# trevorcampbell/bayesian-coresets

Hardware: AMD Instinct MI355X
Metric: greedy coreset iterations/sec (N=10000000, d=512) (higher is better)
Workload: dtype f32 scan + f64 state

## Files before the change

bayesian-coresets_amd/bayesiancoresets_amd/_native.py:

```python
import ctypes
import os

import numpy as np

_HERE = os.path.dirname(os.path.abspath(__file__))
LIB_PATH = os.path.join(os.path.dirname(_HERE), "lib", "libbcx.so")
if not os.path.exists(LIB_PATH) and os.path.exists(os.path.join(_HERE, "_lib", "libbcx.so")):
    LIB_PATH = os.path.join(_HERE, "_lib", "libbcx.so")

ALG_GIGA, ALG_FW, ALG_OMP = 0, 1, 2
F32, F64, F16 = 0, 1, 2
OK, ERR_ARG, ERR_HIP, ERR_ZERO_ROW, ERR_ZERO_B, ERR_NOMEM, ERR_STATE, ERR_EXCHANGE, ERR_TIMEOUT = 0, -1, -2, -3, -4, -5, -6, -7, -8
IT_OK, IT_FAIL_SELECT, IT_FAIL_REWEIGHT, IT_FAIL_MONOTONE = 0, 1, 2, 3
REC_HDR = 4
LOAD_CENTER_ROWS = 1
MAX_ROW_LENGTH = 1048576
CHUNK_ROWS = 1024

SYMBOLS = (
    "bcx_create", "bcx_destroy", "bcx_last_error", "bcx_set_stream", "bcx_load_rows", "bcx_chunk_sums", "bcx_export_chunk_sums",
    "bcx_finalize", "bcx_build_begin", "bcx_step_scan", "bcx_step_apply", "bcx_build_enqueue", "bcx_build_poll",
    "bcx_step_scan_exact", "bcx_build_trace", "bcx_active_count", "bcx_get_weights", "bcx_error", "bcx_optimize",
    "bcx_reset", "bcx_reached_numeric_limit", "bcx_get_vector", "bcx_get_norms", "bcx_get_stored_rows", "bcx_argmax_correlation", "bcx_time_scan",
    "bcx_stats", "bcx_screen_stats", "bcx_screen4_stats", "bcx_screen_read", "bcx_screen4_read", "bcx_screen4_probe", "bcx_profile_scan", "bcx_profile_read", "bcx_version",
    "bcx_project_write", "bcx_project_colsum", "bcx_project_select", "bcx_project_last_error",
    "bcx_build_enqueue_exact", "bcx_exchange_export", "bcx_exchange_attach", "bcx_exchange_probe", "bcx_exchange_disable", "bcx_exchange_set_timeout",
    "bcx_set_check_monotone", "bcx_project_profile", "bcx_project_profile_read", "bcx_exchange_stats", "bcx_load_rows_flags", "bcx_project_write_raw", "bcx_omp_stats", "bcx_project_select_ws", "bcx_project_select_scratch_bytes",
    "bcx_project_moments", "bcx_project_colsum_moments", "bcx_project_moments_scratch_bytes",
    "bcx_project_colsum_moments_scratch_bytes", "bcx_gram", "bcx_gram_scratch_bytes", "bcx_gram_check",
    "bcx_project_colsum_moments_at", "bcx_project_points_colsum_moments", "bcx_linreg_posterior_draw", "bcx_sparsevi_adam_step",
    "bcx_linreg_posterior_apply", "bcx_linreg_posterior_apply_ok",
    "bcx_linreg_posterior_factor", "bcx_linreg_posterior_factor_scratch_bytes", "bcx_linreg_posterior_factor_status",
    "bcx_linreg_posterior_factor_clear_status",
    "bcx_linreg_posterior_draw_factored",
    "bcx_sparsevi_adam_step_ws", "bcx_sparsevi_adam_scratch_bytes", "bcx_standard_normal", "bcx_column_means",
    "bcx_center_rows", "bcx_row_sumsq", "bcx_project_write_points",
    "bcx_laplace_sampler", "bcx_laplace_sampler_ok", "bcx_laplace_sampler_lds_bytes",
    "bcx_project_grad_points", "bcx_psvi_gradient", "bcx_psvi_gradient_scratch_bytes",
    "bcx_gaussian_operand", "bcx_gaussian_first_moment", "bcx_gaussian_first_moment_scratch_bytes", "bcx_gaussian_colsum_moments",
    "bcx_gaussian_posterior_draw", "bcx_project_grad_points_gaussian", "bcx_psvi_gradient_gaussian",
    "bcx_psvi_adam_step",
    "bcx_project_colsum_rows", "bcx_project_select_rows_ws", "bcx_project_select_rows_scratch_bytes", "bcx_gather_rows",
    "bcx_log_joint_grad", "bcx_log_joint_grad_scratch_bytes", "bcx_hmc_coreset", "bcx_hmc_coreset_ok", "bcx_hmc_coreset_lds_bytes",
    "bcx_hmc_stream", "bcx_hmc_stream_scratch_bytes",
    "bcx_nuts_coreset", "bcx_nuts_coreset_ok", "bcx_nuts_coreset_lds_bytes",
    "bcx_nuts_adapt", "bcx_nuts_adapt_ok", "bcx_nuts_adapt_schedule",
    "bcx_nuts_batch", "bcx_nuts_batch_table_bytes",
    "bcx_nuts_stream", "bcx_nuts_stream_scratch_bytes",
    "bcx_log_predictive", "bcx_log_predictive_scratch_bytes",
    "bcx_laplace_sampler_stream", "bcx_laplace_stream_scratch_bytes",
    "bcx_quasi_newton_step", "bcx_quasi_newton_scratch_bytes",
    "bcx_cmc_advance", "bcx_cmc_advance_ok", "bcx_cmc_advance_lds_bytes", "bcx_cmc_state_bytes",
    "bcx_pair_stat", "bcx_pair_stat_scratch_bytes",
)


class Config(ctypes.Structure):
    _fields_ = [
        ("alg", ctypes.c_int32), ("store_dtype", ctypes.c_int32), ("keep_exact_rows", ctypes.c_int32),
        ("device", ctypes.c_int32), ("d", ctypes.c_int32), ("world_size", ctypes.c_int32),
        ("rank", ctypes.c_int32), ("refresh_every", ctypes.c_int32),
        ("n_local", ctypes.c_int64), ("n_global", ctypes.c_int64), ("row_offset", ctypes.c_int64),
    ]


class NutsProblem(ctypes.Structure):
    _fields_ = [
        ("w_dev", ctypes.c_void_p), ("pts_dev", ctypes.c_void_p), ("ldp", ctypes.c_int64),
        ("mu_dev", ctypes.c_void_p), ("W_dev", ctypes.c_void_p), ("ldw", ctypes.c_int64),
        ("k", ctypes.c_int32), ("index", ctypes.c_int32),
    ]


_lib = None


def ensure_ipc_mode():
    import logging
    cur = os.environ.get("HSA_ENABLE_IPC_MODE_LEGACY")
    if cur == "0":
        return True
    if os.environ.get("BCX_KEEP_IPC_MODE"):
        return False
    initialised = False
    try:
        import sys
        t = sys.modules.get("torch")
        initialised = bool(t is not None and t.cuda.is_initialized())
    except Exception:
        pass
    os.environ["HSA_ENABLE_IPC_MODE_LEGACY"] = "0"
    if initialised:
        logging.getLogger().warning("bayesiancoresets_amd: the HIP runtime was initialised before HSA_ENABLE_IPC_MODE_LEGACY=0 "
                                    "could be set (it was %r); peer mailboxes / RCCL between processes may fail -- export it "
                                    "before the first GPU call", cur)
    return not initialised


def load():
    global _lib
    if _lib is not None:
        return _lib
    if not os.path.exists(LIB_PATH):
        raise RuntimeError(
            "libbcx.so not found at %s -- build it with `make -C bayesian-coresets_amd` "
            "(or python -c 'import __graft_entry__ as g; g.build()'). There is no CPU fallback." % LIB_PATH)
    ensure_ipc_mode()
    if not os.environ.get("BCX_NO_TORCH_PRELOAD"):
        try:
            import torch
        except ImportError:
            pass
    lib = ctypes.CDLL(LIB_PATH)
    vp, i32, i64, dbl = ctypes.c_void_p, ctypes.c_int32, ctypes.c_int64, ctypes.c_double
    P = ctypes.POINTER
    lib.bcx_version.restype = ctypes.c_char_p
    lib.bcx_last_error.restype = ctypes.c_char_p
    lib.bcx_last_error.argtypes = [vp]
    sigs = {
        "bcx_create": [P(Config), P(vp)],
        "bcx_destroy": [vp],
        "bcx_set_stream": [vp, vp],
        "bcx_load_rows": [vp, vp, i32, i32, i64, i64, i64],
        "bcx_load_rows_flags": [vp, vp, i32, i32, i64, i64, i64, i32],
        "bcx_chunk_sums": [vp, P(vp), P(i64), P(i64)],
        "bcx_export_chunk_sums": [vp, vp, i64],
        "bcx_finalize": [vp, vp, vp, i64],
        "bcx_build_begin": [vp, i64, dbl, P(i32)],
        "bcx_step_scan": [vp, vp],
        "bcx_step_scan_exact": [vp, vp],
        "bcx_step_apply": [vp, vp],
        "bcx_build_enqueue": [vp, i64],
        "bcx_build_poll": [vp, P(i64), P(i32), P(i32)],
        "bcx_build_trace": [vp, vp, vp, vp, i64, P(i64)],
        "bcx_active_count": [vp, P(i64)],
        "bcx_get_weights": [vp, vp, vp, i64, P(i64)],
        "bcx_error": [vp, P(dbl)],
        "bcx_optimize": [vp, dbl, P(i32)],
        "bcx_reset": [vp],
        "bcx_set_check_monotone": [vp, i32],
        "bcx_reached_numeric_limit": [vp, P(i32)],
        "bcx_get_vector": [vp, i32, vp],
        "bcx_get_norms": [vp, i64, i64, vp],
        "bcx_get_stored_rows": [vp, i64, i64, vp, P(i32)],
        "bcx_argmax_correlation": [vp, vp, P(i64), P(dbl)],
        "bcx_time_scan": [vp, i32, i32, P(dbl), P(dbl)],
        "bcx_stats": [vp, P(i64), P(i64), P(i64)],
        "bcx_omp_stats": [vp, vp],
        "bcx_screen_stats": [vp, vp],
        "bcx_screen4_stats": [vp, vp],
        "bcx_screen_read": [vp, i64, i64, vp, vp, vp, P(i32)],
        "bcx_screen4_read": [vp, i64, i64, vp, vp, vp, P(i32)],
        "bcx_screen4_probe": [vp, vp, vp, P(i32), vp, vp, i32, vp],
        "bcx_profile_scan": [vp, i32],
        "bcx_profile_read": [vp, P(dbl), P(i64)],
        "bcx_build_enqueue_exact": [vp],
        "bcx_exchange_export": [vp, vp, i32],
        "bcx_exchange_attach": [vp, vp, i32, dbl],
        "bcx_exchange_probe": [vp, P(i32)],
        "bcx_exchange_disable": [vp],
        "bcx_exchange_set_timeout": [vp, dbl],
        "bcx_exchange_stats": [vp, P(i64), P(dbl), P(dbl), P(dbl), P(dbl), i32],
    }
    proj_common = [vp, i32, vp, i64, i64, i32, i32, vp, i32, i32, dbl]
    sigs["bcx_project_write"] = proj_common + [vp, i64, vp]
    sigs["bcx_project_write_raw"] = proj_common + [vp, i64]
    sigs["bcx_project_write_points"] = proj_common + [vp, i64, i32]
    sigs["bcx_project_colsum"] = proj_common + [vp, vp]
    sigs["bcx_project_select"] = proj_common + [vp, dbl, vp, vp]
    sigs["bcx_project_select_ws"] = proj_common + [vp, dbl, vp, vp, i64]
    sigs["bcx_project_colsum_rows"] = proj_common + [vp, i64, vp, vp]
    sigs["bcx_project_select_rows_ws"] = proj_common + [vp, i64, vp, dbl, vp, vp, i64]
    sigs["bcx_gather_rows"] = [vp, vp, i64, i32, vp, i64, vp, i64]
    sigs["bcx_project_profile"] = [i32]
    sigs["bcx_project_profile_read"] = [P(dbl), P(i64), P(dbl)]
    sigs["bcx_project_moments"] = [vp, vp, i64, i64, i32, vp, i64, vp, i64]
    sigs["bcx_project_colsum_moments"] = [vp, vp, i64, i32, i32, vp, i32, i32, dbl, vp, vp]
    sigs["bcx_project_colsum_moments_at"] = [vp, vp, i64, i32, i32, vp, i32, i32, dbl, vp, vp, vp]
    sigs["bcx_project_points_colsum_moments"] = [vp, vp, i64, i64, i32, i32, vp, i32, i32, dbl, vp, i64, vp, i64, i32, vp, vp, vp]
    sigs["bcx_linreg_posterior_draw"] = [vp, i32, i32, i32, vp, vp, vp, vp, vp, vp, vp, vp, dbl, vp, vp, i32, vp, vp]
    sigs["bcx_linreg_posterior_apply"] = [vp, i32, i32, i32, vp, vp, vp, vp, vp, vp, vp, dbl, vp, vp, i32, vp, vp, vp]
    sigs["bcx_linreg_posterior_apply_ok"] = [i32, i32]
    sigs["bcx_sparsevi_adam_step"] = [vp, i32, i32, vp, dbl, vp, i64, vp, vp, vp, vp, i32, dbl, dbl, dbl, vp, i32]
    sigs["bcx_gram"] = [vp, vp, i32, i32, i64, vp, i64, vp, i64]
    sigs["bcx_gram_check"] = [vp, vp]
    sigs["bcx_linreg_posterior_factor"] = [vp, i32, i32, i32, vp, vp, vp, vp, i32, vp, dbl, vp, i64, vp, i64, vp, vp]
    sigs["bcx_linreg_posterior_factor_status"] = [vp, i32, vp]
    sigs["bcx_linreg_posterior_factor_clear_status"] = [vp, i32, vp]
    sigs["bcx_standard_normal"] = [vp, ctypes.c_uint64, ctypes.c_uint64, i64, vp]
    sigs["bcx_column_means"] = [vp, vp, i32, i32, i32, i64, vp, i64]
    sigs["bcx_center_rows"] = [vp, vp, i64, i32, i64]
    sigs["bcx_laplace_sampler"] = [vp, i32, i32, i32, vp, vp, i64, vp, i32, dbl, i32, vp, vp, i32, i32, vp, vp, vp]
    sigs["bcx_laplace_sampler_ok"] = [i32, i32]
    lib.bcx_laplace_sampler_lds_bytes.restype = ctypes.c_int64
    lib.bcx_laplace_sampler_lds_bytes.argtypes = [i32, i32]
    sigs["bcx_laplace_sampler_stream"] = sigs["bcx_laplace_sampler"] + [vp, i64]
    lib.bcx_laplace_stream_scratch_bytes.restype = ctypes.c_int64
    lib.bcx_laplace_stream_scratch_bytes.argtypes = [i32, i32]
    sigs["bcx_row_sumsq"] = [vp, vp, i64, i32, i64, vp]
    sigs["bcx_project_grad_points"] = [vp, i32, vp, i32, i64, i32, i32, vp, i32, i32, dbl, vp, vp]
    sigs["bcx_psvi_gradient"] = [vp, i32, vp, i32, i64, i32, i32, vp, i32, i32, dbl, vp, vp, i64, vp, dbl, vp, vp]
    sigs["bcx_gaussian_operand"] = [vp, vp, i32, i64, i32, vp, i64, vp, vp, i64, i32, vp]
    sigs["bcx_gaussian_first_moment"] = [vp, vp, i64, i64, i32, vp, vp, i64]
    lib.bcx_gaussian_first_moment_scratch_bytes.restype = ctypes.c_int64
    lib.bcx_gaussian_first_moment_scratch_bytes.argtypes = [i64, i32]
    sigs["bcx_gaussian_colsum_moments"] = [vp, vp, dbl, i32, vp, i32, i64, vp]
    sigs["bcx_gaussian_posterior_draw"] = [vp, i32, i32, vp, vp, i64, vp, vp, vp, vp, vp, vp, vp, i32, i32, vp, vp, vp, vp]
    sigs["bcx_project_grad_points_gaussian"] = [vp, vp, i32, i64, i32, vp, i32, i64, vp, vp]
    sigs["bcx_psvi_gradient_gaussian"] = [vp, vp, i32, i64, i32, vp, i32, i64, vp, vp, i64, vp, dbl, vp, vp]
    sigs["bcx_psvi_adam_step"] = [vp, i32, i32, vp, i32, vp, vp, i64, vp, vp, vp, i32, dbl, dbl, dbl, vp, i64, vp, vp]
    sigs["bcx_log_joint_grad"] = [vp, i32, vp, i64, i64, i32, vp, vp, i32, i32, vp, vp, vp]
    lib.bcx_log_joint_grad_scratch_bytes.restype = ctypes.c_int64
    lib.bcx_log_joint_grad_scratch_bytes.argtypes = [i64, i32, i32]
    hmc_common = [vp, vp, i64, i32, i32, i32, i32, dbl, dbl, vp, i32, vp, vp, vp, vp, vp, vp, vp]
    sigs["bcx_hmc_coreset"] = [vp, i32, i32, i32, vp, vp, i64] + hmc_common
    sigs["bcx_hmc_stream"] = [vp, i32, i64, i32, vp, vp, i64] + hmc_common + [vp, i64]
    sigs["bcx_hmc_coreset_ok"] = [i32, i32]
    lib.bcx_hmc_coreset_lds_bytes.restype = ctypes.c_int64
    lib.bcx_hmc_coreset_lds_bytes.argtypes = [i32, i32]
    sigs["bcx_cmc_advance"] = [vp, i32, i32, i32, vp, vp, i64, vp, vp, i64, i32, i32, i32, dbl, i32, i32, i32, vp, vp, vp, i64, i64, vp, i64,
                               vp, i64, vp, i32, vp, vp, vp, vp, vp]
    sigs["bcx_cmc_advance_ok"] = [i32, i32]
    lib.bcx_cmc_advance_lds_bytes.restype = ctypes.c_int64
    lib.bcx_cmc_advance_lds_bytes.argtypes = [i32, i32]
    lib.bcx_cmc_state_bytes.restype = ctypes.c_int64
    lib.bcx_cmc_state_bytes.argtypes = [i32]
    sigs["bcx_nuts_coreset"] = [vp, i32, i32, i32, vp, vp, i64, vp, vp, i64, i32, i32, i32, i32, dbl, dbl, vp, i64, i32, vp, vp, vp, vp, vp, vp, vp]
    sigs["bcx_nuts_coreset_ok"] = [i32, i32]
    lib.bcx_nuts_coreset_lds_bytes.restype = ctypes.c_int64
    lib.bcx_nuts_coreset_lds_bytes.argtypes = [i32, i32]
    sigs["bcx_nuts_adapt"] = sigs["bcx_nuts_coreset"] + [i32, vp, vp]
    sigs["bcx_nuts_adapt_ok"] = [i32, i32]
    sigs["bcx_nuts_adapt_schedule"] = [i32, ctypes.POINTER(ctypes.c_int32), i32]
    sigs["bcx_nuts_batch"] = [vp, i32, i32, ctypes.POINTER(NutsProblem), vp, i32, i32, i32, i32, i32, dbl, vp, i64, i32, vp, vp, vp, vp, vp, vp,
                              vp, i32, vp, vp]
    lib.bcx_nuts_batch_table_bytes.restype = ctypes.c_int64
# ... 232 lines not shown
            if done < itrs and not limit:
                self.enqueue(itrs - done)
        return self.trace(itrs)

    def sparse_weights(self):
        k = ctypes.c_int64()
        self._check(self.lib.bcx_active_count(self.h, ctypes.byref(k)))
        idx = np.empty(k.value, dtype=np.int64)
        w = np.empty(k.value, dtype=np.float64)
        if k.value:
            self._check(self.lib.bcx_get_weights(self.h, idx.ctypes.data, w.ctypes.data, k.value, ctypes.byref(k)))
        return idx, w

    def error(self):
        e = ctypes.c_double()
        self._check(self.lib.bcx_error(self.h, ctypes.byref(e)))
        return e.value

    def optimize(self, tol):
        acc = ctypes.c_int32()
        self._check(self.lib.bcx_optimize(self.h, tol, ctypes.byref(acc)))
        return bool(acc.value)

    def reset(self):
        self._check(self.lib.bcx_reset(self.h))

    def set_check_monotone(self, on):
        self._check(self.lib.bcx_set_check_monotone(self.h, int(bool(on))))

    def reached_numeric_limit(self):
        v = ctypes.c_int32()
        self._check(self.lib.bcx_reached_numeric_limit(self.h, ctypes.byref(v)))
        return bool(v.value)

    def vector(self, which):
        out = np.empty(self.d, dtype=np.float64)
        self._check(self.lib.bcx_get_vector(self.h, which, out.ctypes.data))
        return out

    def norms(self, begin=0, count=None):
        count = self.n_local - begin if count is None else count
        out = np.empty(count, dtype=np.float64)
        if count:
            self._check(self.lib.bcx_get_norms(self.h, begin, count, out.ctypes.data))
        return out

    def stored_rows(self, begin=0, count=None):
        count = self.n_local - begin if count is None else count
        ld = ctypes.c_int32()
        self._check(self.lib.bcx_get_stored_rows(self.h, begin, 0, None, ctypes.byref(ld)))
        dt = {F64: np.float64, F16: np.float16}.get(self.cfg.store_dtype, np.float32)
        out = np.empty((count, ld.value), dtype=dt)
        if count:
            self._check(self.lib.bcx_get_stored_rows(self.h, begin, count, out.ctypes.data, ctypes.byref(ld)))
        return out[:, :self.d]

    def argmax_correlation(self, query):
        q = np.ascontiguousarray(query, dtype=np.float64)
        assert q.shape == (self.d,)
        idx, score = ctypes.c_int64(), ctypes.c_double()
        self._check(self.lib.bcx_argmax_correlation(self.h, ctypes.c_void_p(q.ctypes.data), ctypes.byref(idx),
                                                    ctypes.byref(score)))
        return idx.value, score.value

    def time_scan(self, reps=20, exact=False):
        ms, by = ctypes.c_double(), ctypes.c_double()
        self._check(self.lib.bcx_time_scan(self.h, reps, int(exact), ctypes.byref(ms), ctypes.byref(by)))
        return ms.value, by.value

    def stats(self):
        a, b, c = ctypes.c_int64(), ctypes.c_int64(), ctypes.c_int64()
        self._check(self.lib.bcx_stats(self.h, ctypes.byref(a), ctypes.byref(b), ctypes.byref(c)))
        return {"exact_fallbacks": a.value, "candidates": b.value, "resolves": c.value}

    SCREEN_DROP = {0: "in use", 1: "dropped by the overflow rule until reset()", 2: "no device memory for the shadow",
                   3: "switched off or not applicable"}

    SCREEN4_STATE = {0: "in use", 1: "dropped to 8-bit", 2: "no device memory for the second shadow",
                     3: "switched off or not applicable"}

    def screen_stats(self):
        out = (ctypes.c_int64 * 8)()
        self._check(self.lib.bcx_screen_stats(self.h, out))
        o4 = (ctypes.c_int64 * 8)()
        self._check(self.lib.bcx_screen4_stats(self.h, o4))
        return {"active": bool(out[0]), "screened": out[1], "survivors": out[2], "overflows": out[3], "storage_redos": out[4],
                "state": self.SCREEN_DROP.get(int(out[5]), "?"), "device_bytes": out[6], "build_us": out[7],
                "front4_active": bool(o4[0]), "front4_iterations": o4[1], "front4_listed": o4[2], "front4_overflows": o4[3],
                "front4_redos": o4[4], "front4_state": self.SCREEN4_STATE.get(int(o4[5]), "?"), "front4_device_bytes": o4[6],
                "front4_drops": o4[7]}

    def screen_read(self, begin=0, count=None):
        count = self.n_local - begin if count is None else count
        ld8 = (self.d + 15) // 16 * 16
        codes = np.empty((count, ld8), dtype=np.uint8)
        sc = np.empty(count, dtype=np.float32)
        bd = np.empty(count, dtype=np.float32)
        got = ctypes.c_int32()
        self._check(self.lib.bcx_screen_read(self.h, begin, count, codes.ctypes.data, sc.ctypes.data, bd.ctypes.data,
                                             ctypes.byref(got)))
        assert got.value == ld8
        return codes, sc, bd

    def screen4_read(self, begin=0, count=None):
        count = self.n_local - begin if count is None else count
        ld4 = (self.d + 31) // 32 * 16
        codes = np.empty((count, ld4), dtype=np.uint8)
        sc = np.empty(count, dtype=np.float32)
        bd = np.empty(count, dtype=np.float32)
        got = ctypes.c_int32()
        self._check(self.lib.bcx_screen4_read(self.h, begin, count, codes.ctypes.data, sc.ctypes.data, bd.ctypes.data,
                                              ctypes.byref(got)))
        assert got.value == ld4
        return codes, sc, bd

    SCREEN4_MAX_WAVES = 2048

    def screen4_probe(self, query, sentinels, list_stride=1024):
        q = np.ascontiguousarray(query, dtype=np.float64)
        sent = np.ascontiguousarray(sentinels, dtype=np.int32)
        assert q.shape == (self.d,) and sent.shape == (64,)
        cap = self.SCREEN4_MAX_WAVES
        nw = ctypes.c_int32()
        counts = np.zeros(cap, dtype=np.int32)
        lst = np.full((cap, list_stride), -1, dtype=np.int32)
        raw = np.zeros(cap * 40, dtype=np.uint8)
        self._check(self.lib.bcx_screen4_probe(self.h, q.ctypes.data, sent.ctypes.data, ctypes.byref(nw), counts.ctypes.data,
                                               lst.ctypes.data, list_stride, raw.ctypes.data))
        n = nw.value
        dbl = raw[:32 * n].view(np.float64).reshape(4, n)
        idx = raw[32 * n:40 * n].view(np.int32).reshape(2, n)
        return {"counts": counts[:n].copy(), "list": lst[:n].copy(), "U1": dbl[0].copy(), "U2": dbl[1].copy(), "U3": dbl[2].copy(),
                "L": dbl[3].copy(), "i1": idx[0].copy(), "i2": idx[1].copy()}

    def omp_stats(self):
        out = (ctypes.c_int64 * 4)()
        self._check(self.lib.bcx_omp_stats(self.h, out))
        return {"steps": out[0], "columns_left": out[1], "resolves": out[2], "extra_entered": out[3]}

    def profile(self, on):
        self._check(self.lib.bcx_profile_scan(self.h, int(on)))

    def profile_read(self):
        ms, n = ctypes.c_double(), ctypes.c_int64()
        self._check(self.lib.bcx_profile_read(self.h, ctypes.byref(ms), ctypes.byref(n)))
        return ms.value, n.value


def device_row_sumsq(rows):
    import torch
    lib = load()
    if rows.dtype != torch.float64 or rows.stride(1) != 1:
        rows = rows.to(torch.float64).contiguous()
    out = torch.empty(rows.shape[0], dtype=torch.float64, device=rows.device)
    with torch.cuda.device(rows.device):
        rc = lib.bcx_row_sumsq(int(torch.cuda.current_stream(rows.device).cuda_stream), rows.data_ptr(), rows.shape[0], rows.shape[1],
                               rows.stride(0), out.data_ptr())
    if rc != 0:
        raise EngineError(rc, lib.bcx_project_last_error().decode())
    return out.cpu().numpy()


def device_centred_copy(rows):
    import torch
    lib = load()
    out = rows.to(torch.float64).contiguous().clone()
    with torch.cuda.device(out.device):
        rc = lib.bcx_center_rows(int(torch.cuda.current_stream(out.device).cuda_stream), out.data_ptr(), out.shape[0], out.shape[1], out.stride(0))
    if rc != 0:
        raise EngineError(rc, lib.bcx_project_last_error().decode())
    return out
```

bayesian-coresets_amd/csrc/api.hip:

```cpp
#include <stdio.h>
#include <string.h>
#include <algorithm>
#include <cmath>
#include "bcx_internal.h"
#include "dev_util.h"

static thread_local std::string g_create_err;
namespace {
void bounce_acquire(int device);
void bounce_release(int device);
}

extern "C" const char* bcx_version(void) { return "bcx 0.1 gfx950"; }

extern "C" const char* bcx_last_error(const bcx_solver* s) { return s ? s->err.c_str() : g_create_err.c_str(); }

template <typename T> static hipError_t dev_alloc(T** p, size_t count, bool zero = true) {
  *p = nullptr;
  if (count == 0) count = 1;
  hipError_t e = hipMalloc((void**)p, count * sizeof(T));
  if (e != hipSuccess) return e;
  if (zero) e = hipMemset(*p, 0, count * sizeof(T));
  return e;
}

static int round_up(int x, int m) { return (x + m - 1) / m * m; }

static void free_all(bcx_solver* s) {
  void* ptrs[] = {s->An, s->A64, s->norms, s->chunk_sums, s->staging, s->st, s->b, s->bn, s->xw, s->q64, s->qst,
                  s->tmp, s->partials, s->rec_local, s->act_idx, s->act_w, s->act_rows, s->act_norm, s->gram,
                  s->hinv, s->hinv_lo, s->cvec, s->plist, s->ppos, s->nn_x, s->nn_z, s->nn_wv, s->nn_tmp, s->nn_flag, s->nn_wbak, s->nn_xr, s->tr_sel, s->tr_err,
                  s->tr_status};
  for (void* p : ptrs)
    if (p) (void)hipFree(p);
  for (size_t w = 0; w < s->peer_mbox.size(); ++w)
    if (s->peer_mbox[w] && s->peer_mbox[w] != s->mbox) (void)hipIpcCloseMemHandle(s->peer_mbox[w]);
  void* xptrs[] = {s->mbox, s->peer_tab, s->xseq, s->xprobe, s->rec_gather, s->grid_counter, s->fin_part, s->gram_work, s->warm_buf,
                   s->Aq, s->scr_sb, s->scr_partials, s->scr_stat, s->A4, s->s4_sb, s->s4_list, s->s4_counts, s->s4_sent};
  for (void* p : xptrs)
    if (p) (void)hipFree(p);
  for (auto& ev : s->prof_events) { (void)hipEventDestroy(ev.first); (void)hipEventDestroy(ev.second); }
}

extern "C" int bcx_create(const bcx_config* cfg, bcx_solver** out) {
  if (!cfg || !out) { g_create_err = "bcx_create: null argument"; return BCX_ERR_ARG; }
  *out = nullptr;
  if (cfg->alg < BCX_ALG_GIGA || cfg->alg > BCX_ALG_OMP || cfg->d < 1 || cfg->n_local < 0 ||
      cfg->world_size < 1 || cfg->rank < 0 || cfg->rank >= cfg->world_size ||
      (cfg->store_dtype != BCX_F32 && cfg->store_dtype != BCX_F64 && cfg->store_dtype != BCX_F16)) {
    g_create_err = "bcx_create: invalid configuration";
    return BCX_ERR_ARG;
  }
  const int maxd = BCX_MAX_D;
  if (cfg->d > maxd) { g_create_err = "bcx_create: d exceeds the supported row length (" + std::to_string(maxd) + ")"; return BCX_ERR_ARG; }
  if (cfg->n_local >= (int64_t)0x7fffffff) { g_create_err = "bcx_create: n_local must be < 2^31 per shard"; return BCX_ERR_ARG; }
  if (cfg->row_offset % BCX_CHUNK_ROWS != 0) {
    g_create_err = "bcx_create: row_offset must be a multiple of the chunk size (1024 rows)";
    return BCX_ERR_ARG;
  }
  bcx_solver* s = new bcx_solver();
  s->cfg = *cfg;
  if (s->cfg.refresh_every == 0) s->cfg.refresh_every = 64;
  if (const char* e = bcx_dev_env("BCX_SCREEN8")) s->scr_enabled = atoi(e) != 0;
  if (const char* e = bcx_dev_env("BCX_SCREEN4_SEGCAP")) { const int v = atoi(e); if (v >= 1 && v <= BCX_S4_SEG_CAP) s->s4_seg_cap = v; }
  if (const char* e = bcx_dev_env("BCX_SCREEN4")) s->s4_enabled = atoi(e) != 0;
  hipError_t e = hipSetDevice(cfg->device);
  if (e != hipSuccess) { g_create_err = std::string("hipSetDevice: ") + hipGetErrorString(e); delete s; return BCX_ERR_HIP; }
  const int d = cfg->d;
  const int64_t n = cfg->n_local;
  s->elem = cfg->store_dtype == BCX_F32 ? 4 : (cfg->store_dtype == BCX_F16 ? 2 : 8);
  s->qelem = cfg->store_dtype == BCX_F64 ? 8 : 4;
  s->ld = round_up(d, 16 / s->elem);
  s->ld64 = round_up(d, 2);
  s->n_chunks = (n + BCX_CHUNK_ROWS - 1) / BCX_CHUNK_ROWS;
  bool ok = true;
  auto chk = [&](hipError_t r) { if (r != hipSuccess && ok) { ok = false; g_create_err = std::string("hipMalloc: ") + hipGetErrorString(r); } };
  chk(dev_alloc((char**)&s->An, (size_t)n * s->ld * s->elem));
  if (cfg->keep_exact_rows && cfg->store_dtype != BCX_F64) chk(dev_alloc(&s->A64, (size_t)n * s->ld64));
  chk(dev_alloc(&s->norms, (size_t)n));
  chk(dev_alloc(&s->chunk_sums, (size_t)s->n_chunks * (d + 1)));
  chk(dev_alloc(&s->st, 1));
  chk(dev_alloc(&s->b, (size_t)d));
  chk(dev_alloc(&s->bn, (size_t)d));
  chk(dev_alloc(&s->xw, (size_t)d));
  chk(dev_alloc(&s->q64, (size_t)2 * s->ld64));
  chk(dev_alloc((char**)&s->qst, (size_t)2 * s->ld * s->qelem));
  chk(dev_alloc(&s->tmp, (size_t)20 * d));
  s->n_partials = 0;
  chk(dev_alloc((char**)&s->partials, (size_t)bcx_scan_grid(s) * BCX_PARTIAL_BYTES));
  chk(dev_alloc(&s->rec_local, (size_t)(d + BCX_REC_HDR)));
  if (!ok) { free_all(s); delete s; return BCX_ERR_NOMEM; }
  bounce_acquire(cfg->device);
  *out = s;
  return BCX_OK;
}

extern "C" int bcx_destroy(bcx_solver* s) {
  if (!s) return BCX_OK;
  (void)hipSetDevice(s->cfg.device);
  (void)hipDeviceSynchronize();
  free_all(s);
  bounce_release(s->cfg.device);
  delete s;
  return BCX_OK;
}

extern "C" int bcx_set_stream(bcx_solver* s, void* hip_stream) {
  if (!s) return BCX_ERR_ARG;
  s->stream = (hipStream_t)hip_stream;
  return BCX_OK;
}

static int read_state(bcx_solver* s, DevState* h);

#include <mutex>
#include <thread>
namespace {
constexpr size_t kBounceBytes = (size_t)32 << 20;
constexpr int kMaxDevices = 64;
struct Bounce {
  std::mutex mu;
  void* buf[2] = {nullptr, nullptr};
  int users = 0;
};
Bounce g_bounce[kMaxDevices];
Bounce& bounce_of(int device) { return g_bounce[(device >= 0 && device < kMaxDevices) ? device : 0]; }
void bounce_acquire(int device) {
  Bounce& b = bounce_of(device);
  std::lock_guard<std::mutex> lock(b.mu);
  b.users += 1;
}
void bounce_release(int device) {
  Bounce& b = bounce_of(device);
  std::lock_guard<std::mutex> lock(b.mu);
  if (--b.users <= 0) {
    b.users = 0;
    for (int i = 0; i < 2; ++i)
      if (b.buf[i]) { (void)hipHostFree(b.buf[i]); b.buf[i] = nullptr; }
  }
}

void copy_rows_mt(char* dst, size_t dpitch, const char* src, size_t spitch, size_t width, int64_t rows) {
  const size_t bytes = (size_t)rows * width;
  int nt = (int)std::min<size_t>(8, bytes / ((size_t)2 << 20));
  const unsigned hw = std::thread::hardware_concurrency();
  if (hw && (unsigned)nt > hw) nt = (int)hw;
  auto work = [=](int64_t r0, int64_t r1) {
// ... 265 lines not shown
  s->prof_now = (s->prof_tick++ % s->prof_every) == 0;
  if (!s->prof_now) return BCX_OK;
  if (s->prof_used == s->prof_events.size()) {
    hipEvent_t a, b;
    BCX_HIP(hipEventCreate(&a));
    BCX_HIP(hipEventCreate(&b));
    s->prof_events.emplace_back(a, b);
  }
  BCX_HIP(hipEventRecord(s->prof_events[s->prof_used].first, s->stream));
  return BCX_OK;
}
static int prof_end(bcx_solver* s) {
  if (!s->profile || !s->prof_now) return BCX_OK;
  BCX_HIP(hipEventRecord(s->prof_events[s->prof_used].second, s->stream));
  s->prof_used++;
  return BCX_OK;
}

static int step_scan(bcx_solver* s, void* send_dev, int exact, bool with_tail) {
  if (!s->finalized) { s->err = "solver not finalized"; return BCX_ERR_STATE; }
  double* send = send_dev ? (double*)send_dev : s->rec_local;
  int rc;
  if (exact && (rc = bcx_launch_resume_exact(s))) return rc;
  if ((rc = prof_begin(s))) return rc;
  if ((rc = bcx_launch_scan(s, exact))) return rc;
  if ((rc = prof_end(s))) return rc;
  if (with_tail) return bcx_launch_tail(s, exact);
  return bcx_launch_resolve(s, send, exact);
}

static int front_scan(bcx_solver* s, int exact, bool tier, bool four) {
  int rc;
  if (exact && (rc = bcx_launch_resume_exact(s))) return rc;
  if ((rc = prof_begin(s))) return rc;
  if ((rc = (tier && !exact) ? (four ? bcx_launch_screen4(s) : bcx_launch_screen(s)) : bcx_launch_scan(s, exact))) return rc;
  return prof_end(s);
}

extern "C" int bcx_step_scan(bcx_solver* s, void* send_dev) { if (s) s->scr_batch = false; return s ? step_scan(s, send_dev, 0, false) : BCX_ERR_ARG; }
extern "C" int bcx_step_scan_exact(bcx_solver* s, void* send_dev) { if (s) s->scr_batch = false; return s ? step_scan(s, send_dev, 1, false) : BCX_ERR_ARG; }

extern "C" int bcx_step_apply(bcx_solver* s, const void* recv_dev) {
  if (!s) return BCX_ERR_ARG;
  return bcx_launch_apply(s, recv_dev ? (const double*)recv_dev : s->rec_local);
}

static int enqueue_one_launch(bcx_solver* s, int exact, bool tier, bool four) {
  if (!s->finalized) { s->err = "solver not finalized"; return BCX_ERR_STATE; }
  int rc;
  if (s->cfg.world_size != 1) {
    if (!s->exchange_ready) {
      s->err = "bcx_build_enqueue on a row shard needs bcx_exchange_attach (or drive bcx_step_scan / bcx_step_apply)";
      return BCX_ERR_ARG;
    }
    if ((rc = front_scan(s, exact, tier, false))) return rc;
    return bcx_launch_tail_exchange(s, exact);
  }
  if ((rc = front_scan(s, exact, tier, four))) return rc;
  if (s->cfg.alg == BCX_ALG_OMP) {
    rc = bcx_launch_omp_fused(s, exact);
    if (rc != 1) return rc;
    if ((rc = bcx_launch_resolve(s, s->rec_local, exact))) return rc;
    return bcx_launch_apply(s, s->rec_local);
  }
  return bcx_launch_tail(s, exact);
}

static int enqueue_one(bcx_solver* s, int exact, bool tier, bool four = false) {
  const int rc = enqueue_one_launch(s, exact, tier, four);
  if (rc == BCX_OK) s->enq_unpolled = true;
  return rc;
}

static int enqueue_many(bcx_solver* s, int64_t itrs) {
  int rc = bcx_screen_build(s);
  if (rc != BCX_OK) return rc;
  const bool tier = bcx_screen_on(s) && s->scr_valid;
  if (tier && (rc = bcx_screen4_build(s))) return rc;
  const bool tier4 = tier && bcx_screen4_on(s) && s->s4_valid;
  s->scr_batch = false;
  for (int64_t i = 0; i < itrs; ++i) {
    s->scr_batch = tier;
    const bool four = tier4 && s->s4_warm == 0;
    rc = enqueue_one(s, 0, tier, four);
    if (rc != BCX_OK) return rc;
    if (tier && s->s4_warm > 0) s->s4_warm -= 1;
  }
  return BCX_OK;
}

extern "C" int bcx_build_enqueue(bcx_solver* s, int64_t itrs) {
  if (!s) return BCX_ERR_ARG;
  if (!s->finalized) { s->err = "solver not finalized"; return BCX_ERR_STATE; }
  return enqueue_many(s, itrs);
}

extern "C" int bcx_build_enqueue_exact(bcx_solver* s) {
  if (!s) return BCX_ERR_ARG;
  if (!s->finalized) { s->err = "solver not finalized"; return BCX_ERR_STATE; }
  s->scr_batch = false;
  return enqueue_one(s, 1, false);
}

static int mailbox_alloc(bcx_solver* s) {
  if (s->mbox) return BCX_OK;
  const int world = s->cfg.world_size;
  const size_t bytes = bcx_mailbox_slot_offset(world) + 2 * (size_t)world * (s->cfg.d + BCX_REC_HDR) * sizeof(double);
  hipError_t e = hipExtMallocWithFlags(&s->mbox, bytes, hipDeviceMallocFinegrained);
  if (e != hipSuccess) {
    (void)hipGetLastError();
    s->mbox = nullptr;
    s->err = std::string("peer mailbox: fine-grained allocation failed: ") + hipGetErrorString(e);
    return BCX_ERR_HIP;
  }
  s->mbox_bytes = bytes;
  BCX_HIP(hipMemset(s->mbox, 0, bytes));
  BCX_HIP(hipDeviceSynchronize());
  return BCX_OK;
}

extern "C" int bcx_exchange_export(bcx_solver* s, void* handle_out, int32_t handle_bytes) {
  if (!s || !handle_out) return BCX_ERR_ARG;
  if (handle_bytes < (int32_t)sizeof(hipIpcMemHandle_t)) { s->err = "bcx_exchange_export: handle buffer too small"; return BCX_ERR_ARG; }
  if ((size_t)s->cfg.d * sizeof(double) > 144 * 1024) {
    s->err = "peer mailbox: rows of more than 18432 values exchange their records through the all-gather";
    return BCX_ERR_ARG;
  }
  BCX_HIP(hipSetDevice(s->cfg.device));
  int rc = mailbox_alloc(s);
  if (rc != BCX_OK) return rc;
  hipIpcMemHandle_t h;
  BCX_HIP(hipIpcGetMemHandle(&h, s->mbox));
  memset(handle_out, 0, handle_bytes);
  memcpy(handle_out, &h, sizeof(h));
  return BCX_OK;
}

extern "C" int bcx_exchange_attach(bcx_solver* s, const void* handles, int32_t handle_bytes, double timeout_s) {
  if (!s || !handles) return BCX_ERR_ARG;
  if (s->exchange_ready) return BCX_OK;
  if (!s->mbox) { s->err = "bcx_exchange_attach: call bcx_exchange_export first"; return BCX_ERR_STATE; }
  if (handle_bytes < (int32_t)sizeof(hipIpcMemHandle_t)) return BCX_ERR_ARG;
  BCX_HIP(hipSetDevice(s->cfg.device));
  const int world = s->cfg.world_size;
  if (world > BCX_APPLY_THREADS) { s->err = "peer mailbox supports at most 256 shards"; return BCX_ERR_ARG; }
  s->peer_mbox.assign(world, nullptr);
  for (int w = 0; w < world; ++w) {
    if (w == s->cfg.rank) { s->peer_mbox[w] = s->mbox; continue; }
    hipIpcMemHandle_t h;
    memcpy(&h, (const char*)handles + (size_t)w * handle_bytes, sizeof(h));
    hipError_t e = hipIpcOpenMemHandle(&s->peer_mbox[w], h, hipIpcMemLazyEnablePeerAccess);
    if (e != hipSuccess) {
      (void)hipGetLastError();
      s->peer_mbox[w] = nullptr;
      s->err = "peer mailbox: cannot map shard " + std::to_string(w) + ": " + hipGetErrorString(e);
      for (int v = 0; v < w; ++v)
        if (v != s->cfg.rank && s->peer_mbox[v]) { (void)hipIpcCloseMemHandle(s->peer_mbox[v]); s->peer_mbox[v] = nullptr; }
      s->peer_mbox.clear();
      return BCX_ERR_HIP;
    }
  }
  hipError_t e;
  if ((e = dev_alloc(&s->peer_tab, (size_t)world)) != hipSuccess || (e = dev_alloc(&s->xseq, 8)) != hipSuccess ||
      (e = dev_alloc(&s->xprobe, 1)) != hipSuccess ||
      (e = dev_alloc(&s->rec_gather, (size_t)world * (s->cfg.d + BCX_REC_HDR))) != hipSuccess) {
    s->err = std::string("peer mailbox: ") + hipGetErrorString(e);
    return BCX_ERR_NOMEM;
// ... 250 lines not shown
  BCX_HIP(hipSetDevice(s->cfg.device));
  DevState h;
  int rc = read_state(s, &h);
  if (rc != BCX_OK) return rc;
  DevState forced = h;
  forced.active = 1;
  BCX_HIP(hipMemcpy(s->st, &forced, sizeof forced, hipMemcpyHostToDevice));
  hipEvent_t e0, e1;
  BCX_HIP(hipEventCreate(&e0));
  BCX_HIP(hipEventCreate(&e1));
  for (int i = 0; i < 3 && rc == BCX_OK; ++i) rc = bcx_launch_scan(s, exact);
  if (rc == BCX_OK) (void)hipEventRecord(e0, s->stream);
  for (int i = 0; i < reps && rc == BCX_OK; ++i) rc = bcx_launch_scan(s, exact);
  if (rc != BCX_OK) {
    (void)hipEventDestroy(e0); (void)hipEventDestroy(e1);
    (void)hipMemcpy(s->st, &h, sizeof h, hipMemcpyHostToDevice);
    return rc;
  }
  BCX_HIP(hipEventRecord(e1, s->stream));
  BCX_HIP(hipEventSynchronize(e1));
  float ms = 0.f;
  BCX_HIP(hipEventElapsedTime(&ms, e0, e1));
  BCX_HIP(hipEventDestroy(e0));
  BCX_HIP(hipEventDestroy(e1));
  BCX_HIP(hipMemcpy(s->st, &h, sizeof h, hipMemcpyHostToDevice));
  if (ms_per_launch) *ms_per_launch = (double)ms / reps;
  const bool raw64 = exact && s->cfg.store_dtype != BCX_F64 && s->A64;
  if (bytes_per_launch) *bytes_per_launch = (double)s->cfg.n_local * s->cfg.d * (raw64 ? 8.0 : (double)s->elem);
  return BCX_OK;
}

static int upload_query(bcx_solver* s, const double* query_host, bool with64, double* qn_out, int* E_out) {
  const int d = s->cfg.d;
  std::vector<double> q64((size_t)s->ld64, 0.0);
  double qmax = 0.0;
  for (int j = 0; j < d; ++j) { q64[j] = query_host[j]; qmax = std::fmax(qmax, std::fabs(query_host[j])); }
  const bool scalable = qmax > 0.0 && qmax < INFINITY;
  const int E0 = scalable ? std::ilogb(qmax) : 0;
  double qn = 0.0;
  for (int j = 0; j < d; ++j) { const double t = std::ldexp(query_host[j], -E0); qn += t * t; }
  qn = std::sqrt(qn);
  int E = 0;
  if (with64) BCX_HIP(hipMemcpy(s->q64, q64.data(), (size_t)s->ld64 * 8, hipMemcpyHostToDevice));
  if (s->cfg.store_dtype == BCX_F64) {
    std::vector<double> qs((size_t)s->ld, 0.0);
    for (int j = 0; j < d; ++j) qs[j] = query_host[j];
    BCX_HIP(hipMemcpy(s->qst, qs.data(), (size_t)s->ld * 8, hipMemcpyHostToDevice));
    qn = std::ldexp(qn, E0);
  } else {
    const int E1 = (scalable && qn > 0.0 && qn < INFINITY) ? std::ilogb(qn) : 0;
    E = E0 + E1;
    std::vector<float> qs((size_t)s->ld, 0.f);
    for (int j = 0; j < d; ++j) qs[j] = (float)std::ldexp(query_host[j], -E);
    BCX_HIP(hipMemcpy(s->qst, qs.data(), (size_t)s->ld * 4, hipMemcpyHostToDevice));
    qn = std::ldexp(qn, -E1);
  }
  *qn_out = qn; *E_out = E;
  return BCX_OK;
}

extern "C" int bcx_argmax_correlation(bcx_solver* s, const double* query_host, int64_t* idx, double* score) {
  if (!s || !query_host || !idx || !score) return BCX_ERR_ARG;
  if (!s->finalized) { s->err = "solver not finalized"; return BCX_ERR_STATE; }
  if (s->cfg.alg == BCX_ALG_GIGA) { s->err = "bcx_argmax_correlation needs a single-query solver (FW/OMP)"; return BCX_ERR_ARG; }
  BCX_HIP(hipSetDevice(s->cfg.device));
  DevState h;
  int rc = read_state(s, &h);
  if (rc != BCX_OK) return rc;
  double qn = 0.0;
  int E = 0;
  if ((rc = upload_query(s, query_host, true, &qn, &E))) return rc;
  DevState forced = h;
  forced.active = 1; forced.exact_mode = 0; forced.qscale = qn; forced.qexp = E;
  double rec[BCX_REC_HDR];
  for (int attempt = 0; attempt < 2; ++attempt) {
    forced.exact_mode = attempt;
    BCX_HIP(hipMemcpy(s->st, &forced, sizeof forced, hipMemcpyHostToDevice));
    if ((rc = bcx_launch_scan(s, attempt))) return rc;
    if ((rc = bcx_launch_resolve(s, s->rec_local, attempt))) return rc;
    BCX_HIP(hipStreamSynchronize(s->stream));
    BCX_HIP(hipMemcpy(rec, s->rec_local, sizeof rec, hipMemcpyDeviceToHost));
    if (rec[3] != BCX_REC_OVERFLOW) break;
  }
  BCX_HIP(hipMemcpy(s->st, &h, sizeof h, hipMemcpyHostToDevice));
  if (rec[3] != BCX_REC_VALID) { s->err = "no rows to scan"; return BCX_ERR_STATE; }
  *idx = (int64_t)rec[1];
  *score = rec[0];
  return BCX_OK;
}

extern "C" int bcx_stats(bcx_solver* s, int64_t* exact_fallbacks, int64_t* candidates, int64_t* resolves) {
  if (!s) return BCX_ERR_ARG;
  DevState h;
  int rc = read_state(s, &h);
  if (rc != BCX_OK) return rc;
  if (exact_fallbacks) *exact_fallbacks = h.n_exact;
  if (candidates) *candidates = h.n_cand;
  if (resolves) *resolves = h.n_resolved;
  return BCX_OK;
}

extern "C" int bcx_screen_stats(bcx_solver* s, int64_t* out8) {
  if (!s || !out8) return BCX_ERR_ARG;
  unsigned long long st8[SCR_WORDS] = {0, 0, 0, 0, 0, 0, 0, 0};
  if (s->scr_stat) {
    BCX_HIP(hipSetDevice(s->cfg.device));
    BCX_HIP(hipStreamSynchronize(s->stream));
    BCX_HIP(hipMemcpy(st8, s->scr_stat, sizeof st8, hipMemcpyDeviceToHost));
  }
  const bool possible = s->scr_enabled && s->cfg.store_dtype != BCX_F64 && s->cfg.d <= 4096 && s->cfg.n_local > 0;
  out8[0] = bcx_screen_on(s) ? 1 : 0;
  out8[1] = (int64_t)st8[SCR_ITERS];
  out8[2] = (int64_t)st8[SCR_SURVIVORS];
  out8[3] = (int64_t)st8[SCR_OVERFLOWS];
  out8[4] = (int64_t)st8[SCR_REDOS];
  out8[5] = !possible ? 3 : s->scr_dropped;
  out8[6] = s->Aq ? (int64_t)s->scr_cap_rows * (s->ld8 + 8) + (int64_t)BCX_MAX_PARTIALS * BCX_PARTIAL_BYTES + SCR_WORDS * 8 : 0;
  out8[7] = (int64_t)(s->scr_build_ms * 1e3f);
  return BCX_OK;
}

extern "C" int bcx_screen4_stats(bcx_solver* s, int64_t* out8) {
  if (!s || !out8) return BCX_ERR_ARG;
  unsigned long long st8[SCR_WORDS];
  for (auto& w : st8) w = 0;
  if (s->scr_stat) {
    BCX_HIP(hipSetDevice(s->cfg.device));
    BCX_HIP(hipStreamSynchronize(s->stream));
    BCX_HIP(hipMemcpy(st8, s->scr_stat, sizeof st8, hipMemcpyDeviceToHost));
  }
  const bool possible = s->s4_enabled && s->scr_enabled && s->cfg.store_dtype != BCX_F64 && s->cfg.d <= 4096 && s->cfg.n_local > 0 &&
                        s->cfg.alg != BCX_ALG_GIGA && s->cfg.world_size == 1;
  out8[0] = bcx_screen4_on(s) ? 1 : 0;
  out8[1] = (int64_t)st8[SCR4_ITERS];
  out8[2] = (int64_t)st8[SCR4_LISTED];
  out8[3] = (int64_t)st8[SCR4_OVERFLOWS];
  out8[4] = s->s4_redos;
  out8[5] = !possible ? 3 : s->s4_dropped;
  out8[6] = s->A4 ? (int64_t)s->s4_cap_rows * (s->ld4 + 8) + (int64_t)BCX_MAX_PARTIALS * (BCX_S4_SEG_CAP + 1) * 4 : 0;
  out8[7] = s->s4_drops;
  return BCX_OK;
}

extern "C" int bcx_screen_read(bcx_solver* s, int64_t begin, int64_t count, void* codes, float* scales, float* bounds, int32_t* ld8_out) {
  if (!s || begin < 0 || count < 0 || begin + count > s->cfg.n_local) return BCX_ERR_ARG;
  if (!s->finalized) { s->err = "solver not finalized"; return BCX_ERR_STATE; }
  BCX_HIP(hipSetDevice(s->cfg.device));
  int rc = bcx_screen_build(s);
  if (rc != BCX_OK) return rc;
  if (!bcx_screen_on(s) || !s->scr_valid) { s->err = "bcx_screen_read: the 8-bit tier is not in use"; return BCX_ERR_STATE; }
  BCX_HIP(hipStreamSynchronize(s->stream));
  if (ld8_out) *ld8_out = s->ld8;
  if (count == 0) return BCX_OK;
  if (codes) BCX_HIP(hipMemcpy(codes, (const char*)s->Aq + (size_t)begin * s->ld8, (size_t)count * s->ld8, hipMemcpyDeviceToHost));
  std::vector<float> sb((size_t)count * 2);
  BCX_HIP(hipMemcpy(sb.data(), (const char*)s->scr_sb + (size_t)begin * 8, (size_t)count * 8, hipMemcpyDeviceToHost));
  for (int64_t i = 0; i < count; ++i) {
    if (scales) scales[i] = sb[2 * i];
    if (bounds) bounds[i] = sb[2 * i + 1];
  }
  return BCX_OK;
}

static int screen4_ready(bcx_solver* s, const char* who) {
  if (!s->finalized) { s->err = "solver not finalized"; return BCX_ERR_STATE; }
  BCX_HIP(hipSetDevice(s->cfg.device));
  int rc = bcx_screen_build(s);
  if (rc != BCX_OK) return rc;
  if (bcx_screen_on(s) && s->scr_valid && (rc = bcx_screen4_build(s))) return rc;
  if (!bcx_screen_on(s) || !s->scr_valid || !bcx_screen4_on(s) || !s->s4_valid) {
    s->err = std::string(who) + ": the 4-bit front pass is not in use";
    return BCX_ERR_STATE;
  }
  return BCX_OK;
}

extern "C" int bcx_screen4_read(bcx_solver* s, int64_t begin, int64_t count, void* codes, float* scales, float* bounds, int32_t* ld4_out) {
  if (!s || begin < 0 || count < 0 || begin + count > s->cfg.n_local) return BCX_ERR_ARG;
  int rc = screen4_ready(s, "bcx_screen4_read");
  if (rc != BCX_OK) return rc;
  BCX_HIP(hipStreamSynchronize(s->stream));
  if (ld4_out) *ld4_out = s->ld4;
  if (count == 0) return BCX_OK;
  if (codes) BCX_HIP(hipMemcpy(codes, (const char*)s->A4 + (size_t)begin * s->ld4, (size_t)count * s->ld4, hipMemcpyDeviceToHost));
  std::vector<float> sb((size_t)count * 2);
  BCX_HIP(hipMemcpy(sb.data(), (const char*)s->s4_sb + (size_t)begin * 8, (size_t)count * 8, hipMemcpyDeviceToHost));
  for (int64_t i = 0; i < count; ++i) {
    if (scales) scales[i] = sb[2 * i];
    if (bounds) bounds[i] = sb[2 * i + 1];
  }
  return BCX_OK;
}

extern "C" int bcx_screen4_probe(bcx_solver* s, const double* query_host, const int32_t* sentinels, int32_t* n_waves_out,
                                 int32_t* counts, int32_t* list, int32_t list_stride, void* partials) {
  if (!s || !query_host || !sentinels || !n_waves_out || list_stride < 0) return BCX_ERR_ARG;
  for (int i = 0; i < BCX_S4_SENTINELS; ++i)
    if (!(sentinels[i] == -1 || (sentinels[i] >= 0 && (int64_t)sentinels[i] < s->cfg.n_local))) {
      s->err = "bcx_screen4_probe: sentinel " + std::to_string(i) + " is neither -1 nor a local row";
      return BCX_ERR_ARG;
    }
  if (s->enq_unpolled) { s->err = "bcx_screen4_probe: iterations are enqueued; call bcx_build_poll first"; return BCX_ERR_STATE; }
  int rc = screen4_ready(s, "bcx_screen4_probe");
  if (rc != BCX_OK) return rc;
  DevState h;
  if ((rc = read_state(s, &h))) return rc;
  BCX_HIP(hipStreamSynchronize(s->stream));
  int32_t sent_was[BCX_S4_SENTINELS];
  std::vector<char> q_was((size_t)s->ld * 4);
  BCX_HIP(hipMemcpy(sent_was, s->s4_sent, sizeof sent_was, hipMemcpyDeviceToHost));
  BCX_HIP(hipMemcpy(q_was.data(), s->qst, q_was.size(), hipMemcpyDeviceToHost));
  double qn = 0.0;
  int E = 0;
  if ((rc = upload_query(s, query_host, false, &qn, &E))) return rc;
  DevState forced = h;
  forced.active = 1; forced.exact_mode = 0; forced.qscale = qn; forced.qexp = E;
  BCX_HIP(hipMemcpy(s->st, &forced, sizeof forced, hipMemcpyHostToDevice));
  BCX_HIP(hipMemcpy(s->s4_sent, sentinels, sizeof sent_was, hipMemcpyHostToDevice));
  int nw = 0;
  rc = bcx_launch_front4_probe(s, &nw);
  hipError_t e = hipStreamSynchronize(s->stream);
  BCX_HIP(hipMemcpy(s->st, &h, sizeof h, hipMemcpyHostToDevice));
  BCX_HIP(hipMemcpy(s->s4_sent, sent_was, sizeof sent_was, hipMemcpyHostToDevice));
  BCX_HIP(hipMemcpy(s->qst, q_was.data(), q_was.size(), hipMemcpyHostToDevice));
  if (rc != BCX_OK) return rc;
  BCX_HIP(e);
  *n_waves_out = nw;
  std::vector<int32_t> cnt((size_t)nw);
  BCX_HIP(hipMemcpy(cnt.data(), s->s4_counts, (size_t)nw * 4, hipMemcpyDeviceToHost));
  if (counts) memcpy(counts, cnt.data(), (size_t)nw * 4);
  if (list && list_stride > 0) {
    std::vector<int32_t> all((size_t)nw * BCX_S4_SEG_CAP);
    BCX_HIP(hipMemcpy(all.data(), s->s4_list, all.size() * 4, hipMemcpyDeviceToHost));
    for (int b = 0; b < nw; ++b) {
      int m = cnt[b] < s->s4_seg_cap ? cnt[b] : s->s4_seg_cap;
      if (m > list_stride) m = list_stride;
      if (m > 0) memcpy(list + (size_t)b * list_stride, all.data() + (size_t)b * BCX_S4_SEG_CAP, (size_t)m * 4);
    }
  }
  if (partials) BCX_HIP(hipMemcpy(partials, s->scr_partials, (size_t)nw * BCX_PARTIAL_BYTES, hipMemcpyDeviceToHost));
  return BCX_OK;
}

extern "C" int bcx_omp_stats(bcx_solver* s, int64_t* out4) {
  if (!s || !out4) return BCX_ERR_ARG;
  DevState h;
  int rc = read_state(s, &h);
  if (rc != BCX_OK) return rc;
  for (int i = 0; i < 4; ++i) out4[i] = h.n_omp[i];
  out4[2] += s->opt_fallbacks;
  return BCX_OK;
}

extern "C" int bcx_profile_scan(bcx_solver* s, int32_t on) {
  if (!s) return BCX_ERR_ARG;
  s->profile = on != 0;
  s->prof_every = on > 1 ? on : 1;
  s->prof_tick = 0;
  s->prof_ms = 0.0;
  s->prof_launches = 0;
  s->prof_used = 0;
  return BCX_OK;
}

extern "C" int bcx_profile_read(bcx_solver* s, double* scan_ms_total, int64_t* scan_launches) {
  if (!s) return BCX_ERR_ARG;
  if (scan_ms_total) *scan_ms_total = s->prof_ms;
  if (scan_launches) *scan_launches = s->prof_launches;
  return BCX_OK;
}

extern "C" int bcx_debug_stamps(bcx_solver* s, long long* out32) {
  DevState h;
  int rc = read_state(s, &h);
  if (rc != BCX_OK) return rc;
  for (int i = 0; i < 32; ++i) out32[i] = h.dbg_t[i];
  return BCX_OK;
}

extern "C" int bcx_debug_wbak(bcx_solver* s, double* out, int32_t count) {
  if (!s || !s->nn_wbak || count > s->gram_cap) return BCX_ERR_ARG;
  BCX_HIP(hipDeviceSynchronize());
  BCX_HIP(hipMemcpy(out, s->nn_wbak, (size_t)count * sizeof(double), hipMemcpyDeviceToHost));
  return BCX_OK;
}
```

bayesian-coresets_amd/csrc/apply_common.h:

```cpp
#pragma once
#include "bcx_internal.h"
#include "dev_util.h"

struct ApplyArgs {
  DevState* st;
  const double* recs;
  int world;
  int d, ld, ld64;
  int alg;
  int store_f64;
  int refresh_every;
  const double* b;
  const double* bn;
  double* xw;
  double* q64;
  void* qst;
  double* tmp;
  int64_t cap;
  int64_t* act_idx;
  double* act_w;
  double* act_rows;
  double* act_norm;
  int64_t* tr_sel;
  double* tr_err;
  int32_t* tr_status;
};

static __device__ __forceinline__ int query_exponent(const ApplyArgs& a, double qnorm) {
  return (a.store_f64 || !(qnorm > 0.0) || !(qnorm < INFINITY)) ? 0 : ilogb(qnorm);
}

static __device__ __forceinline__ void store_query(const ApplyArgs& a, int which, int j, double v, int E = 0) {
  a.q64[(size_t)which * a.ld64 + j] = v;
  if (a.store_f64) ((double*)a.qst)[(size_t)which * a.ld + j] = v;
  else ((float*)a.qst)[(size_t)which * a.ld + j] = (float)(E ? ldexp(v, -E) : v);
}

static __device__ __forceinline__ void set_query_scale(DevState* st, double qnorm, int E) {
  st->qscale = E ? ldexp(qnorm, -E) : qnorm;
  st->qexp = E;
}

static __device__ bool prepare_query(const ApplyArgs& a, double* scratch) {
  DevState* st = a.st;
  const int d = a.d;
  if (a.alg != BCX_ALG_GIGA) {
    const double qn = st->err;
    const int E = query_exponent(a, qn);
    for (int j = threadIdx.x; j < d; j += blockDim.x) store_query(a, 0, j, a.b[j] - a.xw[j], E);
    if (threadIdx.x == 0) set_query_scale(st, qn, E);
    return true;
  }
  const double nw = st->nw;
  double v[1] = {0.0};
  for (int j = threadIdx.x; j < d; j += blockDim.x) v[0] += a.bn[j] * (a.xw[j] / nw);
  block_allsum<1>(v, scratch);
  const double t = v[0];
  double c2[1] = {0.0};
  for (int j = threadIdx.x; j < d; j += blockDim.x) {
    const double xh = a.xw[j] / nw;
    const double c = a.bn[j] - t * xh;
    a.tmp[j] = c;
    c2[0] += c * c;
  }
  block_allsum<1>(c2, scratch);
  const double cn = sqrt(c2[0]);
  if (cn < st->tol) return false;
  for (int j = threadIdx.x; j < d; j += blockDim.x) {
    store_query(a, 0, j, a.tmp[j] / cn);
    store_query(a, 1, j, a.xw[j] / nw);
  }
  if (threadIdx.x == 0) set_query_scale(st, 1.0, 0);
  return true;
}

static __device__ void refresh_state(const ApplyArgs& a, double* scratch, bool recompute_xw) {
  DevState* st = a.st;
  const int d = a.d, k = st->k;
  double v[2] = {0.0, 0.0};
  for (int j = threadIdx.x; j < d; j += blockDim.x) {
    double x;
    if (recompute_xw) {
      x = 0.0;
      int s = 0;
      for (; s + 8 <= k; s += 8) {
        double r[8], w[8];
#pragma unroll
        for (int t = 0; t < 8; ++t) { w[t] = a.act_w[s + t]; r[t] = a.act_rows[(size_t)(s + t) * d + j]; }
#pragma unroll
        for (int t = 0; t < 8; ++t) x += w[t] * r[t];
      }
      for (; s < k; ++s) x += a.act_w[s] * a.act_rows[(size_t)s * d + j];
      a.xw[j] = x;
    } else {
      x = a.xw[j];
    }
    const double r = x - a.b[j];
    v[0] += r * r;
    v[1] += x * x;
  }
  block_allsum<2>(v, scratch);
  if (threadIdx.x == 0) {
    st->err = sqrt(v[0]);
    const double nw = sqrt(v[1]);
    st->nw = (nw == 0.0) ? 1.0 : nw;
    if (recompute_xw) st->since_refresh = 0;
  }
  __syncthreads();
}

static __device__ void prepare_next(const ApplyArgs& a, double* scratch) {
  DevState* st = a.st;
  __shared__ int go;
  for (;;) {
    __syncthreads();
    if (threadIdx.x == 0) {
      go = 1;
      if (st->it >= st->itrs) { st->active = 0; st->halt = HALT_DONE; go = 0; }
    }
    __syncthreads();
    if (!go) return;
    if (a.refresh_every > 0 && st->since_refresh >= a.refresh_every) refresh_state(a, scratch, true);
    const bool ok = prepare_query(a, scratch);
    if (ok) return;
    __syncthreads();
    if (threadIdx.x == 0) {
      const int64_t it = st->it;
      a.tr_sel[it] = -1; a.tr_err[it] = st->err; a.tr_status[it] = BCX_IT_FAIL_SELECT;
      st->it = it + 1;
      if (st->retried) { st->limit = 1; st->active = 0; st->halt = HALT_LIMIT; go = 0; }
      else st->retried = 1;
    }
    __syncthreads();
    if (!go) return;
  }
}


static inline void fill_apply_args(bcx_solver* s, ApplyArgs& a, const double* recs) {
  a.st = s->st;
  a.recs = recs;
  a.world = s->cfg.world_size;
  a.d = s->cfg.d; a.ld = s->ld; a.ld64 = s->ld64;
  a.alg = s->cfg.alg;
  a.store_f64 = s->cfg.store_dtype == BCX_F64;
  a.refresh_every = s->cfg.refresh_every;
  a.b = s->b; a.bn = s->bn; a.xw = s->xw; a.q64 = s->q64; a.qst = s->qst; a.tmp = s->tmp;
  a.cap = s->cap;
  a.act_idx = s->act_idx; a.act_w = s->act_w; a.act_rows = s->act_rows; a.act_norm = s->act_norm;
  a.tr_sel = s->tr_sel; a.tr_err = s->tr_err; a.tr_status = s->tr_status;
}
```

bayesian-coresets_amd/csrc/bcx_internal.h:

```cpp
#pragma once
#include <hip/hip_runtime.h>
#include <stdint.h>
#include <string>
#include <utility>
#include <vector>
#include "../../include/bcx.h"

#define BCX_CHUNK_ROWS 1024
#define BCX_MAX_CAND 64
#define BCX_REC_HDR 4
#define BCX_REC_VALID 1.0
#define BCX_REC_OVERFLOW 2.0
#define BCX_MAX_D BCX_MAX_ROW_LENGTH
#define BCX_SCAN_THREADS 256
#define BCX_APPLY_THREADS 256

enum { HALT_NONE = 0, HALT_DONE = 1, HALT_LIMIT = 2, HALT_NEED_EXACT = 3, HALT_EXCHANGE_TIMEOUT = 4, HALT_GRID_TIMEOUT = 5 };
enum { OMP_IDLE = 0, OMP_DONE = 1, OMP_FAST_TRY = 2, OMP_FAST_ACCEPT = 3, OMP_GENERAL = 4,
       OMP_OPT_FALLBACK = 5 };

struct PartialView {
  double *U1, *U2, *U3, *L;
  int32_t *i1, *i2;
};
#define BCX_PARTIAL_BYTES 40
#define BCX_MAX_PARTIALS 2048
#define BCX_SCREEN_MAX_SURV 256
enum { SCR_ARMED = 0,
       SCR_ITERS = 1,
       SCR_SURVIVORS = 2,
       SCR_OVERFLOWS = 3,
       SCR_REDOS = 4,
       SCR4_ITERS = 5,
       SCR4_LISTED = 6,
       SCR4_OVERFLOWS = 7,
       SCR4_LAST = 8,
       SCR_WORDS = 9 };
#define BCX_S4_SEG_CAP 1024
#define BCX_S4_SENTINELS 64
static inline __host__ __device__ PartialView partial_view(void* base, int n) {
  PartialView v;
  v.U1 = (double*)base; v.U2 = v.U1 + n; v.U3 = v.U2 + n; v.L = v.U3 + n;
  v.i1 = (int32_t*)(v.L + n); v.i2 = v.i1 + n;
  return v;
}

struct Mailbox {
  void* const* peers;
  unsigned long long* seq;
  int32_t* probe;
  unsigned long long* stat;
  int world, rank, recw;
  unsigned off_slots;
  long long timeout_ticks;
};

static inline unsigned bcx_mailbox_slot_offset(int world) { return (unsigned)((2u * world * 8u + 255u) / 256u * 256u); }

struct DevState {
  int64_t itrs;
  int64_t it;
  int32_t active;
  int32_t halt;
  int32_t retried;
  int32_t limit;
  int32_t k;
  int32_t since_refresh;
  int32_t exact_mode;
  int32_t zero_row;
  int32_t no_monotone;
  int32_t np;
  int32_t hvalid;
  int32_t hlo_valid;
  int32_t omp_mode;
  int32_t omp_slot, omp_fresh, omp_checked, omp_p;
  int32_t omp_ill;
  int64_t omp_f;
  double omp_nf, omp_gff, omp_cf, omp_t, omp_inv;
  double tol;
  double err;
  double nw;
  double bnorm;
  double sigma;
  int64_t n_exact;
  int64_t n_cand;
  int64_t n_resolved;
  int64_t n_omp[4];
  double qscale;
  int32_t qexp;
  int32_t qexp_pad;
  long long dbg_t[32];
};

struct bcx_solver {
  bcx_config cfg;
  hipStream_t stream = nullptr;
  std::string err;
  int ld = 0;
  int elem = 4;
  int qelem = 4;
  int ld64 = 0;
  void* An = nullptr;
  double* A64 = nullptr;
  double* norms = nullptr;
  double* chunk_sums = nullptr;
  int64_t n_chunks = 0;
  void* staging = nullptr;
  size_t staging_bytes = 0;
  DevState* st = nullptr;
  double* b = nullptr;
  double* bn = nullptr;
  double* xw = nullptr;
  double* q64 = nullptr;
  void* qst = nullptr;
  double* tmp = nullptr;
  void* partials = nullptr;
  int n_partials = 0;
  double* rec_local = nullptr;
  double* fin_part = nullptr;
  int64_t fin_cap = 0;
  void* mbox = nullptr;
  size_t mbox_bytes = 0;
  std::vector<void*> peer_mbox;
  void** peer_tab = nullptr;
  unsigned long long* xseq = nullptr;
  int32_t* xprobe = nullptr;
  double* rec_gather = nullptr;
  bool exchange_ready = false;
  double exchange_timeout_s = 20.0;
  int64_t cap = 0;
  int64_t* act_idx = nullptr;
  double* act_w = nullptr;
  double* act_rows = nullptr;
  double* act_norm = nullptr;
  double* gram = nullptr;
  double* hinv = nullptr;
  double* hinv_lo = nullptr;
  double* cvec = nullptr;
  int32_t* plist = nullptr;
  int32_t* ppos = nullptr;
  double* nn_x = nullptr;
  double* nn_z = nullptr;
  double* nn_wv = nullptr;
  double* nn_tmp = nullptr;
  int32_t* nn_flag = nullptr;
  double* nn_wbak = nullptr;
  double* nn_xr = nullptr;
  int64_t gram_cap = 0;
  double* gram_work = nullptr;
  size_t gram_work_bytes = 0;
  void* warm_buf = nullptr;
  size_t warm_bytes = 0;
  int64_t opt_warm = 0, opt_warm_failed = 0;
  int64_t k_ub = 0;
  unsigned long long* grid_counter = nullptr;
  uint64_t grid_epoch = 0;
  int64_t opt_fallbacks = 0;
  bool grid_dirty = false;
  size_t omp_lds_allowed = 0;
  int64_t trace_cap = 0;
  int64_t* tr_sel = nullptr;
  double* tr_err = nullptr;
  int32_t* tr_status = nullptr;
  bool finalized = false;
  int64_t rows_loaded = 0;
  void* Aq = nullptr;
  void* scr_sb = nullptr;
  void* scr_partials = nullptr;
  unsigned long long* scr_stat = nullptr;
  int ld8 = 0;
  int64_t scr_cap_rows = 0;
  bool scr_enabled = true;
  int scr_dropped = 0;
  bool scr_valid = false;
  bool scr_batch = false;
  float scr_build_ms = 0.f;
  uint64_t scr_ovf_at[4] = {0, 0, 0, 0};
  int64_t scr_halts = 0;
  int scr_n_in = 0;
  void* A4 = nullptr;
  void* s4_sb = nullptr;
  void* s4_list = nullptr;
  void* s4_counts = nullptr;
  void* s4_sent = nullptr;
  int ld4 = 0;
  int s4_seg_cap = BCX_S4_SEG_CAP;
  int64_t s4_cap_rows = 0;
  bool s4_enabled = true;
  int s4_dropped = 0;
  bool s4_valid = false;
  int s4_warm = 2;
  uint64_t s4_ovf_at[4] = {0, 0, 0, 0};
  int64_t s4_halts = 0;
  int64_t s4_redos = 0, s4_drops = 0;
  bool enq_unpolled = false;
  bool profile = false;
  bool prof_now = false;
  int prof_every = 1;
  int64_t prof_tick = 0;
  double prof_ms = 0.0;
  int64_t prof_launches = 0;
  std::vector<std::pair<hipEvent_t, hipEvent_t>> prof_events;
  size_t prof_used = 0;
};

int bcx_launch_ingest(bcx_solver* s, const void* src, int src_dtype, int64_t ld_src, int64_t row_begin, int64_t rows,
                      int center);
int bcx_launch_finalize(bcx_solver* s, int have_b, const double* gathered, int64_t n_gathered);
int bcx_launch_scan(bcx_solver* s, int exact);
int bcx_launch_resolve(bcx_solver* s, double* send_dev, int exact);
int bcx_launch_begin(bcx_solver* s, int64_t itrs, double tol);
int bcx_launch_apply(bcx_solver* s, const double* recv_dev);
int bcx_launch_tail(bcx_solver* s, int exact);
int bcx_launch_omp_fused(bcx_solver* s, int exact);
int bcx_launch_tail_exchange(bcx_solver* s, int exact);
int bcx_launch_exchange_probe(bcx_solver* s);
Mailbox bcx_mailbox(const bcx_solver* s);
int bcx_launch_resume_exact(bcx_solver* s);
int bcx_launch_error_refresh(bcx_solver* s);
int bcx_launch_optimize(bcx_solver* s, double tol);
int64_t bcx_gram_rows_scratch_bytes(int k, int d);
int bcx_gram_rows(hipStream_t st, const double* rows, int k, int d, int64_t ld, double* G, int64_t ldg, double* work);
int64_t bcx_gram_tiled_scratch_bytes(int k, int d);
int bcx_gram_rows_tiled(hipStream_t st, const double* rows, int k, int d, int64_t ld, double* G, int64_t ldg, double* work);
unsigned long long bcx_gram_sk_epoch_now();
int bcx_gram_sk_timed_out(hipStream_t st, const double* work, unsigned long long since);
int bcx_scan_grid(const bcx_solver* s);
bool bcx_screen_on(const bcx_solver* s);
int bcx_screen_build(bcx_solver* s);
int bcx_launch_screen(bcx_solver* s);
int bcx_launch_resume_store(bcx_solver* s);
int bcx_launch_refine(bcx_solver* s, int n_in, bool four);
bool bcx_screen4_on(const bcx_solver* s);
int bcx_screen4_build(bcx_solver* s);
int bcx_launch_screen4(bcx_solver* s);
int bcx_launch_front4_probe(bcx_solver* s, int* n_waves);
void bcx_project_set_error(const std::string& msg);
const double* proj_tables();

#ifdef BCX_TIMING
#define BCX_STAMP(st, i) do { if (threadIdx.x == 0) (st)->dbg_t[i] = wall_clock64(); } while (0)
#else
#define BCX_STAMP(st, i) do {} while (0)
#endif

#define BCX_HIP(call)                                                        \
  do {                                                                       \
    hipError_t _e = (call);                                                  \
    if (_e != hipSuccess) {                                                  \
      s->err = std::string(#call) + ": " + hipGetErrorString(_e);            \
      return BCX_ERR_HIP;                                                    \
    }                                                                        \
  } while (0)
```

bayesian-coresets_amd/csrc/resolve.hip:

```cpp
#include <hip/hip_fp16.h>
#include "bcx_internal.h"
#include "dev_util.h"
#include "apply_common.h"

#include "resolve_core.h"
#include "tail_core.h"


__global__ __launch_bounds__(256) void resolve_kernel(ResolveArgs a) {
  if (!a.st->active) return;
  __shared__ double scratch[BCX_SCRATCH];
  __shared__ Winner win;
  resolve_core(a, &win, nullptr, scratch);
}

template <int ALG, bool BIG>
__global__ __launch_bounds__(BCX_APPLY_THREADS) void apply_kernel(ApplyArgs a) {
  DevState* st = a.st;
  if (!st->active) return;
  extern __shared__ double dyn[];
  __shared__ double scratch[BCX_SCRATCH];
  __shared__ int s_win, s_overflow;
  const StateVecs v = carve(vec_base<BIG>(a, dyn), a.d);
  const SlotPre pre = slot_prefetch(a);
  stage_state(a, v);
  const int tid = threadIdx.x, d = a.d;
  const int recw = d + BCX_REC_HDR;
  if (tid == 0) {
    int win = -1, ovf = 0;
    for (int r = 0; r < a.world; ++r) {
      const double* rec = a.recs + (size_t)r * recw;
      if (rec[3] == BCX_REC_OVERFLOW) ovf = 1;
      if (rec[3] != BCX_REC_VALID) continue;
      if (win < 0) { win = r; continue; }
      const double* best = a.recs + (size_t)win * recw;
      if (rec[0] > best[0] || (rec[0] == best[0] && rec[1] < best[1])) win = r;
    }
    s_win = win; s_overflow = ovf;
  }
  __syncthreads();
  if (s_overflow) { if (tid == 0) { st->active = 0; st->halt = HALT_NEED_EXACT; } return; }
  if (s_win < 0) { if (tid == 0) { st->active = 0; st->halt = HALT_DONE; } return; }
  const double* rec = a.recs + (size_t)s_win * recw;
  for (int j = tid; j < d; j += blockDim.x) v.xf[j] = rec[BCX_REC_HDR + j];
  const int64_t f = (int64_t)rec[1];
  const double nf = rec[2];
  __syncthreads();
  apply_core<ALG>(a, v, f, nf, scratch, pre);
}

template <int ALG, bool BIG>
__global__ __launch_bounds__(BCX_APPLY_THREADS) void tail_kernel(ResolveArgs r, ApplyArgs a) {
  DevState* st = a.st;
  if (!st->active) return;
  extern __shared__ double dyn[];
  __shared__ double scratch[BCX_SCRATCH];
  __shared__ Winner win;
  BCX_STAMP(st, 0);
  const StateVecs v = carve(vec_base<BIG>(a, dyn), a.d);
  const SlotPre pre = slot_prefetch(a);
  stage_state(a, v);
  resolve_core(r, &win, v.xf, scratch);
  if (win.flags == BCX_REC_OVERFLOW) { if (threadIdx.x == 0) { st->active = 0; st->halt = HALT_NEED_EXACT; } return; }
  if (win.flags != BCX_REC_VALID) { if (threadIdx.x == 0) { st->active = 0; st->halt = HALT_DONE; } return; }
  apply_core<ALG>(a, v, win.gidx, win.norm, scratch, pre);
}

static __device__ __forceinline__ void st_sys(double* p, double v) {
  __hip_atomic_store((unsigned long long*)p, (unsigned long long)__double_as_longlong(v), __ATOMIC_RELAXED,
                     __HIP_MEMORY_SCOPE_SYSTEM);
}
static __device__ __forceinline__ double ld_sys(const double* p) {
  return __longlong_as_double((long long)__hip_atomic_load((const unsigned long long*)p, __ATOMIC_RELAXED,
                                                           __HIP_MEMORY_SCOPE_SYSTEM));
}

static __device__ const double* mailbox_exchange(const Mailbox& m, const double* hdr, const double* row, int* s_flag) {
  const int tid = threadIdx.x;
  const unsigned long long seq = *m.seq + 1;
  const int par = (int)(seq & 1ull);
  const long long t_in = tid == 0 ? wall_clock64() : 0;
  const size_t my_slot = m.off_slots + ((size_t)par * m.world + m.rank) * m.recw * sizeof(double);
  for (int w = 0; w < m.world; ++w) {
    double* dst = (double*)((char*)m.peers[w] + my_slot);
    for (int j = tid; j < m.recw; j += blockDim.x) st_sys(dst + j, j < BCX_REC_HDR ? hdr[j] : row[j - BCX_REC_HDR]);
  }
  __threadfence_system();
  asm volatile("s_waitcnt vmcnt(0)" ::: "memory");
  if (tid == 0) *s_flag = 0;
  __syncthreads();
  const long long t_posted = tid == 0 ? wall_clock64() : 0;
  if (tid < m.world) {
    unsigned long long* out = (unsigned long long*)m.peers[tid] + (par * m.world + m.rank);
    __hip_atomic_store(out, seq, __ATOMIC_RELEASE, __HIP_MEMORY_SCOPE_SYSTEM);
    const unsigned long long* in = (const unsigned long long*)m.peers[m.rank] + (par * m.world + tid);
    const long long t0 = wall_clock64();
    unsigned polls = 0;
    while (__hip_atomic_load(in, __ATOMIC_ACQUIRE, __HIP_MEMORY_SCOPE_SYSTEM) < seq) {
      ++polls;
      if (polls < 64) __builtin_amdgcn_s_sleep(2);
      else if (polls < 256) __builtin_amdgcn_s_sleep(32);
      else { for (int z = 0; z < 40; ++z) __builtin_amdgcn_s_sleep(127); }
      if (wall_clock64() - t0 > m.timeout_ticks) {
        atomicOr(s_flag, 1);
        atomicOr(&m.stat[5], 1ull << (tid & 63));
        m.stat[6] = seq;
        break;
      }
    }
  }
  __syncthreads();
  __threadfence_system();
  if (*s_flag) return nullptr;
  if (tid == 0) {
    *m.seq = seq;
    const unsigned long long now = (unsigned long long)wall_clock64();
    const unsigned long long wait = now - (unsigned long long)t_posted, all = now - (unsigned long long)t_in;
    m.stat[0] += 1ull;
    m.stat[1] += wait; if (wait > m.stat[2]) m.stat[2] = wait;
    m.stat[3] += all;  if (all > m.stat[4]) m.stat[4] = all;
  }
  return (const double*)((const char*)m.peers[m.rank] + m.off_slots + (size_t)par * m.world * m.recw * sizeof(double));
}

static __device__ int pick_record(const double* recs, int world, int recw, int* overflow) {
  int win = -1;
  double bs = 0.0, bi = 0.0;
  *overflow = 0;
  for (int r = 0; r < world; ++r) {
    const double* rec = recs + (size_t)r * recw;
    const double fl = ld_sys(rec + 3);
    if (fl == BCX_REC_OVERFLOW) *overflow = 1;
    if (fl != BCX_REC_VALID) continue;
    const double sc = ld_sys(rec), gi = ld_sys(rec + 1);
    if (win < 0 || sc > bs || (sc == bs && gi < bi)) { win = r; bs = sc; bi = gi; }
  }
  return win;
}

template <int ALG, bool BIG>
__global__ __launch_bounds__(BCX_APPLY_THREADS) void tail_exchange_kernel(ResolveArgs r, ApplyArgs a, Mailbox m) {
  DevState* st = a.st;
  if (!st->active) return;
  extern __shared__ double dyn[];
  __shared__ double scratch[BCX_SCRATCH];
  __shared__ Winner win;
  __shared__ double s_hdr[BCX_REC_HDR];
  __shared__ int s_flag, s_win, s_overflow;
// ... 81 lines not shown
void bcx_fill_resolve_args(bcx_solver* s, ResolveArgs& a, double* send_dev, int exact) {
  a.pv = partial_view(s->partials, s->n_partials);
  a.n_partials = s->n_partials;
  a.st = s->st;
  a.An = s->An;
  a.store_f64 = s->cfg.store_dtype == BCX_F64;
  a.store_f16 = s->cfg.store_dtype == BCX_F16;
  a.ld = s->ld;
  a.A64 = s->A64;
  a.ld64 = s->ld64;
  a.norms = s->norms;
  a.q64 = s->q64;
  a.d = s->cfg.d;
  a.alg = s->cfg.alg;
  a.n_local = s->cfg.n_local;
  a.row_offset = s->cfg.row_offset;
  a.exact = exact || a.store_f64;
  a.need_score = 1;
  a.rec = send_dev;
}

#define BCX_LDS_VEC_MAX_D 3584
static bool vec_big(const bcx_solver* s) { return s->cfg.d > BCX_LDS_VEC_MAX_D; }
static size_t vec_lds_bytes(const bcx_solver* s) { return vec_big(s) ? 0 : 5 * (size_t)s->cfg.d * sizeof(double); }

template <typename K> static int allow_lds(bcx_solver* s, K kfn, size_t bytes) {
  if (bytes > 48 * 1024) BCX_HIP(hipFuncSetAttribute((const void*)kfn, hipFuncAttributeMaxDynamicSharedMemorySize, (int)bytes));
  return BCX_OK;
}

int bcx_launch_resolve(bcx_solver* s, double* send_dev, int exact) {
  ResolveArgs a;
  bcx_fill_resolve_args(s, a, send_dev, exact);
  hipLaunchKernelGGL(resolve_kernel, dim3(1), dim3(256), 0, s->stream, a);
  BCX_HIP(hipGetLastError());
  return BCX_OK;
}

int bcx_launch_begin(bcx_solver* s, int64_t itrs, double tol) {
  ApplyArgs a;
  fill_apply_args(s, a, nullptr);
  hipLaunchKernelGGL(begin_kernel, dim3(1), dim3(BCX_APPLY_THREADS), 0, s->stream, a, itrs, tol);
  BCX_HIP(hipGetLastError());
  return BCX_OK;
}

int bcx_launch_resume_exact(bcx_solver* s) {
  hipLaunchKernelGGL(resume_exact_kernel, dim3(1), dim3(64), 0, s->stream, s->st);
  BCX_HIP(hipGetLastError());
  return BCX_OK;
}

int bcx_launch_apply_omp(bcx_solver* s, const double* recv_dev);

int bcx_launch_apply(bcx_solver* s, const double* recv_dev) {
  if (s->cfg.alg == BCX_ALG_OMP) return bcx_launch_apply_omp(s, recv_dev);
  ApplyArgs a;
  fill_apply_args(s, a, recv_dev);
  const size_t lds = vec_lds_bytes(s);
  int rc;
  if (s->cfg.alg == BCX_ALG_GIGA) {
    if (vec_big(s)) hipLaunchKernelGGL((apply_kernel<BCX_ALG_GIGA, true>), dim3(1), dim3(BCX_APPLY_THREADS), 0, s->stream, a);
    else {
      if ((rc = allow_lds(s, apply_kernel<BCX_ALG_GIGA, false>, lds))) return rc;
      hipLaunchKernelGGL((apply_kernel<BCX_ALG_GIGA, false>), dim3(1), dim3(BCX_APPLY_THREADS), lds, s->stream, a);
    }
  } else {
    if (vec_big(s)) hipLaunchKernelGGL((apply_kernel<BCX_ALG_FW, true>), dim3(1), dim3(BCX_APPLY_THREADS), 0, s->stream, a);
    else {
      if ((rc = allow_lds(s, apply_kernel<BCX_ALG_FW, false>, lds))) return rc;
      hipLaunchKernelGGL((apply_kernel<BCX_ALG_FW, false>), dim3(1), dim3(BCX_APPLY_THREADS), lds, s->stream, a);
    }
  }
  BCX_HIP(hipGetLastError());
  return BCX_OK;
}

int bcx_launch_tail(bcx_solver* s, int exact) {
  ResolveArgs r;
  bcx_fill_resolve_args(s, r, nullptr, exact);
  r.need_score = 0;
  ApplyArgs a;
  fill_apply_args(s, a, nullptr);
  const size_t lds = vec_lds_bytes(s);
  int rc;
  if (s->cfg.alg == BCX_ALG_GIGA) {
    if (vec_big(s)) hipLaunchKernelGGL((tail_kernel<BCX_ALG_GIGA, true>), dim3(1), dim3(BCX_APPLY_THREADS), 0, s->stream, r, a);
    else {
      if ((rc = allow_lds(s, tail_kernel<BCX_ALG_GIGA, false>, lds))) return rc;
      hipLaunchKernelGGL((tail_kernel<BCX_ALG_GIGA, false>), dim3(1), dim3(BCX_APPLY_THREADS), lds, s->stream, r, a);
    }
  } else {
    if (vec_big(s)) hipLaunchKernelGGL((tail_kernel<BCX_ALG_FW, true>), dim3(1), dim3(BCX_APPLY_THREADS), 0, s->stream, r, a);
    else {
      if ((rc = allow_lds(s, tail_kernel<BCX_ALG_FW, false>, lds))) return rc;
      hipLaunchKernelGGL((tail_kernel<BCX_ALG_FW, false>), dim3(1), dim3(BCX_APPLY_THREADS), lds, s->stream, r, a);
    }
  }
  BCX_HIP(hipGetLastError());
  return BCX_OK;
}

Mailbox bcx_mailbox(const bcx_solver* s) {
  Mailbox m;
  m.peers = s->peer_tab;
  m.seq = s->xseq;
  m.stat = s->xseq + 1;
  m.probe = s->xprobe;
  m.world = s->cfg.world_size;
  m.rank = s->cfg.rank;
  m.recw = s->cfg.d + BCX_REC_HDR;
  m.off_slots = bcx_mailbox_slot_offset(s->cfg.world_size);
  m.timeout_ticks = (long long)(s->exchange_timeout_s * 1e8);
  return m;
}

int bcx_launch_tail_exchange(bcx_solver* s, int exact) {
  ResolveArgs r;
  bcx_fill_resolve_args(s, r, nullptr, exact);
  const Mailbox m = bcx_mailbox(s);
  int rc;
  if (s->cfg.alg == BCX_ALG_OMP) {
    const size_t lds = (size_t)s->cfg.d * sizeof(double);
    if ((rc = allow_lds(s, resolve_exchange_kernel, lds))) return rc;
    hipLaunchKernelGGL(resolve_exchange_kernel, dim3(1), dim3(BCX_APPLY_THREADS), lds, s->stream, r, m, s->rec_gather);
    BCX_HIP(hipGetLastError());
    return bcx_launch_apply_omp(s, s->rec_gather);
  }
  ApplyArgs a;
  fill_apply_args(s, a, nullptr);
  const size_t lds = vec_lds_bytes(s);
  if (s->cfg.alg == BCX_ALG_GIGA) {
    if (vec_big(s)) hipLaunchKernelGGL((tail_exchange_kernel<BCX_ALG_GIGA, true>), dim3(1), dim3(BCX_APPLY_THREADS), 0, s->stream, r, a, m);
    else {
      if ((rc = allow_lds(s, tail_exchange_kernel<BCX_ALG_GIGA, false>, lds))) return rc;
      hipLaunchKernelGGL((tail_exchange_kernel<BCX_ALG_GIGA, false>), dim3(1), dim3(BCX_APPLY_THREADS), lds, s->stream, r, a, m);
    }
  } else {
    if (vec_big(s)) hipLaunchKernelGGL((tail_exchange_kernel<BCX_ALG_FW, true>), dim3(1), dim3(BCX_APPLY_THREADS), 0, s->stream, r, a, m);
    else {
      if ((rc = allow_lds(s, tail_exchange_kernel<BCX_ALG_FW, false>, lds))) return rc;
      hipLaunchKernelGGL((tail_exchange_kernel<BCX_ALG_FW, false>), dim3(1), dim3(BCX_APPLY_THREADS), lds, s->stream, r, a, m);
    }
  }
  BCX_HIP(hipGetLastError());
  return BCX_OK;
}

int bcx_launch_exchange_probe(bcx_solver* s) {
  const Mailbox m = bcx_mailbox(s);
  int rc;
  if ((rc = allow_lds(s, exchange_probe_kernel, (size_t)s->cfg.d * sizeof(double)))) return rc;
  hipLaunchKernelGGL(exchange_probe_kernel, dim3(1), dim3(BCX_APPLY_THREADS), (size_t)s->cfg.d * sizeof(double), s->stream, m);
  BCX_HIP(hipGetLastError());
  return BCX_OK;
}

int bcx_launch_error_refresh(bcx_solver* s) {
  ApplyArgs a;
  fill_apply_args(s, a, nullptr);
  hipLaunchKernelGGL(error_refresh_kernel, dim3(1), dim3(BCX_APPLY_THREADS), 0, s->stream, a);
  BCX_HIP(hipGetLastError());
  return BCX_OK;
}
```

bayesian-coresets_amd/csrc/screen4.hip:

```cpp
#include <float.h>
#include "screen_core.h"

#define BCX_S4_CLIP 0.8
#define BCX_S4_QMAX 1911.0
#define BCX_S4_MAX_NW4 512

struct Front4Head { float Lg, qstep, eA, eB; };

template <int CTRL> __device__ __forceinline__ int dpp_mov_i(int v) { return __builtin_amdgcn_update_dpp(0, v, CTRL, 0xf, 0xf, false); }
template <int G> __device__ __forceinline__ int group_allsum_i32(int v) {
  if (G >= 2) v += dpp_mov_i<0xB1>(v);
  if (G >= 4) v += dpp_mov_i<0x4E>(v);
  if (G >= 8) v += dpp_mov_i<0x141>(v);
  if (G >= 16) v += dpp_mov_i<0x140>(v);
  if (G >= 32) { const v2u r = __builtin_amdgcn_permlane16_swap((unsigned)v, (unsigned)v, false, false); const unsigned x = r.x, y = r.y; v = (int)(x + y); }
  if (G >= 64) { const v2u r = __builtin_amdgcn_permlane32_swap((unsigned)v, (unsigned)v, false, false); const unsigned x = r.x, y = r.y; v = (int)(x + y); }
  return v;
}

static __device__ __forceinline__ float round_up_f32(double v) {
  float f = (float)v;
  if ((double)f < v) f = nextafterf(f, INFINITY);
  return f;
}

struct Front4Args {
  const uint4* A4;
  const float2* sb;
  const float* q;
  const int* sent;
  const unsigned char* Aq;
  const float2* sb8;
  const DevState* st;
  int* list;
  int* counts;
  int64_t n;
  int ldv, nw4, seg_cap;
  int ld8, d;
  float kacc, err_coef;
  PartialView out;
  int ldv8;
};

#define BCX_S4_SPW (BCX_S4_SENTINELS / BCX_SCREEN_WAVES)

static __device__ __forceinline__ Front4Head front4_head(const Front4Args& a, int myrow, float2 mysb, float qscale,
                                                         unsigned* planes, double* scratch) {
  const int tid = threadIdx.x, lane = tid & 63, wave = tid >> 6;
  constexpr int NW = BCX_SCREEN_WAVES;
  constexpr int SPW = BCX_S4_SPW;
  int rows[SPW];
#pragma unroll
  for (int r = 0; r < SPW; ++r) rows[r] = __builtin_amdgcn_readlane(myrow, r);
  double acc[SPW];
#pragma unroll
  for (int r = 0; r < SPW; ++r) acc[r] = 0.0;
  double m = 0.0;
  const int nw8 = a.ld8 / 4;
  const unsigned* A8 = (const unsigned*)a.Aq;
  for (int w0 = lane; w0 < nw8; w0 += 128) {
    unsigned cw[2][SPW];
    float qf[2][4];
#pragma unroll
    for (int h = 0; h < 2; ++h) {
      const int w = w0 + 64 * h;
      const int wc = w < nw8 ? w : 0;
#pragma unroll
      for (int k = 0; k < 4; ++k) { const int j = 4 * w + k; qf[h][k] = a.q[(w < nw8 && j < a.d) ? j : 0]; }
#pragma unroll
      for (int r = 0; r < SPW; ++r) cw[h][r] = A8[(int64_t)(rows[r] < 0 ? 0 : rows[r]) * nw8 + wc];
    }
    __builtin_amdgcn_sched_barrier(0);
    double qv[2][4];
#pragma unroll
    for (int h = 0; h < 2; ++h)
#pragma unroll
      for (int k = 0; k < 4; ++k) {
        const int w = w0 + 64 * h, j = 4 * w + k;
        qv[h][k] = (w < nw8 && j < a.d) ? (double)qf[h][k] : 0.0;
        const double v = fabs(qv[h][k]);
        m = fmax(m, v == v ? v : INFINITY);
      }
#pragma unroll
    for (int h = 0; h < 2; ++h)
#pragma unroll
      for (int r = 0; r < SPW; ++r)
#pragma unroll
        for (int k = 0; k < 4; ++k) acc[r] = fma((double)((int)((cw[h][r] >> (8 * k)) & 0xffu) - 128), qv[h][k], acc[r]);
  }
  double tot = 0.0;
#pragma unroll
  for (int r = 0; r < SPW; ++r) { const double t = wave_allsum(acc[r]); tot = (lane & (SPW - 1)) == r ? t : tot; }
  float lmax = -INFINITY;
  {
    const float s0 = (float)((double)mysb.x * tot);
    float U, L;
    screen_interval(s0, mysb.x, mysb.y, a.kacc, a.err_coef, qscale, U, L);
    if (myrow >= 0) lmax = fmaxf(lmax, L);
  }
  lmax = (float)wave_allmax((double)lmax);
  m = wave_allmax(m);
  float step = (float)(m / BCX_S4_QMAX);
  const bool qok = m < INFINITY && step >= FLT_MIN;
  if (!qok) step = 0.0f;
  double err2 = 0.0;
  for (int w = tid; w < a.nw4; w += BCX_SCAN_THREADS) {
    unsigned p0 = 0, p1 = 0, p2 = 0;
    float q8[8];
#pragma unroll
    for (int k = 0; k < 8; ++k) { const int j = 8 * w + k; q8[k] = a.q[j < a.d ? j : 0]; }
#pragma unroll
    for (int k = 0; k < 8; ++k) {
      const int j = 8 * w + k;
      int x = 0;
      if (j < a.d && qok) {
        const double v = (double)q8[k];
        double c = rint(v / (double)step);
        c = c > BCX_S4_QMAX ? BCX_S4_QMAX : (c < -BCX_S4_QMAX ? -BCX_S4_QMAX : c);
        x = (int)c;
        const double r = v - c * (double)step;
        err2 = fma(r, r, err2);
      }
      const int l = ((x + 8) & 15) - 8;
      const int x1 = (x - l) >> 4;
      const int h1 = ((x1 + 8) & 15) - 8;
      const int h2 = (x1 - h1) >> 4;
      p0 |= (unsigned)(l & 15) << (4 * k); p1 |= (unsigned)(h1 & 15) << (4 * k); p2 |= (unsigned)(h2 & 15) << (4 * k);
    }
    planes[w] = p0; planes[a.nw4 + w] = p1; planes[2 * a.nw4 + w] = p2;
  }
  err2 = wave_allsum(err2);
  if (lane == 0) { scratch[wave] = err2; scratch[NW + wave] = (double)lmax; }
  __syncthreads();
  err2 = scratch[0];
  double lg = scratch[NW];
#pragma unroll
  for (int w = 1; w < NW; ++w) { err2 += scratch[w]; lg = fmax(lg, scratch[NW + w]); }
  const double qerr = sqrt(err2) * (1.0 + 9.5367431640625e-07);
  const double qs = (double)qscale;
  Front4Head h;
  h.Lg = qok ? (float)lg : -INFINITY;
  h.qstep = step;
  h.eA = round_up_f32((qs * 1.000002 + qerr) * 1.000004);
  h.eB = round_up_f32(((double)a.err_coef * qs + 1.001 * qerr) * 1.000004 + 1e-37);
  return h;
}

template <int G, int CH, int UR>
__device__ __forceinline__ void settle8(const Front4Args& a, const int* seg, int b, int cnt, float qscale) {
  constexpr int RPW = 64 / G;
  const int lane = threadIdx.x & 63;
  const int sub = lane % G, rsub = lane / G;
  const bool ovf = cnt > a.seg_cap;

  Track<float> tr;
  tr.U1 = tr.U2 = tr.U3 = tr.L = -INFINITY;
  tr.i1 = tr.i2 = 0x7fffffff;
  if (!ovf && cnt > 0) {
    Q16 q0[CH];
    int voff[CH];
    float qs0 = 0.0f;
#pragma unroll
    for (int c = 0; c < CH; ++c) {
      const int v = c * G + sub;
      const bool ok = v < a.ldv8;
      voff[c] = ok ? v : 0;
      q0[c] = load_q16(a.q, v, a.d, ok, qs0);
    }
    const float off0 = -128.0f * qs0;
    int nxt[UR];
#pragma unroll
    for (int u = 0; u < UR; ++u) { const int kk = u * RPW + rsub; nxt[u] = kk < cnt ? seg[kk] : -1; }
    for (int k0 = 0; k0 < cnt; k0 += RPW * UR) {
      int row[UR];
      uint4 x[UR][CH];
      float2 sbv[UR];
#pragma unroll
      for (int u = 0; u < UR; ++u) row[u] = nxt[u];
#pragma unroll
      for (int u = 0; u < UR; ++u) { const int kk = k0 + RPW * UR + u * RPW + rsub; nxt[u] = kk < cnt ? seg[kk] : -1; }
#pragma unroll
      for (int u = 0; u < UR; ++u) {
        const int64_t rc = row[u] < 0 ? 0 : row[u];
        const uint4* p = (const uint4*)a.Aq + rc * a.ldv8;
#pragma unroll
        for (int c = 0; c < CH; ++c) x[u][c] = stream_load(p + voff[c]);
        sbv[u] = a.sb8[rc];
      }
      __builtin_amdgcn_sched_barrier(0);
#pragma unroll
      for (int u = 0; u < UR; ++u) {
        float t0 = off0;
#pragma unroll
        for (int c = 0; c < CH; ++c) t0 = dot16(x[u][c], q0[c], t0);
        float s0 = group_allsum<float, G>(t0);
        s0 *= sbv[u].x;
        float U, L;
        screen_interval(s0, sbv[u].x, sbv[u].y, a.kacc, a.err_coef, qscale, U, L);
        if (row[u] < 0) { U = -INFINITY; L = -INFINITY; }
        track_update<float>(tr, U, L, row[u] < 0 ? 0x7fffffff : row[u]);
      }
    }
#pragma unroll
    for (int off = G; off < 64; off <<= 1) tr = merge<float>(tr, shfl_track<float>(tr, off));
  }
  if (lane == 0) {
    if (ovf) {
      tr.U1 = tr.U2 = tr.L = -INFINITY; tr.U3 = INFINITY; tr.i1 = tr.i2 = 0x7fffffff;
    }
    a.out.U1[b] = (double)tr.U1; a.out.U2[b] = (double)tr.U2; a.out.U3[b] = (double)tr.U3; a.out.L[b] = (double)tr.L;
    a.out.i1[b] = tr.i1; a.out.i2[b] = tr.i2;
  }
}

template <int G, int CH, int UR, int G8, int CH8, int UR8>
__global__ __launch_bounds__(BCX_SCAN_THREADS) void front4_kernel(Front4Args a) {
  int myrow = a.sent[(threadIdx.x >> 6) * BCX_S4_SPW + (threadIdx.x & (BCX_S4_SPW - 1))];
  const float qscale = (float)a.st->qscale;
  const int active = a.st->active;
  asm volatile("" : "+v"(myrow));
  if (!active) return;
  if (!(myrow >= 0 && (int64_t)myrow < a.n)) myrow = -1;
  const float2 mysb = a.sb8[myrow < 0 ? 0 : myrow];
  __shared__ double scratch[BCX_SCRATCH];
  __shared__ unsigned planes[3 * BCX_S4_MAX_NW4];
  __shared__ int lseg[BCX_SCREEN_WAVES][BCX_S4_SEG_CAP];
  constexpr int RPW = 64 / G;
  constexpr int WAVES = BCX_SCREEN_WAVES;
  constexpr int RPB = WAVES * RPW * UR;
  const int lane = threadIdx.x & 63, wave = threadIdx.x >> 6;
  const int sub = lane % G, rsub = lane / G;
  int voff[CH];
  bool vok[CH];
#pragma unroll
  for (int c = 0; c < CH; ++c) {
    const int v = c * G + sub;
    vok[c] = v < a.ldv;
    voff[c] = vok[c] ? v : 0;
  }
  const int b = blockIdx.x * WAVES + wave;
  int* seg = a.list + (size_t)b * BCX_S4_SEG_CAP;
  int cnt = 0;
  const int64_t n = a.n;
  const int64_t stride = (int64_t)gridDim.x * RPB;
  uint4 x[UR][CH];
  float2 sbv[UR];
  auto load_trip = [&](int64_t r0) {
#pragma unroll
    for (int u = 0; u < UR; ++u) {
      const int64_t rw = r0 + (int64_t)(u * WAVES + wave) * RPW + rsub;
      const int64_t rc = rw < n ? rw : n - 1;
      const uint4* p = a.A4 + rc * a.ldv;
#pragma unroll
      for (int c = 0; c < CH; ++c) x[u][c] = stream_load(p + voff[c]);
      sbv[u] = a.sb[rc];
    }
  };
  int64_t r0 = (int64_t)blockIdx.x * RPB;
  load_trip(r0);
  __builtin_amdgcn_sched_barrier(0);
  const Front4Head h = front4_head(a, myrow, mysb, qscale, planes, scratch);
  int qp[CH][4][3];
#pragma unroll
  for (int c = 0; c < CH; ++c)
#pragma unroll
    for (int k = 0; k < 4; ++k)
#pragma unroll
      for (int p = 0; p < 3; ++p) qp[c][k][p] = vok[c] ? (int)planes[p * a.nw4 + 4 * voff[c] + k] : 0;
  for (;;) {
    __builtin_amdgcn_sched_barrier(0);
#pragma unroll
    for (int u = 0; u < UR; ++u) {
      int a0 = 0, a1 = 0, a2 = 0;
#pragma unroll
      for (int c = 0; c < CH; ++c) {
        const unsigned xs[4] = {x[u][c].x, x[u][c].y, x[u][c].z, x[u][c].w};
#pragma unroll
        for (int k = 0; k < 4; ++k) {
          const int cw = (int)(xs[k] ^ 0x88888888u);
          a0 = __builtin_amdgcn_sdot8(cw, qp[c][k][0], a0, false);
          a1 = __builtin_amdgcn_sdot8(cw, qp[c][k][1], a1, false);
          a2 = __builtin_amdgcn_sdot8(cw, qp[c][k][2], a2, false);
        }
      }
      const int tot = group_allsum_i32<G>((a2 * 16 + a1) * 16 + a0);
      const float s4 = (sbv[u].x * h.qstep) * (float)tot;
      const float e4 = fmaf(sbv[u].y, h.eA, h.eB) + fabsf(s4) * 5e-7f;
      const float U4 = s4 + e4;
      const int64_t rw = r0 + (int64_t)(u * WAVES + wave) * RPW + rsub;
      const bool want = rw < n && sub == 0 && !(U4 < h.Lg);
      const unsigned long long bal = __ballot(want);
      if (bal) {
        const int pos = cnt + (int)__builtin_amdgcn_mbcnt_hi((unsigned)(bal >> 32), __builtin_amdgcn_mbcnt_lo((unsigned)bal, 0u));
        if (want && pos < a.seg_cap) { seg[pos] = (int)rw; lseg[wave][pos] = (int)rw; }
        cnt += __popcll(bal);
      }
    }
    r0 += stride;
    if (!(r0 < n)) break;
    load_trip(r0);
  }
  if (lane == 0) a.counts[b] = cnt;
  settle8<G8, CH8, UR8>(a, lseg[wave], b, cnt, qscale);
}

template <bool F16>
__global__ __launch_bounds__(256) void quantise4_kernel(const void* An, int ld, int d, int nw4, int64_t n, unsigned* A4, float2* sb) {
  const int lane = threadIdx.x & 63;
  const int64_t row = (int64_t)blockIdx.x * 4 + (threadIdx.x >> 6);
  if (row >= n) return;
  auto elem = [&](int j) -> float {
    if (F16) return __half2float(((const __half*)An)[row * (int64_t)ld + j]);
    return ((const float*)An)[row * (int64_t)ld + j];
  };
  float m = 0.0f;
  for (int j = lane; j < d; j += 64) m = fmaxf(m, fabsf(elem(j)));
  m = (float)wave_allmax((double)m);
  float sc = (float)((double)m * BCX_S4_CLIP / 7.0);
  if (!(sc >= FLT_MIN)) sc = FLT_MIN;
  const double dsc = (double)sc;
  double r2 = 0.0;
  for (int w = lane; w < nw4; w += 64) {
    unsigned word = 0;
#pragma unroll
    for (int k = 0; k < 8; ++k) {
      const int j = 8 * w + k;
      int code = 0;
      if (j < d) {
        const double v = (double)elem(j);
        double c = rint(v / dsc);
        c = c > 7.0 ? 7.0 : (c < -7.0 ? -7.0 : c);
        if (c != c) c = 0.0;
        code = (int)c;
        const double r = v - c * dsc;
        r2 = fma(r, r, r2);
      }
      word |= (unsigned)(code + 8) << (4 * k);
    }
    A4[row * (int64_t)nw4 + w] = word;
  }
  r2 = wave_allsum(r2);
  if (lane == 0) {
    const double b = sqrt(r2) * (1.0 + 9.5367431640625e-07);
    float bf = (float)b;
    if ((double)bf < b) bf = nextafterf(bf, INFINITY);
    if (!(bf == bf)) bf = INFINITY;
    sb[row] = make_float2(sc, bf);
  }
}

bool bcx_screen4_on(const bcx_solver* s) {
  return s->s4_enabled && !s->s4_dropped && bcx_screen_on(s) && s->cfg.alg != BCX_ALG_GIGA && s->cfg.world_size == 1;
}

int bcx_screen4_build(bcx_solver* s) {
  if (s->s4_valid || !bcx_screen4_on(s) || !s->scr_valid) return BCX_OK;
  const int d = s->cfg.d;
  const int64_t n = s->cfg.n_local;
  s->ld4 = (d + 31) / 32 * 16;
  const int nw4 = s->ld4 / 4;
  if (s->s4_cap_rows < n || !s->A4) {
    void** all[] = {&s->A4, &s->s4_sb, &s->s4_list, &s->s4_counts, &s->s4_sent};
    for (void** p : all) { if (*p) (void)hipFree(*p); *p = nullptr; }
    s->s4_cap_rows = 0;
    hipError_t e = hipMalloc(&s->A4, (size_t)n * s->ld4);
    if (e == hipSuccess) e = hipMalloc(&s->s4_sb, (size_t)n * 8);
    if (e == hipSuccess) e = hipMalloc(&s->s4_list, (size_t)BCX_MAX_PARTIALS * BCX_S4_SEG_CAP * 4);
    if (e == hipSuccess) e = hipMalloc(&s->s4_counts, (size_t)BCX_MAX_PARTIALS * 4);
    if (e == hipSuccess) e = hipMalloc(&s->s4_sent, (size_t)BCX_S4_SENTINELS * 4);
    if (e != hipSuccess) {
      (void)hipGetLastError();
      for (void** p : all) { if (*p) (void)hipFree(*p); *p = nullptr; }
      s->s4_dropped = 2;
      return BCX_OK;
    }
    s->s4_cap_rows = n;
    BCX_HIP(hipMemsetAsync(s->s4_sent, 0xff, (size_t)BCX_S4_SENTINELS * 4, s->stream));
  }
  const unsigned grid = (unsigned)((n + 3) / 4);
  if (s->cfg.store_dtype == BCX_F16)
    hipLaunchKernelGGL((quantise4_kernel<true>), dim3(grid), dim3(256), 0, s->stream, s->An, s->ld, d, nw4, n, (unsigned*)s->A4, (float2*)s->s4_sb);
  else
    hipLaunchKernelGGL((quantise4_kernel<false>), dim3(grid), dim3(256), 0, s->stream, s->An, s->ld, d, nw4, n, (unsigned*)s->A4, (float2*)s->s4_sb);
  BCX_HIP(hipGetLastError());
  s->s4_valid = true;
  s->s4_warm = 2;
  return BCX_OK;
}

static int launch_front4(bcx_solver* s, const Front4Args& a, int G, int CH, int G8, int CH8, int grid) {
  dim3 g(grid), b(BCX_SCAN_THREADS);
#define L(GG, CC, UU, G8_, C8_, U8_)                                                                   \
  if (G == GG && CH == CC && G8 == G8_ && CH8 == C8_) {                                                \
    hipLaunchKernelGGL((front4_kernel<GG, CC, UU, G8_, C8_, U8_>), g, b, 0, s->stream, a);             \
    return BCX_OK;                                                                                     \
  }
  L(1, 1, 8, 1, 1, 16) L(1, 1, 8, 2, 1, 16) L(2, 1, 8, 4, 1, 16) L(4, 1, 8, 8, 1, 16) L(8, 1, 8, 16, 1, 16)
  L(16, 1, 8, 32, 1, 16) L(32, 1, 8, 64, 1, 16) L(64, 1, 8, 64, 2, 8) L(64, 2, 4, 64, 4, 4)
#undef L
  s->err = "front4: unsupported row length";
  return BCX_ERR_ARG;
}

struct Front4Plan { Front4Args f; int G, CH, G8, CH8, grid, n_in; };

static int front4_plan(bcx_solver* s, Front4Plan* p) {
  const int d = s->cfg.d;
  const int64_t n = s->cfg.n_local;
  const int nw4 = s->ld4 / 4;
  if (nw4 > BCX_S4_MAX_NW4) { s->err = "front4: unsupported row length"; return BCX_ERR_ARG; }
  ScanArgs sa;
  ScanPlan sp;
  int rc = bcx_scan_plan(s, 0, &sa, &sp);
  if (rc != BCX_OK) return rc;
  const int ldv8 = s->ld8 / 16;
  const int G8 = screen_group(ldv8), CH8 = screen_chunks(ldv8, G8);
  const float kacc = screen_kacc(G8, CH8, d);

  Front4Args& f = p->f;
  f.A4 = (const uint4*)s->A4; f.sb = (const float2*)s->s4_sb; f.q = (const float*)s->qst; f.sent = (const int*)s->s4_sent;
  f.Aq = (const unsigned char*)s->Aq; f.sb8 = (const float2*)s->scr_sb; f.st = s->st;
  f.list = (int*)s->s4_list; f.counts = (int*)s->s4_counts;
  f.n = n; f.ldv = s->ld4 / 16; f.nw4 = nw4; f.seg_cap = s->s4_seg_cap;
  f.ld8 = s->ld8; f.d = d; f.kacc = kacc; f.err_coef = sa.err_coef;
  const int G = screen_group(f.ldv), CH = screen_chunks(f.ldv, G);
  const int ur = CH == 1 ? 8 : 4;
  const int rpb = BCX_SCREEN_WAVES * (64 / G) * ur;
  const int64_t want = (n + rpb - 1) / rpb;
  int cap = 512;
  if (cap > BCX_MAX_PARTIALS / BCX_SCREEN_WAVES) cap = BCX_MAX_PARTIALS / BCX_SCREEN_WAVES;
  const int grid = (int)(want < 1 ? 1 : (want > cap ? cap : want));

  const int n_in = grid * BCX_SCREEN_WAVES;
  f.out = partial_view(s->scr_partials, n_in); f.ldv8 = ldv8;
  p->G = G; p->CH = CH; p->G8 = G8; p->CH8 = CH8; p->grid = grid; p->n_in = n_in;
  return BCX_OK;
}

int bcx_launch_screen4(bcx_solver* s) {
  Front4Plan p;
  int rc = front4_plan(s, &p);
  if (rc != BCX_OK) return rc;
  if ((rc = launch_front4(s, p.f, p.G, p.CH, p.G8, p.CH8, p.grid))) return rc;
  BCX_HIP(hipGetLastError());
  s->scr_n_in = p.n_in;
  return bcx_launch_refine(s, p.n_in, true);
}

int bcx_launch_front4_probe(bcx_solver* s, int* n_waves) {
  Front4Plan p;
  int rc = front4_plan(s, &p);
  if (rc != BCX_OK) return rc;
  if ((rc = launch_front4(s, p.f, p.G, p.CH, p.G8, p.CH8, p.grid))) return rc;
  BCX_HIP(hipGetLastError());
  *n_waves = p.n_in;
  return BCX_OK;
}
```

bayesian-coresets_amd/csrc/screen8.hip:

```cpp
#include <float.h>
#include "screen_core.h"

#define BCX_REFINE_THREADS 1024

struct ScreenArgs {
  const uint4* Aq;
  const float2* sb;
  const float* q;
  const DevState* st;
  PartialView out;
  int64_t n;
  int ldv;
  int ldq;
  int d;
  float kacc;
  float err_coef;
};

template <bool DUAL, int G, int CH, int UR>
__global__ __launch_bounds__(BCX_SCAN_THREADS) void screen_kernel(ScreenArgs a) {
  if (!a.st->active) return;
  constexpr int RPW = 64 / G;
  constexpr int WAVES = BCX_SCREEN_WAVES;
  constexpr int RPB = WAVES * RPW * UR;
// ... 47 lines not shown
    __builtin_amdgcn_sched_barrier(0);
#pragma unroll
    for (int t = 0; t < NT; ++t) {
      float s0, s1 = 0.0f;
      if constexpr (PACK4) {
        float a0[4], a1[4];
#pragma unroll
        for (int u = 0; u < 4; ++u) {
          float t0 = off0, t1 = off1;
#pragma unroll
          for (int c = 0; c < CH; ++c) {
            t0 = dot16(x[t * 4 + u][c], q0[c], t0);
            if (DUAL) t1 = dot16(x[t * 4 + u][c], q1[c], t1);
          }
          a0[u] = t0; a1[u] = t1;
        }
        s0 = reduce4_pack<G, float>(a0[0], a0[1], a0[2], a0[3]);
        if (DUAL) s1 = reduce4_pack<G, float>(a1[0], a1[1], a1[2], a1[3]);
      } else {
        float t0 = off0, t1 = off1;
#pragma unroll
        for (int c = 0; c < CH; ++c) {
          t0 = dot16(x[t][c], q0[c], t0);
          if (DUAL) t1 = dot16(x[t][c], q1[c], t1);
        }
        s0 = group_allsum<float, G>(t0);
        if (DUAL) s1 = group_allsum<float, G>(t1);
      }
      const int64_t myrow = tracked(r0, t);
      const float scale = sbv[t].x, bound = sbv[t].y;
      s0 *= scale; s1 *= scale;
      float U, L;
      if (DUAL) giga_interval(s0, s1, (fmaf(scale, a.kacc, bound) * 1.000002f + a.err_coef) * qscale, U, L);
      else screen_interval(s0, scale, bound, a.kacc, a.err_coef, qscale, U, L);
      if (!(myrow < n)) { U = -INFINITY; L = -INFINITY; }
      track_update<float>(tr, U, L, (int)myrow);
    }
  }
#pragma unroll
  for (int off = GSZ; off < 64; off <<= 1) tr = merge<float>(tr, shfl_track<float>(tr, off));
  if (lane == 0) {
    const int b = blockIdx.x * WAVES + wave;
    a.out.U1[b] = (double)tr.U1; a.out.U2[b] = (double)tr.U2; a.out.U3[b] = (double)tr.U3; a.out.L[b] = (double)tr.L;
    a.out.i1[b] = tr.i1; a.out.i2[b] = tr.i2;
  }
}

struct RefineArgs {
  PartialView in;
  int n_in;
  PartialView out;
  DevState* st;
  unsigned long long* stat;
  const void* An;
  const float* q;
  int store_f16, ld, ldq, d, dual;
  double coef_mid;
  int* sent;
  const int* counts;
  int seg_cap;
  int64_t n;
};

#define BCX_REFINE_PF 8

__global__ __launch_bounds__(BCX_REFINE_THREADS) void refine_kernel(RefineArgs a) {
  if (!a.st->active) return;
  __shared__ double scratch[BCX_SCRATCH];
  __shared__ int surv[BCX_SCREEN_MAX_SURV];
  __shared__ int nsurv, overflow, listed, full;
  constexpr int PP = BCX_MAX_PARTIALS / BCX_REFINE_THREADS;
  const int tid = threadIdx.x, lane = tid & 63, wave = tid >> 6, nwaves = BCX_REFINE_THREADS / 64;
  double u1[PP], u2[PP], u3[PP], lo[PP];
  int r1[PP], r2[PP], cn[PP];
#pragma unroll
  for (int t = 0; t < PP; ++t) {
    const int p = tid + t * BCX_REFINE_THREADS;
    const bool ok = p < a.n_in;
    u1[t] = ok ? a.in.U1[p] : -INFINITY; u2[t] = ok ? a.in.U2[p] : -INFINITY;
    u3[t] = ok ? a.in.U3[p] : -INFINITY; lo[t] = ok ? a.in.L[p] : -INFINITY;
    r1[t] = ok ? a.in.i1[p] : 0; r2[t] = ok ? a.in.i2[p] : 0;
    cn[t] = (ok && a.counts) ? a.counts[p] : 0;
  }
  if (tid == 0) { nsurv = 0; overflow = 0; listed = 0; full = 0; }
  double lmax = -INFINITY;
#pragma unroll
  for (int t = 0; t < PP; ++t) lmax = fmax(lmax, lo[t]);
  const double Lstar = block_allmax(lmax, scratch);
#pragma unroll
  for (int t = 0; t < PP; ++t) {
    if (u1[t] > -INFINITY && u1[t] >= Lstar) { const int s = atomicAdd(&nsurv, 1); if (s < BCX_SCREEN_MAX_SURV) surv[s] = r1[t]; }
    if (u2[t] > -INFINITY && u2[t] >= Lstar) { const int s = atomicAdd(&nsurv, 1); if (s < BCX_SCREEN_MAX_SURV) surv[s] = r2[t]; }
    if (u3[t] > -INFINITY && u3[t] >= Lstar) overflow = 1;
  }
  if (a.counts) {
    double li = 0.0, fu = 0.0;
#pragma unroll
    for (int t = 0; t < PP; ++t) { li += (double)(cn[t] > a.seg_cap ? a.seg_cap : cn[t]); fu += cn[t] > a.seg_cap ? 1.0 : 0.0; }
    li = wave_allsum(li); fu = wave_allsum(fu);
    if (lane == 0) { atomicAdd(&listed, (int)li); atomicAdd(&full, (int)fu); }
  }
  __syncthreads();
  const int ns = nsurv;
  const bool ovf = overflow || ns > BCX_SCREEN_MAX_SURV;
  for (int p = tid; p < BCX_SCREEN_MAX_SURV; p += BCX_REFINE_THREADS) {
    if (ovf || p >= ns) {
      const bool mark = ovf && p == 0;
      a.out.U1[p] = -INFINITY; a.out.U2[p] = -INFINITY; a.out.U3[p] = mark ? INFINITY : -INFINITY; a.out.L[p] = mark ? 0.0 : -INFINITY;
      a.out.i1[p] = 0x7fffffff; a.out.i2[p] = 0x7fffffff;
    }
  }
  if (tid == 0) {
    a.stat[SCR_ARMED] = 1ull;
    atomicAdd(&a.stat[SCR_ITERS], 1ull);
    if (ovf) atomicAdd(&a.stat[SCR_OVERFLOWS], 1ull); else atomicAdd(&a.stat[SCR_SURVIVORS], (unsigned long long)ns);
    a.stat[SCR4_LAST] = a.counts ? 1ull : 0ull;
    if (a.counts) {
      atomicAdd(&a.stat[SCR4_ITERS], 1ull);
      atomicAdd(&a.stat[SCR4_LISTED], (unsigned long long)listed);
      atomicAdd(&a.stat[SCR4_OVERFLOWS], (unsigned long long)full);
    }
  }
  auto stored = [&](int64_t i, int j) -> double {
    return a.store_f16 ? (double)__half2float(((const __half*)a.An)[i * (int64_t)a.ld + j])
                       : (double)((const float*)a.An)[i * (int64_t)a.ld + j];
  };
  double pv[BCX_REFINE_PF];
  float pq0[BCX_REFINE_PF];
  const bool ahead = a.sent && !a.dual && !ovf && wave < ns;
#pragma unroll
  for (int k = 0; k < BCX_REFINE_PF; ++k) { pv[k] = 0.0; pq0[k] = 0.0f; }
  if (ahead) {
    const int64_t row0 = surv[wave];
#pragma unroll
    for (int k = 0; k < BCX_REFINE_PF; ++k) {
      const int j = lane + 64 * k, jc = j < a.d ? j : 0;
      pv[k] = stored(row0, jc); pq0[k] = a.q[jc];
    }
  }
  __builtin_amdgcn_sched_barrier(0);
  if (a.sent) {
    constexpr int SPW = BCX_S4_SENTINELS / (BCX_REFINE_THREADS / 64);
    double cu[2 * PP];
    int ci[2 * PP];
#pragma unroll
    for (int t = 0; t < 2 * PP; ++t) {
      const double u = (t & 1) ? u2[t >> 1] : u1[t >> 1];
      const int i = (t & 1) ? r2[t >> 1] : r1[t >> 1];
      const bool use = u > -INFINITY && u < INFINITY && i >= 0 && (int64_t)i < a.n;
      cu[t] = use ? u : -INFINITY; ci[t] = use ? i : -1;
    }
#pragma unroll
    for (int r = 0; r < SPW; ++r) {
      double best = -INFINITY;
      int bt = -1, bi = -1;
#pragma unroll
      for (int t = 0; t < 2 * PP; ++t) if (cu[t] > best) { best = cu[t]; bt = t; bi = ci[t]; }
      const double wm = wave_allmax(best);
      const unsigned long long bal = __ballot(bt >= 0 && best == wm);
      const int src = bal ? __ffsll((long long)bal) - 1 : 0;
      const int row = __shfl(bi, src, BCX_WAVE);
      if (lane == 0) a.sent[wave * SPW + r] = bal ? row : -1;
#pragma unroll
      for (int t = 0; t < 2 * PP; ++t) if (bal && lane == src && t == bt) cu[t] = -INFINITY;
    }
  }
  if (ovf) return;
  const double qs = a.st->qscale;
  const double e = a.coef_mid * qs;
  for (int c = wave; c < ns; c += nwaves) {
    const int64_t i = surv[c];
    double s0 = 0.0, s1 = 0.0;
    int j = lane;
    if (ahead && c == wave) {
#pragma unroll
      for (int k = 0; k < BCX_REFINE_PF; ++k, j += 64) {
        const double t0 = fma(pv[k], (double)pq0[k], s0);
        s0 = j < a.d ? t0 : s0;
      }
    }
    for (; j < a.d; j += 64) {
      const double v = stored(i, j);
      s0 = fma(v, (double)a.q[j], s0);
      if (a.dual) s1 = fma(v, (double)a.q[a.ldq + j], s1);
    }
    s0 = wave_allsum(s0);
    if (a.dual) s1 = wave_allsum(s1);
    if (lane == 0) {
      double U, L;
      if (a.dual) {
        float Uf, Lf;
        giga_interval((float)s0, (float)s1, (float)(e * 1.000001) , Uf, Lf);
        U = Uf; L = Lf;
      } else { U = s0 + e; L = s0 - e; }
      a.out.U1[c] = U; a.out.L[c] = L; a.out.i1[c] = (int)i;
      a.out.U2[c] = -INFINITY; a.out.U3[c] = -INFINITY; a.out.i2[c] = 0x7fffffff;
    }
  }
}

__global__ __launch_bounds__(64) void resume_store_kernel(DevState* st, unsigned long long* stat) {
  if (threadIdx.x == 0 && st->halt == HALT_NEED_EXACT && stat[SCR_ARMED]) {
    st->active = 1; st->halt = HALT_NONE; st->exact_mode = 0;
// ... 181 lines not shown
```

bayesian-coresets_amd/csrc/tail_core.h:

```cpp
#pragma once
#include "bcx_internal.h"
#include "dev_util.h"
#include "apply_common.h"
#include "resolve_core.h"

struct StateVecs {
  double *xw, *b, *bn, *xf, *tx;
};

template <bool BIG> static __device__ __forceinline__ double* vec_base(const ApplyArgs& a, double* dyn) {
  return BIG ? a.tmp + 8 * (size_t)a.d : dyn;
}
static __device__ __forceinline__ StateVecs carve(double* dyn, int d) {
  StateVecs v;
  v.xw = dyn; v.b = dyn + d; v.bn = dyn + 2 * (size_t)d; v.xf = dyn + 3 * (size_t)d; v.tx = dyn + 4 * (size_t)d;
  return v;
}

static __device__ __forceinline__ void stage_state(const ApplyArgs& a, const StateVecs& v) {
  for (int j = threadIdx.x; j < a.d; j += blockDim.x) {
    v.xw[j] = a.xw[j];
    v.b[j] = a.b[j];
    v.bn[j] = a.bn[j];
  }
}

#define SLOT_PRE 4
struct SlotPre {
  long long id[SLOT_PRE];
  double w[SLOT_PRE];
  int k;
  double nw, err0, bnorm, sigma, tol;
  int64_t it, itrs;
  int retried, since;
};
static __device__ __forceinline__ SlotPre slot_prefetch(const ApplyArgs& a) {
  SlotPre p;
  const DevState* st = a.st;
  p.k = st->k;
  p.nw = st->nw; p.err0 = st->err; p.bnorm = st->bnorm; p.sigma = st->sigma; p.tol = st->tol;
  p.it = st->it; p.itrs = st->itrs; p.retried = st->retried; p.since = st->since_refresh;
#pragma unroll
  for (int t = 0; t < SLOT_PRE; ++t) {
    const int s = threadIdx.x + t * blockDim.x;
    const bool ok = s < p.k;
    p.id[t] = ok ? a.act_idx[s] : -1;
    p.w[t] = ok ? a.act_w[s] : 0.0;
  }
  return p;
}

template <int ALG>
static __device__ void apply_core(const ApplyArgs& a, const StateVecs& v, int64_t f, double nf, double* scratch,
                                  const SlotPre& pre) {
  DevState* st = a.st;
  __shared__ int s_slot, s_npos;
  __shared__ double s_wf;
  const int tid = threadIdx.x, d = a.d;
  const int k = pre.k;
  const double nw = pre.nw, err0 = pre.err0, bnorm = pre.bnorm, sigma = pre.sigma, tol = pre.tol;
  const int64_t it = pre.it, itrs = pre.itrs;
  const int retried = pre.retried, since = pre.since;
  if (tid == 0) { s_slot = 0x7fffffff; s_npos = 0; }
  __syncthreads();
  {
    int npos = 0, slot = 0x7fffffff;
    double wf = 0.0;
    if (k <= SLOT_PRE * (int)blockDim.x) {
#pragma unroll
      for (int t = 0; t < SLOT_PRE; ++t) {
        if (pre.id[t] == f && pre.id[t] >= 0) { slot = tid + t * blockDim.x; wf = pre.w[t]; }
        if (pre.w[t] > 0.0) ++npos;
      }
    } else {
      for (int s = tid; s < k; s += blockDim.x) {
        const int64_t id = a.act_idx[s];
        const double w = a.act_w[s];
        if (id == f) { slot = s; wf = w; }
        if (w > 0.0) ++npos;
      }
    }
    if (slot != 0x7fffffff) { atomicMin(&s_slot, slot); s_wf = wf; }
#pragma unroll
    for (int off = 32; off >= 1; off >>= 1) npos += __shfl_xor(npos, off, BCX_WAVE);
    if ((tid & 63) == 0 && npos) atomicAdd(&s_npos, npos);
  }
  __syncthreads();
  BCX_STAMP(st, 5);
  const bool checked = s_npos > 0;
  const int slot = s_slot == 0x7fffffff ? -1 : s_slot;
  const double wf_old = slot >= 0 ? s_wf : 0.0;
  int status = BCX_IT_OK;
  double alpha = 0.0, beta = 0.0;
  if (ALG == BCX_ALG_GIGA) {
    double r[3] = {0.0, 0.0, 0.0};
    for (int j = tid; j < d; j += blockDim.x) {
      const double xh = v.xw[j] / nw, fh = v.xf[j] / nf, bj = v.bn[j];
      r[0] += bj * fh; r[1] += bj * xh; r[2] += xh * fh;
    }
    block_allsum<3>(r, scratch);
    const double gA = r[0] - r[1] * r[2];
    const double gB = r[1] - r[0] * r[2];
    if (gA <= 0.0 || gB < 0.0) {
      status = BCX_IT_FAIL_REWEIGHT;
    } else {
      const double ca = gB / (gA + gB) / nw;
      const double cb = gA / (gA + gB) / nf;
      double u[2] = {0.0, 0.0};
      for (int j = tid; j < d; j += blockDim.x) {
        const double x = ca * v.xw[j] + cb * v.xf[j];
        u[0] += x * x;
        u[1] += x * v.bn[j];
      }
      block_allsum<2>(u, scratch);
      const double nx = sqrt(u[0]);
      const double scale = bnorm / nx * (u[1] / nx);
      alpha = ca * scale; beta = cb * scale;
    }
  } else {
    if (!checked) {
      alpha = 0.0; beta = sigma / nf;
    } else {
      const double sc = sigma / nf;
      double r[2] = {0.0, 0.0};
      for (int j = tid; j < d; j += blockDim.x) {
        const double vv = sc * v.xf[j] - v.xw[j];
        r[0] += vv * (v.b[j] - v.xw[j]);
        r[1] += vv * vv;
      }
      block_allsum<2>(r, scratch);
      const double gnum = r[0], gden = r[1];
      if (gnum < 0.0 || gden == 0.0 || gnum > gden) status = BCX_IT_FAIL_REWEIGHT;
      else { alpha = 1.0 - gnum / gden; beta = sc * gnum / gden; }
    }
  }
  BCX_STAMP(st, 6);
  double new_err = err0, new_nw = nw, tdot = 0.0, wf_new = 0.0;
  if (status == BCX_IT_OK) {
    const double wf_scaled = alpha * wf_old;
    wf_new = fmax(0.0, wf_scaled + beta);
    const double delta = wf_new - wf_scaled;
    double r[3] = {0.0, 0.0, 0.0};
    for (int j = tid; j < d; j += blockDim.x) {
      const double x = alpha * v.xw[j] + delta * v.xf[j];
      v.tx[j] = x;
      const double e = x - v.b[j];
      r[0] += e * e; r[1] += x * x;
      if (ALG == BCX_ALG_GIGA) r[2] += v.bn[j] * x;
    }
    block_allsum<3>(r, scratch);
    new_err = sqrt(r[0]);
    const double n2 = sqrt(r[1]);
    new_nw = n2 == 0.0 ? 1.0 : n2;
    tdot = r[2];
    if (checked && !st->no_monotone && new_err > err0) status = BCX_IT_FAIL_MONOTONE;
  }
  BCX_STAMP(st, 7);
  bool limit = false;
  if (status == BCX_IT_OK) {
    for (int s = tid; s < k; s += blockDim.x)
      if (s != slot) a.act_w[s] = alpha * a.act_w[s];
    for (int j = tid; j < d; j += blockDim.x) { const double x = v.tx[j]; a.xw[j] = x; v.xw[j] = x; }
    const int dst = slot >= 0 ? slot : k;
    if (slot < 0)
      for (int j = tid; j < d; j += blockDim.x) a.act_rows[(size_t)dst * d + j] = v.xf[j];
    if (tid == 0) {
      a.act_w[dst] = wf_new;
      if (slot < 0) { a.act_idx[dst] = f; a.act_norm[dst] = nf; st->k = k + 1; }
      st->err = new_err;
      st->nw = new_nw;
      st->since_refresh = since + 1;
      if (checked && !st->no_monotone) st->retried = 0;
    }
  } else {
    limit = retried != 0;
  }
  if (tid == 0) {
    a.tr_sel[it] = f; a.tr_err[it] = (status == BCX_IT_OK) ? new_err : err0; a.tr_status[it] = status;
    st->it = it + 1;
    st->exact_mode = 0;
    if (status != BCX_IT_OK) {
      if (limit) { st->limit = 1; st->active = 0; st->halt = HALT_LIMIT; }
      else st->retried = 1;
    }
  }
  BCX_STAMP(st, 8);
  if (limit) return;
  const bool fast = status == BCX_IT_OK && it + 1 < itrs &&
                    !(a.refresh_every > 0 && since + 1 >= a.refresh_every);
  if (fast) {
    if (ALG != BCX_ALG_GIGA) {
      const int E = query_exponent(a, new_err);
      for (int j = tid; j < d; j += blockDim.x) store_query(a, 0, j, v.b[j] - v.xw[j], E);
      if (tid == 0) set_query_scale(st, new_err, E);
      BCX_STAMP(st, 9);
      return;
    }
    const double t = tdot / new_nw;
    double c2[1] = {0.0};
    for (int j = tid; j < d; j += blockDim.x) {
      const double c = v.bn[j] - t * (v.xw[j] / new_nw);
      v.tx[j] = c;
      c2[0] += c * c;
    }
    block_allsum<1>(c2, scratch);
    const double cn = sqrt(c2[0]);
    if (!(cn < tol)) {
      for (int j = tid; j < d; j += blockDim.x) {
        store_query(a, 0, j, v.tx[j] / cn);
        store_query(a, 1, j, v.xw[j] / new_nw);
      }
      if (tid == 0) set_query_scale(st, 1.0, 0);
      BCX_STAMP(st, 9);
      return;
    }
  }
  __syncthreads();
  prepare_next(a, scratch);
}
```

include/bcx.h:

```cpp
#ifndef BCX_H
#define BCX_H

#include <stdint.h>

#ifdef __cplusplus
extern "C" {
#endif

typedef struct bcx_solver bcx_solver;

enum { BCX_ALG_GIGA = 0, BCX_ALG_FW = 1, BCX_ALG_OMP = 2 };
enum { BCX_F32 = 0, BCX_F64 = 1, BCX_F16 = 2 };

enum {
  BCX_OK = 0,
  BCX_ERR_ARG = -1,
  BCX_ERR_HIP = -2,
  BCX_ERR_ZERO_ROW = -3,
  BCX_ERR_ZERO_B = -4,
  BCX_ERR_NOMEM = -5,
  BCX_ERR_STATE = -6,
  BCX_ERR_EXCHANGE = -7,
  BCX_ERR_TIMEOUT = -8
};

enum {
  BCX_IT_OK = 0,
  BCX_IT_FAIL_SELECT = 1,
  BCX_IT_FAIL_REWEIGHT = 2,
  BCX_IT_FAIL_MONOTONE = 3
};

typedef struct bcx_config {
  int32_t alg;
  int32_t store_dtype;
  int32_t keep_exact_rows;
  int32_t device;
  int32_t d;
  int32_t world_size;
  int32_t rank;
  int32_t refresh_every;
  int64_t n_local;
  int64_t n_global;
  int64_t row_offset;
} bcx_config;

#define BCX_MAX_ROW_LENGTH 1048576
int bcx_create(const bcx_config* cfg, bcx_solver** out);
int bcx_destroy(bcx_solver* s);
const char* bcx_last_error(const bcx_solver* s);
int bcx_set_stream(bcx_solver* s, void* hip_stream);

int bcx_load_rows(bcx_solver* s, const void* src, int32_t src_is_device, int32_t src_dtype,
                  int64_t row_begin, int64_t rows, int64_t ld);
#define BCX_LOAD_CENTER_ROWS 1
int bcx_load_rows_flags(bcx_solver* s, const void* src, int32_t src_is_device, int32_t src_dtype,
                        int64_t row_begin, int64_t rows, int64_t ld, int32_t flags);
int bcx_chunk_sums(bcx_solver* s, const void** dev_ptr, int64_t* n_chunks, int64_t* chunk_rows);
int bcx_export_chunk_sums(bcx_solver* s, void* dst_dev, int64_t cap_chunks);
int bcx_finalize(bcx_solver* s, const double* b_host, const void* gathered_sums_dev, int64_t n_gathered);

int bcx_build_begin(bcx_solver* s, int64_t itrs, double tol, int32_t* skip);
int bcx_step_scan(bcx_solver* s, void* send_dev);
int bcx_step_apply(bcx_solver* s, const void* recv_dev);
int bcx_build_enqueue(bcx_solver* s, int64_t itrs);
int bcx_build_enqueue_exact(bcx_solver* s);
int bcx_exchange_export(bcx_solver* s, void* handle_out, int32_t handle_bytes);
int bcx_exchange_attach(bcx_solver* s, const void* handles, int32_t handle_bytes, double timeout_s);
int bcx_exchange_probe(bcx_solver* s, int32_t* result);
int bcx_exchange_set_timeout(bcx_solver* s, double timeout_s);
int bcx_exchange_disable(bcx_solver* s);
int bcx_exchange_stats(bcx_solver* s, int64_t* n, double* wait_us_mean, double* wait_us_max, double* total_us_mean,
                       double* total_us_max, int32_t reset);
int bcx_build_poll(bcx_solver* s, int64_t* n_done, int32_t* need_exact, int32_t* limit);
int bcx_step_scan_exact(bcx_solver* s, void* send_dev);
int bcx_build_trace(bcx_solver* s, int64_t* sel, double* err, int32_t* status, int64_t cap, int64_t* n_out);

int bcx_active_count(bcx_solver* s, int64_t* k);
int bcx_get_weights(bcx_solver* s, int64_t* idx, double* w, int64_t cap, int64_t* k);
int bcx_error(bcx_solver* s, double* err);
int bcx_optimize(bcx_solver* s, double tol, int32_t* accepted);
int bcx_reset(bcx_solver* s);
int bcx_set_check_monotone(bcx_solver* s, int32_t on);
int bcx_reached_numeric_limit(bcx_solver* s, int32_t* limit);

int bcx_get_vector(bcx_solver* s, int32_t which, double* out);
int bcx_get_norms(bcx_solver* s, int64_t begin, int64_t count, double* out);
int bcx_get_stored_rows(bcx_solver* s, int64_t begin, int64_t count, void* out, int32_t* ld_out);
int bcx_argmax_correlation(bcx_solver* s, const double* query_host, int64_t* idx, double* score);
int bcx_time_scan(bcx_solver* s, int32_t reps, int32_t exact, double* ms_per_launch, double* bytes_per_launch);
int bcx_stats(bcx_solver* s, int64_t* exact_fallbacks, int64_t* candidates, int64_t* resolves);
int bcx_screen_stats(bcx_solver* s, int64_t* out8);
int bcx_screen4_stats(bcx_solver* s, int64_t* out8);
int bcx_screen_read(bcx_solver* s, int64_t begin, int64_t count, void* codes, float* scales, float* bounds, int32_t* ld8_out);
int bcx_screen4_read(bcx_solver* s, int64_t begin, int64_t count, void* codes, float* scales, float* bounds, int32_t* ld4_out);
#define BCX_SCREEN4_MAX_WAVES 2048
int bcx_screen4_probe(bcx_solver* s, const double* query_host, const int32_t* sentinels, int32_t* n_waves_out,
                      int32_t* counts, int32_t* list, int32_t list_stride, void* partials);
int bcx_omp_stats(bcx_solver* s, int64_t* out4);
int bcx_profile_scan(bcx_solver* s, int32_t on);
int bcx_profile_read(bcx_solver* s, double* scan_ms_total, int64_t* scan_launches);
int bcx_project_write(void* stream, int32_t family, const void* Z_dev, int64_t N, int64_t ldz, int32_t D,
                      int32_t ycol, const void* theta_dev, int32_t S, int32_t ldt, double param,
                      void* out_dev, int64_t ldo, void* rowsum_dev);
int bcx_project_write_raw(void* stream, int32_t family, const void* Z_dev, int64_t N, int64_t ldz, int32_t D,
                          int32_t ycol, const void* theta_dev, int32_t S, int32_t ldt, double param,
                          void* out_dev, int64_t ldo);
int bcx_project_write_points(void* stream, int32_t family, const void* Z_dev, int64_t N, int64_t ldz, int32_t D,
                             int32_t ycol, const void* theta_dev, int32_t S, int32_t ldt, double param,
                             void* out_dev, int64_t ldo, int32_t center);
int bcx_project_colsum(void* stream, int32_t family, const void* Z_dev, int64_t N, int64_t ldz, int32_t D,
                       int32_t ycol, const void* theta_dev, int32_t S, int32_t ldt, double param,
                       void* colsum_dev, void* work_dev);
int bcx_project_select(void* stream, int32_t family, const void* Z_dev, int64_t N, int64_t ldz, int32_t D,
                       int32_t ycol, const void* theta_dev, int32_t S, int32_t ldt, double param,
                       const void* resid_dev, double resid_sum, void* result_dev, void* work_dev);
int64_t bcx_project_select_scratch_bytes(int32_t family, int64_t N, int32_t S);
int bcx_project_select_ws(void* stream, int32_t family, const void* Z_dev, int64_t N, int64_t ldz, int32_t D,
                          int32_t ycol, const void* theta_dev, int32_t S, int32_t ldt, double param,
                          const void* resid_dev, double resid_sum, void* result_dev, void* work_dev, int64_t work_bytes);
int bcx_project_colsum_rows(void* stream, int32_t family, const void* Z_dev, int64_t N, int64_t ldz, int32_t D,
                            int32_t ycol, const void* theta_dev, int32_t S, int32_t ldt, double param,
                            const void* rows_dev, int64_t n_rows, void* colsum_dev, void* work_dev);
int64_t bcx_project_select_rows_scratch_bytes(int32_t family, int64_t n_rows, int32_t S);
int bcx_project_select_rows_ws(void* stream, int32_t family, const void* Z_dev, int64_t N, int64_t ldz, int32_t D,
                               int32_t ycol, const void* theta_dev, int32_t S, int32_t ldt, double param,
                               const void* rows_dev, int64_t n_rows, const void* resid_dev, double resid_sum,
                               void* result_dev, void* work_dev, int64_t work_bytes);
int bcx_gather_rows(void* stream, const void* Z_dev, int64_t ldz, int32_t C, const void* rows_dev, int64_t n_rows,
                    void* out_dev, int64_t ldo);
int64_t bcx_project_moments_scratch_bytes(int64_t N, int32_t C);
int64_t bcx_project_colsum_moments_scratch_bytes(int32_t D, int32_t S);
int bcx_project_moments(void* stream, const void* Z_dev, int64_t N, int64_t ldz, int32_t C, void* M_dev, int64_t ldm,
                        void* work_dev, int64_t work_bytes);
int bcx_project_colsum_moments(void* stream, const void* M_dev, int64_t ldm, int32_t D, int32_t ycol,
                               const void* theta_dev, int32_t S, int32_t ldt, double sigsq, void* colsum_dev, void* work_dev);
int bcx_project_colsum_moments_at(void* stream, const void* M_dev, int64_t ldm, int32_t D, int32_t ycol,
                                  const void* theta_dev, int32_t S, int32_t ldt, double sigsq, void* colsum_dev, void* work_dev,
                                  const void* tbar_dev);
int bcx_project_points_colsum_moments(void* stream, const void* Zc_dev, int64_t Nc, int64_t ldzc, int32_t D, int32_t ycol,
                                      const void* theta_dev, int32_t S, int32_t ldt, double sigsq, void* out_dev, int64_t ldo,
                                      const void* M_dev, int64_t ldm, int32_t ycol_m, void* colsum_dev, void* work_dev,
                                      const void* tbar_dev);
int bcx_linreg_posterior_draw(void* stream, int32_t k, int32_t D, int32_t ld, const void* w_dev, const void* K0_dev,
                              const void* xmu0_dev, const void* y_dev, const void* XU0_dev, const void* XS0_dev,
                              const void* U0T_dev, const void* mu0_dev, double sigsq, const void* R_dev, const void* Rbar_dev,
                              int32_t S, void* theta_dev, void* tbar_dev);
int bcx_linreg_posterior_apply_ok(int32_t k, int32_t ld);
int bcx_linreg_posterior_apply(void* stream, int32_t k, int32_t D, int32_t ld, const void* w_dev, const void* K0_dev,
                               const void* xmu0_dev, const void* y_dev, const void* X_dev, const void* XS0_dev,
                               const void* mu0_dev, double sigsq, const void* G_dev, const void* Gbar_dev, int32_t S,
                               void* theta_dev, void* tbar_dev, const void* gscale_dev);
int bcx_sparsevi_adam_step(void* stream, int32_t k, int32_t S, const void* colsum_dev, double scaling, const void* core_dev,
                           int64_t ldc, void* w_dev, void* mom1_dev, void* mom2_dev, const void* sched_dev, int32_t step,
                           double b1, double b2, double eps, void* trace_dev, int32_t core_is_raw);
int bcx_standard_normal(void* stream, uint64_t seed, uint64_t offset, int64_t count, void* out_dev);
int bcx_column_means(void* stream, const void* rows_dev, int32_t nblocks, int32_t n, int32_t ld, int64_t block_stride,
                     void* out_dev, int64_t out_stride);
int64_t bcx_sparsevi_adam_scratch_bytes(int32_t k, int32_t S);
int bcx_sparsevi_adam_step_ws(void* stream, int32_t k, int32_t S, const void* colsum_dev, double scaling, const void* core_dev,
                              int64_t ldc, void* w_dev, void* mom1_dev, void* mom2_dev, const void* sched_dev, int32_t step,
                              double b1, double b2, double eps, void* trace_dev, int32_t core_is_raw, void* work_dev,
                              int64_t work_bytes);
int64_t bcx_quasi_newton_scratch_bytes(int32_t k, int32_t S);
int bcx_quasi_newton_step(void* stream, int32_t k, int32_t S, const void* colsum_dev, double scaling, const void* core_dev,
                          int64_t ldc, int32_t core_is_raw, void* w_dev, const void* sched_dev, int32_t step, double tau,
                          void* dir_dev, void* trace_dev, void* status_dev, void* work_dev, int64_t work_bytes);
int64_t bcx_linreg_posterior_factor_scratch_bytes(int32_t D);
int bcx_linreg_posterior_factor(void* stream, int32_t k, int32_t D, int32_t ldx, const void* w_dev, const void* XT_dev,
                                const void* y_dev, const void* S0inv_dev, int32_t lds0, const void* rhs0_dev, double sigsq,
                                void* work_dev, int64_t work_bytes, void* U_dev, int64_t ldu, void* u_dev, void* mu_dev);
int bcx_linreg_posterior_factor_clear_status(void* stream, int32_t D, void* work_dev);
int bcx_linreg_posterior_factor_status(void* stream, int32_t D, const void* work_dev);
int bcx_linreg_posterior_draw_factored(void* stream, int32_t D, int32_t ld, const void* U_dev, int64_t ldu, const void* u_dev,
                                       const void* R_dev, const void* Rbar_dev, int32_t S, void* theta_dev, void* tbar_dev);
int bcx_laplace_sampler_ok(int32_t k, int32_t D);
int64_t bcx_laplace_sampler_lds_bytes(int32_t k, int32_t D);
int bcx_laplace_sampler(void* stream, int32_t family, int32_t k, int32_t D, const void* w_dev, const void* pts_dev, int64_t ldp,
                        void* mu_dev, int32_t warm, double tol, int32_t max_iter, const void* R_dev, const void* Rbar_dev,
                        int32_t S, int32_t ld, void* theta_dev, void* tbar_dev, void* status_dev);
int64_t bcx_laplace_stream_scratch_bytes(int32_t k, int32_t D);
// ... 115 lines not shown
```

Measured before the change: 2356.

## Precompute 4-bit screen query head in apply tail, reuse via generation tag

Moves computation of the front4 screening head (quantised query bit-planes, scale and error bounds) out of every scan block and into the previous iteration's apply tail. The result goes into a device record tagged with a query generation counter, and the scan kernel reuses it when the generation matches, falling back to recomputing it otherwise. This removes redundant per-block head work from the scan. In exchange it adds a qgen field, extra atomics, and extra work and synchronisation in the tail kernel.

```diff
diff --git a/bayesian-coresets_amd/bayesiancoresets_amd/_native.py b/bayesian-coresets_amd/bayesiancoresets_amd/_native.py
--- a/bayesian-coresets_amd/bayesiancoresets_amd/_native.py
+++ b/bayesian-coresets_amd/bayesiancoresets_amd/_native.py
@@ -22,7 +22,7 @@
     "bcx_finalize", "bcx_build_begin", "bcx_step_scan", "bcx_step_apply", "bcx_build_enqueue", "bcx_build_poll",
     "bcx_step_scan_exact", "bcx_build_trace", "bcx_active_count", "bcx_get_weights", "bcx_error", "bcx_optimize",
     "bcx_reset", "bcx_reached_numeric_limit", "bcx_get_vector", "bcx_get_norms", "bcx_get_stored_rows", "bcx_argmax_correlation", "bcx_time_scan",
-    "bcx_stats", "bcx_screen_stats", "bcx_screen4_stats", "bcx_screen_read", "bcx_screen4_read", "bcx_screen4_probe", "bcx_profile_scan", "bcx_profile_read", "bcx_version",
+    "bcx_stats", "bcx_screen_stats", "bcx_screen4_stats", "bcx_screen_read", "bcx_screen4_read", "bcx_screen4_probe", "bcx_screen4_probe_head", "bcx_screen4_head_read", "bcx_profile_scan", "bcx_profile_read", "bcx_version",
     "bcx_project_write", "bcx_project_colsum", "bcx_project_select", "bcx_project_last_error",
     "bcx_build_enqueue_exact", "bcx_exchange_export", "bcx_exchange_attach", "bcx_exchange_probe", "bcx_exchange_disable", "bcx_exchange_set_timeout",
     "bcx_set_check_monotone", "bcx_project_profile", "bcx_project_profile_read", "bcx_exchange_stats", "bcx_load_rows_flags", "bcx_project_write_raw", "bcx_omp_stats", "bcx_project_select_ws", "bcx_project_select_scratch_bytes",
@@ -152,6 +152,8 @@
         "bcx_screen_read": [vp, i64, i64, vp, vp, vp, P(i32)],
         "bcx_screen4_read": [vp, i64, i64, vp, vp, vp, P(i32)],
         "bcx_screen4_probe": [vp, vp, vp, P(i32), vp, vp, i32, vp],
+        "bcx_screen4_probe_head": [vp, vp, vp, P(i32), vp, vp, i32, vp, P(i32)],
+        "bcx_screen4_head_read": [vp, vp, vp, vp, P(i32)],
         "bcx_profile_scan": [vp, i32],
         "bcx_profile_read": [vp, P(dbl), P(i64)],
         "bcx_build_enqueue_exact": [vp],
@@ -550,13 +552,14 @@
     def screen_stats(self):
         out = (ctypes.c_int64 * 8)()
         self._check(self.lib.bcx_screen_stats(self.h, out))
-        o4 = (ctypes.c_int64 * 8)()
+        o4 = (ctypes.c_int64 * 9)()
         self._check(self.lib.bcx_screen4_stats(self.h, o4))
         return {"active": bool(out[0]), "screened": out[1], "survivors": out[2], "overflows": out[3], "storage_redos": out[4],
                 "state": self.SCREEN_DROP.get(int(out[5]), "?"), "device_bytes": out[6], "build_us": out[7],
                 "front4_active": bool(o4[0]), "front4_iterations": o4[1], "front4_listed": o4[2], "front4_overflows": o4[3],
                 "front4_redos": o4[4], "front4_state": self.SCREEN4_STATE.get(int(o4[5]), "?"), "front4_device_bytes": o4[6],
-                "front4_drops": o4[7]}
+                "front4_drops": o4[7],
+                "front4_head_hits": o4[8]}
 
     def screen_read(self, begin=0, count=None):
         count = self.n_local - begin if count is None else count
@@ -584,7 +587,7 @@
 
     SCREEN4_MAX_WAVES = 2048
 
-    def screen4_probe(self, query, sentinels, list_stride=1024):
+    def screen4_probe(self, query, sentinels, list_stride=1024, head_kernel=False):
         q = np.ascontiguousarray(query, dtype=np.float64)
         sent = np.ascontiguousarray(sentinels, dtype=np.int32)
         assert q.shape == (self.d,) and sent.shape == (64,)
@@ -593,13 +596,31 @@
         counts = np.zeros(cap, dtype=np.int32)
         lst = np.full((cap, list_stride), -1, dtype=np.int32)
         raw = np.zeros(cap * 40, dtype=np.uint8)
-        self._check(self.lib.bcx_screen4_probe(self.h, q.ctypes.data, sent.ctypes.data, ctypes.byref(nw), counts.ctypes.data,
-                                               lst.ctypes.data, list_stride, raw.ctypes.data))
+        hit = ctypes.c_int32(0)
+        if head_kernel:
+            self._check(self.lib.bcx_screen4_probe_head(self.h, q.ctypes.data, sent.ctypes.data, ctypes.byref(nw), counts.ctypes.data,
+                                                        lst.ctypes.data, list_stride, raw.ctypes.data, ctypes.byref(hit)))
+        else:
+            self._check(self.lib.bcx_screen4_probe(self.h, q.ctypes.data, sent.ctypes.data, ctypes.byref(nw), counts.ctypes.data,
+                                                   lst.ctypes.data, list_stride, raw.ctypes.data))
         n = nw.value
         dbl = raw[:32 * n].view(np.float64).reshape(4, n)
         idx = raw[32 * n:40 * n].view(np.int32).reshape(2, n)
-        return {"counts": counts[:n].copy(), "list": lst[:n].copy(), "U1": dbl[0].copy(), "U2": dbl[1].copy(), "U3": dbl[2].copy(),
-                "L": dbl[3].copy(), "i1": idx[0].copy(), "i2": idx[1].copy()}
+        out = {"counts": counts[:n].copy(), "list": lst[:n].copy(), "U1": dbl[0].copy(), "U2": dbl[1].copy(), "U3": dbl[2].copy(),
+               "L": dbl[3].copy(), "i1": idx[0].copy(), "i2": idx[1].copy()}
+        if head_kernel:
+            out["head_hit"] = bool(hit.value)
+        return out
+
+    def screen4_head_read(self):
+        gen = (ctypes.c_uint64 * 2)()
+        sc = np.zeros(4, dtype=np.float32)
+        planes = np.zeros(3 * 512, dtype=np.uint32)
+        nw4 = ctypes.c_int32()
+        self._check(self.lib.bcx_screen4_head_read(self.h, gen, sc.ctypes.data, planes.ctypes.data, ctypes.byref(nw4)))
+        n = nw4.value
+        return {"gen": int(gen[0]), "query_gen": int(gen[1]), "Lg": sc[0], "qstep": sc[1], "eA": sc[2], "eB": sc[3],
+                "planes": planes[:3 * n].reshape(3, n).copy()}
 
     def omp_stats(self):
         out = (ctypes.c_int64 * 4)()
diff --git a/bayesian-coresets_amd/csrc/api.hip b/bayesian-coresets_amd/csrc/api.hip
--- a/bayesian-coresets_amd/csrc/api.hip
+++ b/bayesian-coresets_amd/csrc/api.hip
@@ -36,7 +36,7 @@
   for (size_t w = 0; w < s->peer_mbox.size(); ++w)
     if (s->peer_mbox[w] && s->peer_mbox[w] != s->mbox) (void)hipIpcCloseMemHandle(s->peer_mbox[w]);
   void* xptrs[] = {s->mbox, s->peer_tab, s->xseq, s->xprobe, s->rec_gather, s->grid_counter, s->fin_part, s->gram_work, s->warm_buf,
-                   s->Aq, s->scr_sb, s->scr_partials, s->scr_stat, s->A4, s->s4_sb, s->s4_list, s->s4_counts, s->s4_sent};
+                   s->Aq, s->scr_sb, s->scr_partials, s->scr_stat, s->A4, s->s4_sb, s->s4_list, s->s4_counts, s->s4_sent, s->s4_head};
   for (void* p : xptrs)
     if (p) (void)hipFree(p);
   for (auto& ev : s->prof_events) { (void)hipEventDestroy(ev.first); (void)hipEventDestroy(ev.second); }
@@ -63,6 +63,7 @@
   if (s->cfg.refresh_every == 0) s->cfg.refresh_every = 64;
   if (const char* e = bcx_dev_env("BCX_SCREEN8")) s->scr_enabled = atoi(e) != 0;
   if (const char* e = bcx_dev_env("BCX_SCREEN4_SEGCAP")) { const int v = atoi(e); if (v >= 1 && v <= BCX_S4_SEG_CAP) s->s4_seg_cap = v; }
+  if (const char* e = bcx_dev_env("BCX_S4_HEAD")) s->s4_head_on = atoi(e) != 0;
   if (const char* e = bcx_dev_env("BCX_SCREEN4")) s->s4_enabled = atoi(e) != 0;
   hipError_t e = hipSetDevice(cfg->device);
   if (e != hipSuccess) { g_create_err = std::string("hipSetDevice: ") + hipGetErrorString(e); delete s; return BCX_ERR_HIP; }
@@ -494,7 +495,9 @@
   for (int64_t i = 0; i < itrs; ++i) {
     s->scr_batch = tier;
     const bool four = tier4 && s->s4_warm == 0;
+    s->s4_head_next = tier4 && i + 1 < itrs && s->s4_warm <= 1;
     rc = enqueue_one(s, 0, tier, four);
+    s->s4_head_next = false;
     if (rc != BCX_OK) return rc;
     if (tier && s->s4_warm > 0) s->s4_warm -= 1;
   }
@@ -911,6 +914,7 @@
     BCX_HIP(hipMemcpy(rec, s->rec_local, sizeof rec, hipMemcpyDeviceToHost));
     if (rec[3] != BCX_REC_OVERFLOW) break;
   }
+  h.qgen += 1;
   BCX_HIP(hipMemcpy(s->st, &h, sizeof h, hipMemcpyHostToDevice));
   if (rec[3] != BCX_REC_VALID) { s->err = "no rows to scan"; return BCX_ERR_STATE; }
   *idx = (int64_t)rec[1];
@@ -931,7 +935,7 @@
 
 extern "C" int bcx_screen_stats(bcx_solver* s, int64_t* out8) {
   if (!s || !out8) return BCX_ERR_ARG;
-  unsigned long long st8[SCR_WORDS] = {0, 0, 0, 0, 0, 0, 0, 0};
+  unsigned long long st8[SCR_WORDS] = {0};
   if (s->scr_stat) {
     BCX_HIP(hipSetDevice(s->cfg.device));
     BCX_HIP(hipStreamSynchronize(s->stream));
@@ -949,7 +953,8 @@
   return BCX_OK;
 }
 
-extern "C" int bcx_screen4_stats(bcx_solver* s, int64_t* out8) {
+extern "C" int bcx_screen4_stats(bcx_solver* s, int64_t* out9) {
+  int64_t* out8 = out9;
   if (!s || !out8) return BCX_ERR_ARG;
   unsigned long long st8[SCR_WORDS];
   for (auto& w : st8) w = 0;
@@ -968,6 +973,7 @@
   out8[5] = !possible ? 3 : s->s4_dropped;
   out8[6] = s->A4 ? (int64_t)s->s4_cap_rows * (s->ld4 + 8) + (int64_t)BCX_MAX_PARTIALS * (BCX_S4_SEG_CAP + 1) * 4 : 0;
   out8[7] = s->s4_drops;
+  out9[8] = (int64_t)st8[SCR4_HEAD_HITS];
   return BCX_OK;
 }
 
@@ -1021,8 +1027,8 @@
   return BCX_OK;
 }
 
-extern "C" int bcx_screen4_probe(bcx_solver* s, const double* query_host, const int32_t* sentinels, int32_t* n_waves_out,
-                                 int32_t* counts, int32_t* list, int32_t list_stride, void* partials) {
+static int screen4_probe(bcx_solver* s, const double* query_host, const int32_t* sentinels, int32_t* n_waves_out,
+                         int32_t* counts, int32_t* list, int32_t list_stride, void* partials, bool with_head, int32_t* head_hit) {
   if (!s || !query_host || !sentinels || !n_waves_out || list_stride < 0) return BCX_ERR_ARG;
   for (int i = 0; i < BCX_S4_SENTINELS; ++i)
     if (!(sentinels[i] == -1 || (sentinels[i] >= 0 && (int64_t)sentinels[i] < s->cfg.n_local))) {
@@ -1044,10 +1050,12 @@
   if ((rc = upload_query(s, query_host, false, &qn, &E))) return rc;
   DevState forced = h;
   forced.active = 1; forced.exact_mode = 0; forced.qscale = qn; forced.qexp = E;
+  forced.qgen = h.qgen + 1;
+  h.qgen += 2;
   BCX_HIP(hipMemcpy(s->st, &forced, sizeof forced, hipMemcpyHostToDevice));
   BCX_HIP(hipMemcpy(s->s4_sent, sentinels, sizeof sent_was, hipMemcpyHostToDevice));
   int nw = 0;
-  rc = bcx_launch_front4_probe(s, &nw);
+  rc = bcx_launch_front4_probe(s, &nw, with_head);
   hipError_t e = hipStreamSynchronize(s->stream);
   BCX_HIP(hipMemcpy(s->st, &h, sizeof h, hipMemcpyHostToDevice));
   BCX_HIP(hipMemcpy(s->s4_sent, sent_was, sizeof sent_was, hipMemcpyHostToDevice));
@@ -1055,6 +1063,7 @@
   if (rc != BCX_OK) return rc;
   BCX_HIP(e);
   *n_waves_out = nw;
+  if (head_hit) BCX_HIP(hipMemcpy(head_hit, (const int*)s->s4_counts + BCX_MAX_PARTIALS, 4, hipMemcpyDeviceToHost));
   std::vector<int32_t> cnt((size_t)nw);
   BCX_HIP(hipMemcpy(cnt.data(), s->s4_counts, (size_t)nw * 4, hipMemcpyDeviceToHost));
   if (counts) memcpy(counts, cnt.data(), (size_t)nw * 4);
@@ -1071,6 +1080,33 @@
   return BCX_OK;
 }
 
+extern "C" int bcx_screen4_probe(bcx_solver* s, const double* query_host, const int32_t* sentinels, int32_t* n_waves_out,
+                                 int32_t* counts, int32_t* list, int32_t list_stride, void* partials) {
+  return screen4_probe(s, query_host, sentinels, n_waves_out, counts, list, list_stride, partials, false, nullptr);
+}
+
+extern "C" int bcx_screen4_probe_head(bcx_solver* s, const double* query_host, const int32_t* sentinels, int32_t* n_waves_out,
+                                      int32_t* counts, int32_t* list, int32_t list_stride, void* partials, int32_t* head_hit) {
+  return screen4_probe(s, query_host, sentinels, n_waves_out, counts, list, list_stride, partials, true, head_hit);
+}
+
+extern "C" int bcx_screen4_head_read(bcx_solver* s, uint64_t* gen2, float* scalars4, uint32_t* planes, int32_t* nw4_out) {
+  if (!s) return BCX_ERR_ARG;
+  int rc = screen4_ready(s, "bcx_screen4_head_read");
+  if (rc != BCX_OK) return rc;
+  DevState h;
+  if ((rc = read_state(s, &h))) return rc;
+  BCX_HIP(hipStreamSynchronize(s->stream));
+  std::vector<S4HeadRec> r(1);
+  BCX_HIP(hipMemcpy(r.data(), s->s4_head, sizeof(S4HeadRec), hipMemcpyDeviceToHost));
+  const int nw4 = s->ld4 / 4;
+  if (gen2) { gen2[0] = r[0].gen; gen2[1] = h.qgen; }
+  if (scalars4) { scalars4[0] = r[0].Lg; scalars4[1] = r[0].qstep; scalars4[2] = r[0].eA; scalars4[3] = r[0].eB; }
+  if (planes) memcpy(planes, r[0].planes, (size_t)3 * nw4 * 4);
+  if (nw4_out) *nw4_out = nw4;
+  return BCX_OK;
+}
+
 extern "C" int bcx_omp_stats(bcx_solver* s, int64_t* out4) {
   if (!s || !out4) return BCX_ERR_ARG;
   DevState h;
diff --git a/bayesian-coresets_amd/csrc/apply_common.h b/bayesian-coresets_amd/csrc/apply_common.h
--- a/bayesian-coresets_amd/csrc/apply_common.h
+++ b/bayesian-coresets_amd/csrc/apply_common.h
@@ -30,24 +30,30 @@
   return (a.store_f64 || !(qnorm > 0.0) || !(qnorm < INFINITY)) ? 0 : ilogb(qnorm);
 }
 
-static __device__ __forceinline__ void store_query(const ApplyArgs& a, int which, int j, double v, int E = 0) {
+static __device__ __forceinline__ float store_query(const ApplyArgs& a, int which, int j, double v, int E = 0) {
   a.q64[(size_t)which * a.ld64 + j] = v;
-  if (a.store_f64) ((double*)a.qst)[(size_t)which * a.ld + j] = v;
-  else ((float*)a.qst)[(size_t)which * a.ld + j] = (float)(E ? ldexp(v, -E) : v);
+  if (a.store_f64) { ((double*)a.qst)[(size_t)which * a.ld + j] = v; return (float)v; }
+  const float f = (float)(E ? ldexp(v, -E) : v);
+  ((float*)a.qst)[(size_t)which * a.ld + j] = f;
+  return f;
 }
 
 static __device__ __forceinline__ void set_query_scale(DevState* st, double qnorm, int E) {
   st->qscale = E ? ldexp(qnorm, -E) : qnorm;
   st->qexp = E;
+  atomicAdd(&st->qgen, 1ull);
 }
 
-static __device__ bool prepare_query(const ApplyArgs& a, double* scratch) {
+static __device__ bool prepare_query(const ApplyArgs& a, double* scratch, float* qcopy = nullptr) {
   DevState* st = a.st;
   const int d = a.d;
   if (a.alg != BCX_ALG_GIGA) {
     const double qn = st->err;
     const int E = query_exponent(a, qn);
-    for (int j = threadIdx.x; j < d; j += blockDim.x) store_query(a, 0, j, a.b[j] - a.xw[j], E);
+    for (int j = threadIdx.x; j < d; j += blockDim.x) {
+      const float qf = store_query(a, 0, j, a.b[j] - a.xw[j], E);
+      if (qcopy) qcopy[j] = qf;
+    }
     if (threadIdx.x == 0) set_query_scale(st, qn, E);
     return true;
   }
@@ -109,7 +115,7 @@
   __syncthreads();
 }
 
-static __device__ void prepare_next(const ApplyArgs& a, double* scratch) {
+static __device__ bool prepare_next(const ApplyArgs& a, double* scratch, float* qcopy = nullptr) {
   DevState* st = a.st;
   __shared__ int go;
   for (;;) {
@@ -119,10 +125,10 @@
       if (st->it >= st->itrs) { st->active = 0; st->halt = HALT_DONE; go = 0; }
     }
     __syncthreads();
-    if (!go) return;
+    if (!go) return false;
     if (a.refresh_every > 0 && st->since_refresh >= a.refresh_every) refresh_state(a, scratch, true);
-    const bool ok = prepare_query(a, scratch);
-    if (ok) return;
+    const bool ok = prepare_query(a, scratch, qcopy);
+    if (ok) return true;
     __syncthreads();
     if (threadIdx.x == 0) {
       const int64_t it = st->it;
@@ -132,7 +138,7 @@
       else st->retried = 1;
     }
     __syncthreads();
-    if (!go) return;
+    if (!go) return false;
   }
 }
 
diff --git a/bayesian-coresets_amd/csrc/bcx_internal.h b/bayesian-coresets_amd/csrc/bcx_internal.h
--- a/bayesian-coresets_amd/csrc/bcx_internal.h
+++ b/bayesian-coresets_amd/csrc/bcx_internal.h
@@ -35,9 +35,17 @@
        SCR4_LISTED = 6,
        SCR4_OVERFLOWS = 7,
        SCR4_LAST = 8,
-       SCR_WORDS = 9 };
+       SCR4_HEAD_HITS = 9,
+       SCR_WORDS = 10 };
 #define BCX_S4_SEG_CAP 1024
 #define BCX_S4_SENTINELS 64
+#define BCX_S4_MAX_NW4 512
+struct S4HeadRec {
+  unsigned long long gen;
+  float Lg, qstep, eA, eB;
+  unsigned pad[2];
+  unsigned planes[3 * BCX_S4_MAX_NW4];
+};
 static inline __host__ __device__ PartialView partial_view(void* base, int n) {
   PartialView v;
   v.U1 = (double*)base; v.U2 = v.U1 + n; v.U3 = v.U2 + n; v.L = v.U3 + n;
@@ -89,6 +97,7 @@
   double qscale;
   int32_t qexp;
   int32_t qexp_pad;
+  unsigned long long qgen;
   long long dbg_t[32];
 };
 
@@ -183,6 +192,9 @@
   void* s4_list = nullptr;
   void* s4_counts = nullptr;
   void* s4_sent = nullptr;
+  S4HeadRec* s4_head = nullptr;
+  bool s4_head_on = true;
+  bool s4_head_next = false;
   int ld4 = 0;
   int s4_seg_cap = BCX_S4_SEG_CAP;
   int64_t s4_cap_rows = 0;
@@ -234,7 +246,7 @@
 bool bcx_screen4_on(const bcx_solver* s);
 int bcx_screen4_build(bcx_solver* s);
 int bcx_launch_screen4(bcx_solver* s);
-int bcx_launch_front4_probe(bcx_solver* s, int* n_waves);
+int bcx_launch_front4_probe(bcx_solver* s, int* n_waves, bool with_head);
 void bcx_project_set_error(const std::string& msg);
 const double* proj_tables();
 
diff --git a/bayesian-coresets_amd/csrc/front4_head.h b/bayesian-coresets_amd/csrc/front4_head.h
--- /dev/null
+++ b/bayesian-coresets_amd/csrc/front4_head.h
@@ -0,0 +1,196 @@
+#pragma once
+#include <float.h>
+#include "screen_core.h"
+
+#define BCX_S4_QMAX 1911.0
+#define BCX_S4_SPW (BCX_S4_SENTINELS / BCX_SCREEN_WAVES)
+
+struct Front4Head { float Lg, qstep, eA, eB; };
+
+struct Front4HeadIn {
+  const unsigned char* Aq;
+  const float2* sb8;
+  const int* sent;
+  int64_t n;
+  int ld8, d, nw4;
+  float kacc, err_coef;
+};
+
+struct Front4Rows { unsigned cw[2][BCX_S4_SPW]; };
+
+static __device__ __forceinline__ float round_up_f32(double v) {
+  float f = (float)v;
+  if ((double)f < v) f = nextafterf(f, INFINITY);
+  return f;
+}
+
+static __device__ __forceinline__ int front4_row_load(const Front4HeadIn& a) {
+  return a.sent[(threadIdx.x >> 6) * BCX_S4_SPW + (threadIdx.x & (BCX_S4_SPW - 1))];
+}
+static __device__ __forceinline__ int front4_row_ok(const Front4HeadIn& a, int myrow) {
+  return (myrow >= 0 && (int64_t)myrow < a.n) ? myrow : -1;
+}
+
+static __device__ __forceinline__ void front4_rows_of(int myrow, int (&rows)[BCX_S4_SPW]) {
+#pragma unroll
+  for (int r = 0; r < BCX_S4_SPW; ++r) rows[r] = __builtin_amdgcn_readlane(myrow, r);
+}
+
+static __device__ __forceinline__ void front4_rows_trip(const Front4HeadIn& a, const int (&rows)[BCX_S4_SPW], int w0,
+                                                        unsigned (&cw)[2][BCX_S4_SPW]) {
+  const int nw8 = a.ld8 / 4;
+  const unsigned* A8 = (const unsigned*)a.Aq;
+#pragma unroll
+  for (int h = 0; h < 2; ++h) {
+    const int w = w0 + 64 * h;
+    const int wc = w < nw8 ? w : 0;
+#pragma unroll
+    for (int r = 0; r < BCX_S4_SPW; ++r) cw[h][r] = A8[(int64_t)(rows[r] < 0 ? 0 : rows[r]) * nw8 + wc];
+  }
+}
+
+static __device__ __forceinline__ Front4Rows front4_head_rows(const Front4HeadIn& a, int myrow) {
+  int rows[BCX_S4_SPW];
+  front4_rows_of(myrow, rows);
+  Front4Rows f;
+  front4_rows_trip(a, rows, threadIdx.x & 63, f.cw);
+  return f;
+}
+
+template <class Q>
+static __device__ __forceinline__ Front4Head front4_head(const Front4HeadIn& a, int myrow, float2 mysb, const Front4Rows& first,
+                                                         float qscale, Q q, unsigned* planes, double* scratch) {
+  const int tid = threadIdx.x, lane = tid & 63, wave = tid >> 6;
+  constexpr int NW = BCX_SCREEN_WAVES;
+  constexpr int SPW = BCX_S4_SPW;
+  int rows[SPW];
+  front4_rows_of(myrow, rows);
+  double acc[SPW];
+#pragma unroll
+  for (int r = 0; r < SPW; ++r) acc[r] = 0.0;
+  double m = 0.0;
+  const int nw8 = a.ld8 / 4;
+  for (int w0 = lane; w0 < nw8; w0 += 128) {
+    unsigned cw[2][SPW];
+    float qf[2][4];
+#pragma unroll
+    for (int h = 0; h < 2; ++h) {
+      const int w = w0 + 64 * h;
+#pragma unroll
+      for (int k = 0; k < 4; ++k) { const int j = 4 * w + k; qf[h][k] = q((w < nw8 && j < a.d) ? j : 0); }
+    }
+    if (w0 == lane) {
+#pragma unroll
+      for (int h = 0; h < 2; ++h)
+#pragma unroll
+        for (int r = 0; r < SPW; ++r) cw[h][r] = first.cw[h][r];
+    } else {
+      front4_rows_trip(a, rows, w0, cw);
+    }
+    __builtin_amdgcn_sched_barrier(0);
+    double qv[2][4];
+#pragma unroll
+    for (int h = 0; h < 2; ++h)
+#pragma unroll
+      for (int k = 0; k < 4; ++k) {
+        const int w = w0 + 64 * h, j = 4 * w + k;
+        qv[h][k] = (w < nw8 && j < a.d) ? (double)qf[h][k] : 0.0;
+        const double v = fabs(qv[h][k]);
+        m = fmax(m, v == v ? v : INFINITY);
+      }
+#pragma unroll
+    for (int h = 0; h < 2; ++h)
+#pragma unroll
+      for (int r = 0; r < SPW; ++r)
+#pragma unroll
+        for (int k = 0; k < 4; ++k) acc[r] = fma((double)((int)((cw[h][r] >> (8 * k)) & 0xffu) - 128), qv[h][k], acc[r]);
+  }
+  double tot = 0.0;
+#pragma unroll
+  for (int r = 0; r < SPW; ++r) { const double t = wave_allsum(acc[r]); tot = (lane & (SPW - 1)) == r ? t : tot; }
+  float lmax = -INFINITY;
+  {
+    const float s0 = (float)((double)mysb.x * tot);
+    float U, L;
+    screen_interval(s0, mysb.x, mysb.y, a.kacc, a.err_coef, qscale, U, L);
+    if (myrow >= 0) lmax = fmaxf(lmax, L);
+  }
+  lmax = (float)wave_allmax((double)lmax);
+  m = wave_allmax(m);
+  float step = (float)(m / BCX_S4_QMAX);
+  const bool qok = m < INFINITY && step >= FLT_MIN;
+  if (!qok) step = 0.0f;
+  double err2 = 0.0;
+  for (int w = tid; w < a.nw4; w += BCX_SCAN_THREADS) {
+    unsigned p0 = 0, p1 = 0, p2 = 0;
+    float q8[8];
+#pragma unroll
+    for (int k = 0; k < 8; ++k) { const int j = 8 * w + k; q8[k] = q(j < a.d ? j : 0); }
+#pragma unroll
+    for (int k = 0; k < 8; ++k) {
+      const int j = 8 * w + k;
+      int x = 0;
+      if (j < a.d && qok) {
+        const double v = (double)q8[k];
+        double c = rint(v / (double)step);
+        c = c > BCX_S4_QMAX ? BCX_S4_QMAX : (c < -BCX_S4_QMAX ? -BCX_S4_QMAX : c);
+        x = (int)c;
+        const double r = v - c * (double)step;
+        err2 = fma(r, r, err2);
+      }
+      const int l = ((x + 8) & 15) - 8;
+      const int x1 = (x - l) >> 4;
+      const int h1 = ((x1 + 8) & 15) - 8;
+      const int h2 = (x1 - h1) >> 4;
+      p0 |= (unsigned)(l & 15) << (4 * k); p1 |= (unsigned)(h1 & 15) << (4 * k); p2 |= (unsigned)(h2 & 15) << (4 * k);
+    }
+    planes[w] = p0; planes[a.nw4 + w] = p1; planes[2 * a.nw4 + w] = p2;
+  }
+  err2 = wave_allsum(err2);
+  if (lane == 0) { scratch[wave] = err2; scratch[NW + wave] = (double)lmax; }
+  __syncthreads();
+  err2 = scratch[0];
+  double lg = scratch[NW];
+#pragma unroll
+  for (int w = 1; w < NW; ++w) { err2 += scratch[w]; lg = fmax(lg, scratch[NW + w]); }
+  const double qerr = sqrt(err2) * (1.0 + 9.5367431640625e-07);
+  const double qs = (double)qscale;
+  Front4Head h;
+  h.Lg = qok ? (float)lg : -INFINITY;
+  h.qstep = step;
+  h.eA = round_up_f32((qs * 1.000002 + qerr) * 1.000004);
+  h.eB = round_up_f32(((double)a.err_coef * qs + 1.001 * qerr) * 1.000004 + 1e-37);
+  return h;
+}
+
+static __device__ __forceinline__ void front4_head_publish(S4HeadRec* rec, const Front4Head& h, unsigned long long gen) {
+  rec->Lg = h.Lg; rec->qstep = h.qstep; rec->eA = h.eA; rec->eB = h.eB;
+  rec->gen = gen;
+}
+
+struct TailHeadArgs {
+  int on;
+  Front4HeadIn in;
+  S4HeadRec* rec;
+};
+
+struct HeadPre { int myrow; float2 mysb; Front4Rows rows; };
+static __device__ __forceinline__ int head_prefetch_row(const TailHeadArgs& th) {
+  return th.on ? front4_row_load(th.in) : -1;
+}
+static __device__ __forceinline__ HeadPre head_prefetch_rest(const TailHeadArgs& th, int myrow) {
+  HeadPre p;
+  p.myrow = -1; p.mysb = make_float2(0.f, 0.f);
+#pragma unroll
+  for (int h = 0; h < 2; ++h)
+#pragma unroll
+    for (int r = 0; r < BCX_S4_SPW; ++r) p.rows.cw[h][r] = 0u;
+  if (th.on) {
+    p.myrow = front4_row_ok(th.in, myrow);
+    p.mysb = th.in.sb8[p.myrow < 0 ? 0 : p.myrow];
+    p.rows = front4_head_rows(th.in, p.myrow);
+  }
+  return p;
+}
+
+void bcx_front4_tail_head(bcx_solver* s, bool next_is_four, TailHeadArgs* th);
diff --git a/bayesian-coresets_amd/csrc/resolve.hip b/bayesian-coresets_amd/csrc/resolve.hip
--- a/bayesian-coresets_amd/csrc/resolve.hip
+++ b/bayesian-coresets_amd/csrc/resolve.hip
@@ -5,6 +5,7 @@
 
 #include "resolve_core.h"
 #include "tail_core.h"
+#include "front4_head.h"
 
 
 __global__ __launch_bounds__(256) void resolve_kernel(ResolveArgs a) {
@@ -50,7 +51,7 @@
 }
 
 template <int ALG, bool BIG>
-__global__ __launch_bounds__(BCX_APPLY_THREADS) void tail_kernel(ResolveArgs r, ApplyArgs a) {
+__global__ __launch_bounds__(BCX_APPLY_THREADS) void tail_kernel(ResolveArgs r, ApplyArgs a, TailHeadArgs th) {
   DevState* st = a.st;
   if (!st->active) return;
   extern __shared__ double dyn[];
@@ -58,12 +59,37 @@
   __shared__ Winner win;
   BCX_STAMP(st, 0);
   const StateVecs v = carve(vec_base<BIG>(a, dyn), a.d);
+  int hrow = -1;
+  if (ALG == BCX_ALG_FW) hrow = head_prefetch_row(th);
   const SlotPre pre = slot_prefetch(a);
   stage_state(a, v);
+  HeadPre hp;
+  if (ALG == BCX_ALG_FW) hp = head_prefetch_rest(th, hrow);
   resolve_core(r, &win, v.xf, scratch);
   if (win.flags == BCX_REC_OVERFLOW) { if (threadIdx.x == 0) { st->active = 0; st->halt = HALT_NEED_EXACT; } return; }
   if (win.flags != BCX_REC_VALID) { if (threadIdx.x == 0) { st->active = 0; st->halt = HALT_DONE; } return; }
-  apply_core<ALG>(a, v, win.gidx, win.norm, scratch, pre);
+  const bool wrote = apply_core<ALG>(a, v, win.gidx, win.norm, scratch, pre);
+  if (ALG == BCX_ALG_FW) {
+    if (!(th.on && wrote)) return;
+    unsigned long long gen = 0;
+    float qscale = 0.f;
+    if (BIG) __threadfence();
+    __syncthreads();
+    gen = __hip_atomic_load(&st->qgen, __ATOMIC_RELAXED, __HIP_MEMORY_SCOPE_AGENT);
+    qscale = (float)__longlong_as_double((long long)__hip_atomic_load((const unsigned long long*)&st->qscale, __ATOMIC_RELAXED,
+                                                                      __HIP_MEMORY_SCOPE_AGENT));
+    Front4Head h;
+    if (BIG) {
+      const unsigned* qs = (const unsigned*)a.qst;
+      h = front4_head(th.in, hp.myrow, hp.mysb, hp.rows, qscale,
+                      [&](int j) { return __uint_as_float(__hip_atomic_load(qs + j, __ATOMIC_RELAXED, __HIP_MEMORY_SCOPE_AGENT)); },
+                      th.rec->planes, scratch);
+    } else {
+      const float* qc = (const float*)v.tx;
+      h = front4_head(th.in, hp.myrow, hp.mysb, hp.rows, qscale, [&](int j) { return qc[j]; }, th.rec->planes, scratch);
+    }
+    if (threadIdx.x == 0) front4_head_publish(th.rec, h, gen);
+  }
 }
 
 static __device__ __forceinline__ void st_sys(double* p, double v) {
@@ -311,19 +337,21 @@
   r.need_score = 0;
   ApplyArgs a;
   fill_apply_args(s, a, nullptr);
+  TailHeadArgs th;
+  bcx_front4_tail_head(s, s->s4_head_next && s->cfg.alg == BCX_ALG_FW, &th);
   const size_t lds = vec_lds_bytes(s);
   int rc;
   if (s->cfg.alg == BCX_ALG_GIGA) {
-    if (vec_big(s)) hipLaunchKernelGGL((tail_kernel<BCX_ALG_GIGA, true>), dim3(1), dim3(BCX_APPLY_THREADS), 0, s->stream, r, a);
+    if (vec_big(s)) hipLaunchKernelGGL((tail_kernel<BCX_ALG_GIGA, true>), dim3(1), dim3(BCX_APPLY_THREADS), 0, s->stream, r, a, th);
     else {
       if ((rc = allow_lds(s, tail_kernel<BCX_ALG_GIGA, false>, lds))) return rc;
-      hipLaunchKernelGGL((tail_kernel<BCX_ALG_GIGA, false>), dim3(1), dim3(BCX_APPLY_THREADS), lds, s->stream, r, a);
+      hipLaunchKernelGGL((tail_kernel<BCX_ALG_GIGA, false>), dim3(1), dim3(BCX_APPLY_THREADS), lds, s->stream, r, a, th);
     }
   } else {
-    if (vec_big(s)) hipLaunchKernelGGL((tail_kernel<BCX_ALG_FW, true>), dim3(1), dim3(BCX_APPLY_THREADS), 0, s->stream, r, a);
+    if (vec_big(s)) hipLaunchKernelGGL((tail_kernel<BCX_ALG_FW, true>), dim3(1), dim3(BCX_APPLY_THREADS), 0, s->stream, r, a, th);
     else {
       if ((rc = allow_lds(s, tail_kernel<BCX_ALG_FW, false>, lds))) return rc;
-      hipLaunchKernelGGL((tail_kernel<BCX_ALG_FW, false>), dim3(1), dim3(BCX_APPLY_THREADS), lds, s->stream, r, a);
+      hipLaunchKernelGGL((tail_kernel<BCX_ALG_FW, false>), dim3(1), dim3(BCX_APPLY_THREADS), lds, s->stream, r, a, th);
     }
   }
   BCX_HIP(hipGetLastError());
diff --git a/bayesian-coresets_amd/csrc/screen4.hip b/bayesian-coresets_amd/csrc/screen4.hip
--- a/bayesian-coresets_amd/csrc/screen4.hip
+++ b/bayesian-coresets_amd/csrc/screen4.hip
@@ -1,11 +1,9 @@
 #include <float.h>
+#include <string.h>
 #include "screen_core.h"
+#include "front4_head.h"
 
 #define BCX_S4_CLIP 0.8
-#define BCX_S4_QMAX 1911.0
-#define BCX_S4_MAX_NW4 512
-
-struct Front4Head { float Lg, qstep, eA, eB; };
 
 template <int CTRL> __device__ __forceinline__ int dpp_mov_i(int v) { return __builtin_amdgcn_update_dpp(0, v, CTRL, 0xf, 0xf, false); }
 template <int G> __device__ __forceinline__ int group_allsum_i32(int v) {
@@ -16,12 +14,6 @@
   if (G >= 32) { const v2u r = __builtin_amdgcn_permlane16_swap((unsigned)v, (unsigned)v, false, false); const unsigned x = r.x, y = r.y; v = (int)(x + y); }
   if (G >= 64) { const v2u r = __builtin_amdgcn_permlane32_swap((unsigned)v, (unsigned)v, false, false); const unsigned x = r.x, y = r.y; v = (int)(x + y); }
   return v;
-}
-
-static __device__ __forceinline__ float round_up_f32(double v) {
-  float f = (float)v;
-  if ((double)f < v) f = nextafterf(f, INFINITY);
-  return f;
 }
 
 struct Front4Args {
@@ -40,109 +32,13 @@
   float kacc, err_coef;
   PartialView out;
   int ldv8;
+  S4HeadRec* rec;
+  int use_rec;
 };
 
-#define BCX_S4_SPW (BCX_S4_SENTINELS / BCX_SCREEN_WAVES)
-
-static __device__ __forceinline__ Front4Head front4_head(const Front4Args& a, int myrow, float2 mysb, float qscale,
-                                                         unsigned* planes, double* scratch) {
-  const int tid = threadIdx.x, lane = tid & 63, wave = tid >> 6;
-  constexpr int NW = BCX_SCREEN_WAVES;
-  constexpr int SPW = BCX_S4_SPW;
-  int rows[SPW];
-#pragma unroll
-  for (int r = 0; r < SPW; ++r) rows[r] = __builtin_amdgcn_readlane(myrow, r);
-  double acc[SPW];
-#pragma unroll
-  for (int r = 0; r < SPW; ++r) acc[r] = 0.0;
-  double m = 0.0;
-  const int nw8 = a.ld8 / 4;
-  const unsigned* A8 = (const unsigned*)a.Aq;
-  for (int w0 = lane; w0 < nw8; w0 += 128) {
-    unsigned cw[2][SPW];
-    float qf[2][4];
-#pragma unroll
-    for (int h = 0; h < 2; ++h) {
-      const int w = w0 + 64 * h;
-      const int wc = w < nw8 ? w : 0;
-#pragma unroll
-      for (int k = 0; k < 4; ++k) { const int j = 4 * w + k; qf[h][k] = a.q[(w < nw8 && j < a.d) ? j : 0]; }
-#pragma unroll
-      for (int r = 0; r < SPW; ++r) cw[h][r] = A8[(int64_t)(rows[r] < 0 ? 0 : rows[r]) * nw8 + wc];
-    }
-    __builtin_amdgcn_sched_barrier(0);
-    double qv[2][4];
-#pragma unroll
-    for (int h = 0; h < 2; ++h)
-#pragma unroll
-      for (int k = 0; k < 4; ++k) {
-        const int w = w0 + 64 * h, j = 4 * w + k;
-        qv[h][k] = (w < nw8 && j < a.d) ? (double)qf[h][k] : 0.0;
-        const double v = fabs(qv[h][k]);
-        m = fmax(m, v == v ? v : INFINITY);
-      }
-#pragma unroll
-    for (int h = 0; h < 2; ++h)
-#pragma unroll
-      for (int r = 0; r < SPW; ++r)
-#pragma unroll
-        for (int k = 0; k < 4; ++k) acc[r] = fma((double)((int)((cw[h][r] >> (8 * k)) & 0xffu) - 128), qv[h][k], acc[r]);
-  }
-  double tot = 0.0;
-#pragma unroll
-  for (int r = 0; r < SPW; ++r) { const double t = wave_allsum(acc[r]); tot = (lane & (SPW - 1)) == r ? t : tot; }
-  float lmax = -INFINITY;
-  {
-    const float s0 = (float)((double)mysb.x * tot);
-    float U, L;
-    screen_interval(s0, mysb.x, mysb.y, a.kacc, a.err_coef, qscale, U, L);
-    if (myrow >= 0) lmax = fmaxf(lmax, L);
-  }
-  lmax = (float)wave_allmax((double)lmax);
-  m = wave_allmax(m);
-  float step = (float)(m / BCX_S4_QMAX);
-  const bool qok = m < INFINITY && step >= FLT_MIN;
-  if (!qok) step = 0.0f;
-  double err2 = 0.0;
-  for (int w = tid; w < a.nw4; w += BCX_SCAN_THREADS) {
-    unsigned p0 = 0, p1 = 0, p2 = 0;
-    float q8[8];
-#pragma unroll
-    for (int k = 0; k < 8; ++k) { const int j = 8 * w + k; q8[k] = a.q[j < a.d ? j : 0]; }
-#pragma unroll
-    for (int k = 0; k < 8; ++k) {
-      const int j = 8 * w + k;
-      int x = 0;
-      if (j < a.d && qok) {
-        const double v = (double)q8[k];
-        double c = rint(v / (double)step);
-        c = c > BCX_S4_QMAX ? BCX_S4_QMAX : (c < -BCX_S4_QMAX ? -BCX_S4_QMAX : c);
-        x = (int)c;
-        const double r = v - c * (double)step;
-        err2 = fma(r, r, err2);
-      }
-      const int l = ((x + 8) & 15) - 8;
-      const int x1 = (x - l) >> 4;
-      const int h1 = ((x1 + 8) & 15) - 8;
-      const int h2 = (x1 - h1) >> 4;
-      p0 |= (unsigned)(l & 15) << (4 * k); p1 |= (unsigned)(h1 & 15) << (4 * k); p2 |= (unsigned)(h2 & 15) << (4 * k);
-    }
-    planes[w] = p0; planes[a.nw4 + w] = p1; planes[2 * a.nw4 + w] = p2;
-  }
-  err2 = wave_allsum(err2);
-  if (lane == 0) { scratch[wave] = err2; scratch[NW + wave] = (double)lmax; }
-  __syncthreads();
-  err2 = scratch[0];
-  double lg = scratch[NW];
-#pragma unroll
-  for (int w = 1; w < NW; ++w) { err2 += scratch[w]; lg = fmax(lg, scratch[NW + w]); }
-  const double qerr = sqrt(err2) * (1.0 + 9.5367431640625e-07);
-  const double qs = (double)qscale;
-  Front4Head h;
-  h.Lg = qok ? (float)lg : -INFINITY;
-  h.qstep = step;
-  h.eA = round_up_f32((qs * 1.000002 + qerr) * 1.000004);
-  h.eB = round_up_f32(((double)a.err_coef * qs + 1.001 * qerr) * 1.000004 + 1e-37);
+static __device__ __forceinline__ Front4HeadIn head_in(const Front4Args& a) {
+  Front4HeadIn h;
+  h.Aq = a.Aq; h.sb8 = a.sb8; h.sent = a.sent; h.n = a.n; h.ld8 = a.ld8; h.d = a.d; h.nw4 = a.nw4; h.kacc = a.kacc; h.err_coef = a.err_coef;
   return h;
 }
 
@@ -215,12 +111,15 @@
 
 template <int G, int CH, int UR, int G8, int CH8, int UR8>
 __global__ __launch_bounds__(BCX_SCAN_THREADS) void front4_kernel(Front4Args a) {
-  int myrow = a.sent[(threadIdx.x >> 6) * BCX_S4_SPW + (threadIdx.x & (BCX_S4_SPW - 1))];
+  const Front4HeadIn hin = head_in(a);
+  int myrow = front4_row_load(hin);
   const float qscale = (float)a.st->qscale;
   const int active = a.st->active;
+  const unsigned long long qgen = a.st->qgen, rgen = a.rec->gen;
   asm volatile("" : "+v"(myrow));
   if (!active) return;
-  if (!(myrow >= 0 && (int64_t)myrow < a.n)) myrow = -1;
+  const bool hit = a.use_rec && qgen == rgen;
+  myrow = front4_row_ok(hin, myrow);
   const float2 mysb = a.sb8[myrow < 0 ? 0 : myrow];
   __shared__ double scratch[BCX_SCRATCH];
   __shared__ unsigned planes[3 * BCX_S4_MAX_NW4];
@@ -259,14 +158,30 @@
   int64_t r0 = (int64_t)blockIdx.x * RPB;
   load_trip(r0);
   __builtin_amdgcn_sched_barrier(0);
-  const Front4Head h = front4_head(a, myrow, mysb, qscale, planes, scratch);
+  Front4Head h;
   int qp[CH][4][3];
-#pragma unroll
-  for (int c = 0; c < CH; ++c)
-#pragma unroll
-    for (int k = 0; k < 4; ++k)
-#pragma unroll
-      for (int p = 0; p < 3; ++p) qp[c][k][p] = vok[c] ? (int)planes[p * a.nw4 + 4 * voff[c] + k] : 0;
+  if (hit) {
+    const S4HeadRec* rec = a.rec;
+    h.Lg = rec->Lg; h.qstep = rec->qstep; h.eA = rec->eA; h.eB = rec->eB;
+#pragma unroll
+    for (int c = 0; c < CH; ++c)
+#pragma unroll
+      for (int p = 0; p < 3; ++p) {
+        const uint4 t = *(const uint4*)(rec->planes + p * a.nw4 + 4 * voff[c]);
+        qp[c][0][p] = vok[c] ? (int)t.x : 0; qp[c][1][p] = vok[c] ? (int)t.y : 0;
+        qp[c][2][p] = vok[c] ? (int)t.z : 0; qp[c][3][p] = vok[c] ? (int)t.w : 0;
+      }
+  } else {
+    const float* q = a.q;
+    h = front4_head(hin, myrow, mysb, front4_head_rows(hin, myrow), qscale, [&](int j) { return q[j]; }, planes, scratch);
+#pragma unroll
+    for (int c = 0; c < CH; ++c)
+#pragma unroll
+      for (int k = 0; k < 4; ++k)
+#pragma unroll
+        for (int p = 0; p < 3; ++p) qp[c][k][p] = vok[c] ? (int)planes[p * a.nw4 + 4 * voff[c] + k] : 0;
+  }
+  if (blockIdx.x == 0 && threadIdx.x == 0) a.counts[BCX_MAX_PARTIALS] = hit ? 1 : 0;
   for (;;) {
     __builtin_amdgcn_sched_barrier(0);
 #pragma unroll
@@ -302,6 +217,19 @@
   }
   if (lane == 0) a.counts[b] = cnt;
   settle8<G8, CH8, UR8>(a, lseg[wave], b, cnt, qscale);
+}
+
+__global__ __launch_bounds__(BCX_SCAN_THREADS) void head4_kernel(Front4Args a) {
+  __shared__ double scratch[BCX_SCRATCH];
+  const Front4HeadIn hin = head_in(a);
+  const float qscale = (float)a.st->qscale;
+  const unsigned long long qgen = a.st->qgen;
+  const int myrow = front4_row_ok(hin, front4_row_load(hin));
+  const float2 mysb = a.sb8[myrow < 0 ? 0 : myrow];
+  const float* q = a.q;
+  const Front4Head h = front4_head(hin, myrow, mysb, front4_head_rows(hin, myrow), qscale, [&](int j) { return q[j]; },
+                                   a.rec->planes, scratch);
+  if (threadIdx.x == 0) front4_head_publish(a.rec, h, qgen);
 }
 
 template <bool F16>
@@ -360,14 +288,15 @@
   s->ld4 = (d + 31) / 32 * 16;
   const int nw4 = s->ld4 / 4;
   if (s->s4_cap_rows < n || !s->A4) {
-    void** all[] = {&s->A4, &s->s4_sb, &s->s4_list, &s->s4_counts, &s->s4_sent};
+    void** all[] = {&s->A4, &s->s4_sb, &s->s4_list, &s->s4_counts, &s->s4_sent, (void**)&s->s4_head};
     for (void** p : all) { if (*p) (void)hipFree(*p); *p = nullptr; }
     s->s4_cap_rows = 0;
     hipError_t e = hipMalloc(&s->A4, (size_t)n * s->ld4);
     if (e == hipSuccess) e = hipMalloc(&s->s4_sb, (size_t)n * 8);
     if (e == hipSuccess) e = hipMalloc(&s->s4_list, (size_t)BCX_MAX_PARTIALS * BCX_S4_SEG_CAP * 4);
-    if (e == hipSuccess) e = hipMalloc(&s->s4_counts, (size_t)BCX_MAX_PARTIALS * 4);
+    if (e == hipSuccess) e = hipMalloc(&s->s4_counts, (size_t)(BCX_MAX_PARTIALS + 1) * 4);
     if (e == hipSuccess) e = hipMalloc(&s->s4_sent, (size_t)BCX_S4_SENTINELS * 4);
+    if (e == hipSuccess) e = hipMalloc((void**)&s->s4_head, sizeof(S4HeadRec));
     if (e != hipSuccess) {
       (void)hipGetLastError();
       for (void** p : all) { if (*p) (void)hipFree(*p); *p = nullptr; }
@@ -376,6 +305,8 @@
     }
     s->s4_cap_rows = n;
     BCX_HIP(hipMemsetAsync(s->s4_sent, 0xff, (size_t)BCX_S4_SENTINELS * 4, s->stream));
+    BCX_HIP(hipMemsetAsync(s->s4_head, 0xff, sizeof(S4HeadRec), s->stream));
+    BCX_HIP(hipMemsetAsync((int*)s->s4_counts + BCX_MAX_PARTIALS, 0, 4, s->stream));
   }
   const unsigned grid = (unsigned)((n + 3) / 4);
   if (s->cfg.store_dtype == BCX_F16)
@@ -433,6 +364,7 @@
 
   const int n_in = grid * BCX_SCREEN_WAVES;
   f.out = partial_view(s->scr_partials, n_in); f.ldv8 = ldv8;
+  f.rec = s->s4_head; f.use_rec = s->s4_head_on ? 1 : 0;
   p->G = G; p->CH = CH; p->G8 = G8; p->CH8 = CH8; p->grid = grid; p->n_in = n_in;
   return BCX_OK;
 }
@@ -447,12 +379,28 @@
   return bcx_launch_refine(s, p.n_in, true);
 }
 
-int bcx_launch_front4_probe(bcx_solver* s, int* n_waves) {
+int bcx_launch_front4_probe(bcx_solver* s, int* n_waves, bool with_head) {
   Front4Plan p;
   int rc = front4_plan(s, &p);
   if (rc != BCX_OK) return rc;
+  if (with_head) {
+    p.f.use_rec = 1;
+    hipLaunchKernelGGL(head4_kernel, dim3(1), dim3(BCX_SCAN_THREADS), 0, s->stream, p.f);
+    BCX_HIP(hipGetLastError());
+  }
   if ((rc = launch_front4(s, p.f, p.G, p.CH, p.G8, p.CH8, p.grid))) return rc;
   BCX_HIP(hipGetLastError());
   *n_waves = p.n_in;
   return BCX_OK;
 }
+
+void bcx_front4_tail_head(bcx_solver* s, bool next_is_four, TailHeadArgs* th) {
+  memset(th, 0, sizeof *th);
+  Front4Plan p;
+  if (!next_is_four || !s->s4_head_on || !s->s4_head || !bcx_screen4_on(s) || !s->s4_valid || front4_plan(s, &p) != BCX_OK) return;
+  const Front4Args& f = p.f;
+  th->on = 1;
+  th->in.Aq = f.Aq; th->in.sb8 = f.sb8; th->in.sent = f.sent; th->in.n = f.n; th->in.ld8 = f.ld8; th->in.d = f.d; th->in.nw4 = f.nw4;
+  th->in.kacc = f.kacc; th->in.err_coef = f.err_coef;
+  th->rec = s->s4_head;
+}
diff --git a/bayesian-coresets_amd/csrc/screen8.hip b/bayesian-coresets_amd/csrc/screen8.hip
--- a/bayesian-coresets_amd/csrc/screen8.hip
+++ b/bayesian-coresets_amd/csrc/screen8.hip
@@ -153,6 +153,7 @@
     r1[t] = ok ? a.in.i1[p] : 0; r2[t] = ok ? a.in.i2[p] : 0;
     cn[t] = (ok && a.counts) ? a.counts[p] : 0;
   }
+  const int head_hit = (a.counts && tid == 0) ? a.counts[BCX_MAX_PARTIALS] : 0;
   if (tid == 0) { nsurv = 0; overflow = 0; listed = 0; full = 0; }
   double lmax = -INFINITY;
 #pragma unroll
@@ -190,6 +191,7 @@
       atomicAdd(&a.stat[SCR4_ITERS], 1ull);
       atomicAdd(&a.stat[SCR4_LISTED], (unsigned long long)listed);
       atomicAdd(&a.stat[SCR4_OVERFLOWS], (unsigned long long)full);
+      if (head_hit) atomicAdd(&a.stat[SCR4_HEAD_HITS], 1ull);
     }
   }
   auto stored = [&](int64_t i, int j) -> double {
diff --git a/bayesian-coresets_amd/csrc/tail_core.h b/bayesian-coresets_amd/csrc/tail_core.h
--- a/bayesian-coresets_amd/csrc/tail_core.h
+++ b/bayesian-coresets_amd/csrc/tail_core.h
@@ -51,7 +51,7 @@
 }
 
 template <int ALG>
-static __device__ void apply_core(const ApplyArgs& a, const StateVecs& v, int64_t f, double nf, double* scratch,
+static __device__ bool apply_core(const ApplyArgs& a, const StateVecs& v, int64_t f, double nf, double* scratch,
                                   const SlotPre& pre) {
   DevState* st = a.st;
   __shared__ int s_slot, s_npos;
@@ -185,16 +185,18 @@
     }
   }
   BCX_STAMP(st, 8);
-  if (limit) return;
+  if (limit) return false;
   const bool fast = status == BCX_IT_OK && it + 1 < itrs &&
                     !(a.refresh_every > 0 && since + 1 >= a.refresh_every);
   if (fast) {
     if (ALG != BCX_ALG_GIGA) {
       const int E = query_exponent(a, new_err);
-      for (int j = tid; j < d; j += blockDim.x) store_query(a, 0, j, v.b[j] - v.xw[j], E);
+      float* qcopy = (float*)v.tx;
+      __syncthreads();
+      for (int j = tid; j < d; j += blockDim.x) qcopy[j] = store_query(a, 0, j, v.b[j] - v.xw[j], E);
       if (tid == 0) set_query_scale(st, new_err, E);
       BCX_STAMP(st, 9);
-      return;
+      return true;
     }
     const double t = tdot / new_nw;
     double c2[1] = {0.0};
@@ -212,9 +214,10 @@
       }
       if (tid == 0) set_query_scale(st, 1.0, 0);
       BCX_STAMP(st, 9);
-      return;
+      return false;
     }
   }
   __syncthreads();
-  prepare_next(a, scratch);
-}
+  const bool wrote = prepare_next(a, scratch, ALG != BCX_ALG_GIGA ? (float*)v.tx : nullptr);
+  return wrote && ALG != BCX_ALG_GIGA;
+}
diff --git a/include/bcx.h b/include/bcx.h
--- a/include/bcx.h
+++ b/include/bcx.h
@@ -91,12 +91,15 @@
 int bcx_time_scan(bcx_solver* s, int32_t reps, int32_t exact, double* ms_per_launch, double* bytes_per_launch);
 int bcx_stats(bcx_solver* s, int64_t* exact_fallbacks, int64_t* candidates, int64_t* resolves);
 int bcx_screen_stats(bcx_solver* s, int64_t* out8);
-int bcx_screen4_stats(bcx_solver* s, int64_t* out8);
+int bcx_screen4_stats(bcx_solver* s, int64_t* out9);
 int bcx_screen_read(bcx_solver* s, int64_t begin, int64_t count, void* codes, float* scales, float* bounds, int32_t* ld8_out);
 int bcx_screen4_read(bcx_solver* s, int64_t begin, int64_t count, void* codes, float* scales, float* bounds, int32_t* ld4_out);
 #define BCX_SCREEN4_MAX_WAVES 2048
 int bcx_screen4_probe(bcx_solver* s, const double* query_host, const int32_t* sentinels, int32_t* n_waves_out,
                       int32_t* counts, int32_t* list, int32_t list_stride, void* partials);
+int bcx_screen4_probe_head(bcx_solver* s, const double* query_host, const int32_t* sentinels, int32_t* n_waves_out,
+                           int32_t* counts, int32_t* list, int32_t list_stride, void* partials, int32_t* head_hit);
+int bcx_screen4_head_read(bcx_solver* s, uint64_t* gen2, float* scalars4, uint32_t* planes, int32_t* nw4_out);
 int bcx_omp_stats(bcx_solver* s, int64_t* out4);
 int bcx_profile_scan(bcx_solver* s, int32_t on);
 int bcx_profile_read(bcx_solver* s, double* scan_ms_total, int64_t* scan_launches);
```

Result: no change. 2356 (median of 2 runs) (+0.0%).
